# tum-vision/LDSO

Measured on AMD Instinct MI355X. Metric: GN iters/sec + Mresiduals/sec, 7-KF/2000-pt window, higher is better.
Workload: dtype f32; 1 GPU; C3: 7 KF x 2000 pt x 8 px, 640x480, R=12000, forced GN iterations, synthetic rank-6 marginalisation prior H_M/b_M; arithmetic=f32 residuals / Jacobians / accumulators as the reference, f64 stitch and solve, parallelism=1 GPU

## Files before the change

### ldso_amd/csrc/ba_api.hip

```cpp
#include "ba_host.h"
#include "lie_dev.h"

static thread_local std::string g_err;
void ldso_set_error(const std::string &s) { g_err = s; }

extern "C" {

int ldso_version(void) { return 100; }
const char *ldso_last_error(void) { return g_err.c_str(); }
int ldso_device_count(void) { int n = 0; if (hipGetDeviceCount(&n) != hipSuccess) return 0; return n; }

int ldso_settings_default(ldso_settings_t *s) {
    if (!s) return LDSO_E_INVALID;
    memset(s, 0, sizeof(*s));
    s->huberTH = 9; s->outlierTHSumComponent = 50 * 50; s->affineOptModeA = 1e12f; s->affineOptModeB = 1e8f;
    s->frameEnergyTHN = 0.7f; s->frameEnergyTHFacMedian = 1.5f; s->frameEnergyTHConstWeight = 0.5f; s->overallEnergyTHWeight = 1;
    s->initialCalibHessian = 5e9f; s->margWeightFac = 0.5f * 0.5f; s->idepthFixPriorMargFac = 600 * 600; s->thOptIterations = 1.2f;
    s->coarseCutoffTH = 20; s->minOptIterations = 1; s->solverMode = LDSO_SOLVER_FIX_LAMBDA | LDSO_SOLVER_ORTHOGONALIZE_X_LATER;
    s->forceAcceptStep = 1; s->solverModeDelta = 0.00001;
    return LDSO_OK;
}

int ldso_pyr_levels_used(int w, int h) {
    int wl = w, hl = h, lv = 1;
// ... 38 lines not shown
#define DA(ptr, n) do { int r_ = dalloc(H, &(ptr), (n)); if (r_ != LDSO_OK) return r_; } while (0)
static int down_reserve(ldso_ba *H, size_t bytes) {
    if (bytes <= H->downCap) return LDSO_OK;
    CHK(hipStreamSynchronize(H->stream));
    if (H->h_down) (void) hipHostFree(H->h_down);
    H->h_down = nullptr; H->downCap = 0;
    const size_t cap = bytes + bytes / 2 + 4096;
    CHK(hipHostMalloc((void **) &H->h_down, cap));
    H->downCap = cap;
    return LDSO_OK;
}
template <class T> static const T *down_put(ldso_ba *H, size_t &used, const T *src, size_t n, int &rc) {
    const size_t bytes = (n * sizeof(T) + 63) & ~(size_t) 63;
    const T *p = reinterpret_cast<const T *>(H->h_down + used);
    if (rc == LDSO_OK && n) { if (hipMemcpyAsync(H->h_down + used, src, n * sizeof(T), hipMemcpyDeviceToHost, H->stream) != hipSuccess) { ldso_set_error("hipMemcpyAsync (fetch) failed"); rc = LDSO_E_HIP; } }
    used += bytes;
    return p;
}

template <class T> static int d2h(ldso_ba *H, std::vector<T> &dst, const T *src, size_t n) {
    dst.resize(n);
    if (n == 0) return LDSO_OK;
    CHK(hipMemcpyAsync(dst.data(), src, n * sizeof(T), hipMemcpyDeviceToHost, H->stream));
    return LDSO_OK;
}
extern "C" {

static int alloc_set(ldso_ba *H, ResSet &S) {
    const size_t P = H->maxP, FS = H->FSmax, PS = P * FS, C = H->maxChunks;
    DA(S.slot, PS); DA(S.pt, P); DA(S.acc, P); DA(S.candE, P);
    DA(S.G, P * (8 * FS + LD_GEXTRA)); DA(S.topA, C * FS * LD_TOPN); DA(S.topL, C * FS * LD_TOPN);
    DA(S.chunkEnergy, C); DA(S.chunkCnt, C * 2); DA(S.chunkNID, C * 2);
    return LDSO_OK;
}

static int create_body(ldso_ba *H, int device, int w, int h, int max_frames, int max_points);

int ldso_ba_create(int device, int w, int h, int max_frames, int max_points, ldso_ba_t **out) {
    REQ(out && w > 8 && h > 8 && max_frames >= 2 && max_frames <= LD_MAXF && max_points > 0, "ldso_ba_create: bad arguments");
    *out = nullptr;
    int ndev = 0;
    if (hipGetDeviceCount(&ndev) != hipSuccess || ndev <= 0) { ldso_set_error("no HIP device visible"); return LDSO_E_NODEVICE; }
    REQ(device >= 0 && device < ndev, "ldso_ba_create: device index out of range");
    CHK(hipSetDevice(device));
    ldso_ba *H = new ldso_ba();
    { const char *e = getenv("LDSO_GN_GRAPHS"); if (e && e[0] == '0') H->gnUseGraphs = false; }
    const int r = create_body(H, device, w, h, max_frames, max_points);
    if (r != LDSO_OK) { const std::string keep = g_err; ldso_ba_destroy(H); g_err = keep; return r; }
    *out = H;
    return LDSO_OK;
}

static int create_body(ldso_ba *H, int device, int w, int h, int max_frames, int max_points) {
    H->device = device; H->w = w; H->h = h; H->maxF = max_frames; H->maxP = max_points;
    H->FSmax = (max_frames + 7) / 8 * 8;
    H->maxChunks = max_points / 4 + max_frames + 4;
    { hipDeviceProp_t pr; if (hipGetDeviceProperties(&pr, device) == hipSuccess && pr.multiProcessorCount > 0) H->numCU = pr.multiProcessorCount; }
    ldso_settings_default(&H->settings);
    CHK(hipStreamCreateWithFlags(&H->stream, hipStreamNonBlocking));
    H->ownStream = true;
    CHK(hipHostMalloc((void **) &H->h_item, sizeof(BatchItem)));
    { void *q_ = nullptr; CHK(hipMalloc(&q_, sizeof(BatchItem))); H->d_item = (BatchItem *) q_; }
    { void *q_ = nullptr; CHK(hipMalloc(&q_, (size_t) H->maxChunks * sizeof(BatchBlock))); H->d_blocks = (BatchBlock *) q_; }
    CHK(hipHostMalloc((void **) &H->h_stop, 4 * sizeof(int), hipHostMallocMapped));
    CHK(hipHostGetDevicePointer((void **) &H->d_stop, H->h_stop, 0));
    memset(&H->B, 0, sizeof(H->B));
    memset(&H->D, 0, sizeof(H->D));
    BaPtrs &B = H->B;
    const size_t F = max_frames, P = max_points, FS = H->FSmax, nmax = 8 * F + 4;
    DA(B.frames, F); DA(B.calib, 1); DA(B.pairs, F * F); DA(B.pairRt, F * F * 12);
    DA(B.adHost, F * F * 64); DA(B.adTarget, F * F * 64); DA(B.adHostF, F * F * 64); DA(B.adTargetF, F * F * 64);
    DA(B.nsProj, nmax * 7); DA(B.HM, nmax * nmax); DA(B.bM, nmax);
    DA(B.pgeo, P); DA(B.pcw, P * 8); DA(B.phost, P);
    DA(B.rtab, P * FS);
    DA(B.Jlin, P * FS); DA(B.rtz, P * FS * 8);
    DA(B.chunk_p0, H->maxChunks); DA(B.chunk_n, H->maxChunks); DA(B.chunk_host, H->maxChunks);
    DA(H->d_chunkStart, F + 2);
    DA(H->d_waitCtr, 4);
    DA(H->d_margFlags, P);
    DA(B.pairC, 2 * F * F * LD_PAIRC);
    const size_t GSPmax = (8 * FS + LD_GEXTRA + 15) / 16 * 16;
    DA(B.scPart, (size_t) LD_SC_SPLITS * GSPmax * GSPmax);
    DA(B.sys, 4 * (nmax * nmax + nmax));
    DA(B.acc, nmax * nmax + nmax); H->ownAcc = B.acc;
    DA(B.x, nmax); DA(B.xAd, F * F * 8); DA(B.xc, 4); DA(B.scalars, 16); DA(B.energyLog, 64);
    DA(H->d_dumpJ, P * FS);
    B.dumpJ = nullptr;
    int r;
    if ((r = alloc_set(H, H->sets[0])) != LDSO_OK) return r;
    if ((r = alloc_set(H, H->sets[1])) != LDSO_OK) return r;
    return LDSO_OK;
}

int ldso_ba_destroy(ldso_ba_t *H) {
    if (!H) return LDSO_OK;
    REQ(H->inBatch == nullptr, "ldso_ba_destroy: the handle is part of a live batch (ldso_ba_batch_destroy first: the batch dereferences its handles)");
    hipSetDevice(H->device);
    hipDeviceSynchronize();
    for (void *p : H->allocs) hipFree(p);
    for (int i = 0; i < LD_MAXF; i++) if (H->imgOwned[i] && H->imgSlots[i]) hipFree(H->imgSlots[i]);
    if (H->d_color) hipFree(H->d_color);
    if (H->h_item) hipHostFree(H->h_item);
    if (H->d_item) hipFree(H->d_item);
    if (H->d_blocks) hipFree(H->d_blocks);
    if (H->h_stop) hipHostFree(H->h_stop);
    if (H->h_down) hipHostFree(H->h_down);
    if (H->h_stage) hipHostFree(H->h_stage);
    if (H->d_stage) hipFree(H->d_stage);
    if (H->d_act) hipFree(H->d_act);
    if (H->d_sel) hipFree(H->d_sel);
    if (H->distBuf) hipFree(H->distBuf);
    if (H->d_p2pErr) hipFree(H->d_p2pErr);
    for (auto &t : H->timers) { hipEventDestroy(t.a); hipEventDestroy(t.b); }
    for (ldso_ba::GnGraph &g : H->gnGraphs) { hipGraphExecDestroy(g.exec); hipGraphDestroy(g.graph); }
    if (H->ownStream && H->stream) hipStreamDestroy(H->stream);
    delete H;
    return LDSO_OK;
}

int ldso_ba_set_stream(ldso_ba_t *H, void *s) {
    REQ(H, "null handle");
    CHK(hipSetDevice(H->device));
    if (H->stream && (H->ownStream || H->stageBusy)) { CHK(hipStreamSynchronize(H->stream)); H->stageBusy = false; }
    if (H->ownStream && H->stream && s) { hipStreamDestroy(H->stream); H->ownStream = false; }
    if (s) { H->stream = (hipStream_t) s; H->ownStream = false; }
    else if (!H->ownStream) { CHK(hipStreamCreateWithFlags(&H->stream, hipStreamNonBlocking)); H->ownStream = true; }
    return LDSO_OK;
}

int ldso_ba_set_settings(ldso_ba_t *H, const ldso_settings_t *s) {
    REQ(H && s, "null argument");
    if (s->solverMode & (LDSO_SOLVER_SVD | LDSO_SOLVER_ORTHOGONALIZE_SYSTEM | LDSO_SOLVER_ORTHOGONALIZE_POINTMARG | LDSO_SOLVER_ORTHOGONALIZE_FULL |
                         LDSO_SOLVER_MOMENTUM | LDSO_SOLVER_STEPMOMENTUM)) {
        ldso_set_error("solverMode bits SVD/ORTHOGONALIZE_SYSTEM/_POINTMARG/_FULL/MOMENTUM/STEPMOMENTUM are not provided by the device path");
        return LDSO_E_UNSUPPORTED;
    }
    H->settings = *s;
    return LDSO_OK;
}

static void rebind_slot(ldso_ba *H, int slot) {
    for (int f = 0; f < H->D.F && f < (int) H->imageSlot.size(); f++) if (H->imageSlot[f] == slot) H->B.img[f] = H->imgSlots[slot];
}

int ldso_ba_set_image(ldso_ba_t *H, int slot, const float *src) {
    REQ(H && src && slot >= 0 && slot < H->maxF, "ldso_ba_set_image: bad arguments");
    CHK(hipSetDevice(H->device));
    size_t bytes = (size_t) H->w * H->h * 3 * sizeof(float);
    if (!H->imgOwned[slot]) { void *p; CHK(hipMalloc(&p, bytes)); H->imgSlots[slot] = (float *) p; H->imgOwned[slot] = true; rebind_slot(H, slot); }
    CHK(hipMemcpyAsync(H->imgSlots[slot], src, bytes, hipMemcpyHostToDevice, H->stream));
    CHK(hipStreamSynchronize(H->stream));
    return LDSO_OK;
}

int ldso_ba_set_image_raw(ldso_ba_t *H, int slot, const float *irradiance) {
    REQ(H && irradiance && slot >= 0 && slot < H->maxF, "ldso_ba_set_image_raw: bad arguments");
    CHK(hipSetDevice(H->device));
    const size_t n = (size_t) H->w * H->h;
    if (!H->imgOwned[slot]) { void *q; CHK(hipMalloc(&q, n * 12)); H->imgSlots[slot] = (float *) q; H->imgOwned[slot] = true; rebind_slot(H, slot); }
    if (!H->d_color) CHK(hipMalloc(&H->d_color, n * sizeof(float)));
    CHK(hipMemcpyAsync(H->d_color, irradiance, n * sizeof(float), hipMemcpyHostToDevice, H->stream));
    float *lv[1] = {H->imgSlots[slot]};
    CHK(img_launch_make_images(H->d_color, H->w, H->h, 1, lv, H->stream));
    CHK(hipStreamSynchronize(H->stream));
    return LDSO_OK;
}

// ... 192 lines not shown
    if (rcD != LDSO_OK) return rcD;
    CHK(hipStreamSynchronize(H->stream));
    fetch_res_unpack(H, f, out, state_state, is_active, to_remove);
    return LDSO_OK;
}

int ldso_ba_get_points(ldso_ba_t *H, ldso_point_out_t *out) {
    REQ(H && out && H->D.P > 0, "bad arguments");
    CHK(hipSetDevice(H->device));
    RUN(down_reserve(H, fetch_pts_bytes(H)));
    size_t used = 0; int rcD = LDSO_OK;
    const FetchPts f = fetch_pts_put(H, used, rcD);
    if (rcD != LDSO_OK) return rcD;
    CHK(hipStreamSynchronize(H->stream));
    fetch_pts_unpack(H, f, out);
    return LDSO_OK;
}

int ldso_ba_get_frames(ldso_ba_t *H, ldso_frame_t *fr, double *step, double *cv, double *cs, double *pre) {
    REQ(H && H->D.F > 0, "no window");
    CHK(hipSetDevice(H->device));
    RUN(down_reserve(H, fetch_frm_bytes(H)));
    size_t used = 0; int rcD = LDSO_OK;
    const FetchFrm f = fetch_frm_put(H, used, rcD);
    if (rcD != LDSO_OK) return rcD;
    CHK(hipStreamSynchronize(H->stream));
    fetch_frm_unpack(H, f, fr, step, cv, cs, pre);
    return LDSO_OK;
}

int ldso_ba_get_results(ldso_ba_t *H, ldso_res_out_t *res, int32_t *state_state, int32_t *is_active, int32_t *to_remove, ldso_point_out_t *points,
                        ldso_frame_t *frames, double *step, double *calib_value, double *calib_step) {
    REQ(H && H->D.P > 0 && H->D.F > 0 && points, "ldso_ba_get_results: bad arguments");
    CHK(hipSetDevice(H->device));
    RUN(down_reserve(H, fetch_res_bytes(H) + fetch_pts_bytes(H) + fetch_frm_bytes(H)));
    size_t used = 0; int rcD = LDSO_OK;
    const FetchFrm ff = fetch_frm_put(H, used, rcD);
    const FetchPts fp = fetch_pts_put(H, used, rcD);
    const FetchRes fr_ = fetch_res_put(H, used, rcD);
    if (rcD != LDSO_OK) return rcD;
    CHK(hipStreamSynchronize(H->stream));
    fetch_frm_unpack(H, ff, frames, step, calib_value, calib_step, nullptr);
    fetch_pts_unpack(H, fp, points);
    fetch_res_unpack(H, fr_, res, state_state, is_active, to_remove);
    return LDSO_OK;
}

int ldso_ba_get_system(ldso_ba_t *H, double *HA, double *bA, double *HL, double *bL, double *Hsc, double *bsc, double *HF, double *bF, double *x) {
    REQ(H && H->D.n > 0, "no window");
    CHK(hipSetDevice(H->device));
    const size_t n = H->D.n, blk = n * n + n;
    std::vector<double> sys, xx;
    D2H(sys, H->B.sys, 4 * blk); D2H(xx, H->B.x, n);
    CHK(hipStreamSynchronize(H->stream));
    double *Hs[4] = {HA, HL, Hsc, HF}, *bs[4] = {bA, bL, bsc, bF};
    for (int m = 0; m < 4; m++) {
        if (Hs[m]) memcpy(Hs[m], sys.data() + m * blk, n * n * 8);
        if (bs[m]) memcpy(bs[m], sys.data() + m * blk + n * n, n * 8);
    }
    if (x) memcpy(x, xx.data(), n * 8);
    return LDSO_OK;
}

int ldso_ba_set_debug_split_launch(ldso_ba_t *H, int enable) {
    REQ(H, "null handle");
    H->noFusedLaunch = enable != 0;
    return LDSO_OK;
}

int ldso_ba_set_debug_dump(ldso_ba_t *H, int enable) {
    REQ(H, "null handle");
    H->B.dumpJ = enable ? H->d_dumpJ : nullptr;
    return LDSO_OK;
}

int ldso_ba_get_jacobians(ldso_ba_t *H, const int32_t *ids, int n, ldso_rawjac_t *out) {
    REQ(H && ids && out && n >= 0 && H->D.P > 0, "bad arguments");
    CHK(hipSetDevice(H->device));
    std::vector<ldso_rawjac_t> all;
    if (H->B.dumpJ == nullptr) {
        REQ(!H->pendingApply, "ldso_ba_get_jacobians: a linearisation is pending (call ldso_ba_apply_res first, or enable ldso_ba_set_debug_dump)");
        BaPtrs Bd = H->B;
        Bd.dumpJ = H->d_dumpJ;
        CHK(ba_launch_linearize(Bd, H->D, H->sets[H->cur], H->sets[H->cur ^ 1], H->settings, H->hasL, false, 0, GnInit{0, 0, 0.0f, -1}, H->stream));
    }
    D2H(all, H->d_dumpJ, (size_t) H->R);
    CHK(hipStreamSynchronize(H->stream));
    for (int i = 0; i < n; i++) { REQ(ids[i] >= 0 && ids[i] < H->R, "residual id out of range"); out[i] = all[ids[i]]; }
    return LDSO_OK;
}

int ldso_ba_get_precalc(ldso_ba_t *H, float *out) {
    REQ(H && out && H->D.F > 0, "bad arguments");
    CHK(hipSetDevice(H->device));
    const int F = H->D.F;
    std::vector<DevPair> dp;
    D2H(dp, H->B.pairs, (size_t) F * F);
    CHK(hipStreamSynchronize(H->stream));
    for (int i = 0; i < F * F; i++) {
        float *o = out + i * 27;
        memcpy(o, dp[i].KRKi, 36); memcpy(o + 9, dp[i].Kt, 12); memcpy(o + 12, dp[i].R0, 36); memcpy(o + 21, dp[i].t0, 12);
        o[24] = dp[i].aff[0]; o[25] = dp[i].aff[1]; o[26] = dp[i].b0;
    }
    return LDSO_OK;
}

int ldso_ba_get_pair_rt(ldso_ba_t *H, float *out) {
    REQ(H && out && H->D.F > 0, "bad arguments");
    CHK(hipSetDevice(H->device));
    const int F = H->D.F;
    std::vector<DevPair> dp;
    std::vector<float> rt;
    D2H(dp, H->B.pairs, (size_t) F * F);
    D2H(rt, H->B.pairRt, (size_t) F * F * 12);
    CHK(hipStreamSynchronize(H->stream));
    for (int i = 0; i < F * F; i++) { memcpy(out + i * 14, rt.data() + i * 12, 48); out[i * 14 + 12] = dp[i].aff[0]; out[i * 14 + 13] = dp[i].aff[1]; }
    return LDSO_OK;
}

int ldso_ba_get_counts(ldso_ba_t *H, int *a, int *l) {
    REQ(H, "null handle");
    double sc[16];
    RUN(read_scalars(H, sc));
    if (a) *a = (int) sc[9];
    if (l) *l = (int) sc[10];
    return LDSO_OK;
}

int ldso_ba_get_energy_log(ldso_ba_t *H, double *out, int cap) {
    REQ(H && out, "bad arguments");
    std::vector<double> e;
    D2H(e, H->B.energyLog, (size_t) 64);
    CHK(hipStreamSynchronize(H->stream));
    int n = H->lastIterations + 2;
    if (cap >= 64) { for (int i = 0; i < 64; i++) out[i] = e[i]; return n; }
    for (int i = 0; i < std::min(n, cap); i++) out[i] = e[i];
    return n;
}

}
```

### ldso_amd/csrc/ba_batch.hip

```cpp
#include "ba_host.h"

static int batch_refresh(ldso_ba_batch *Bt) {
    ldso_ba *H0 = Bt->h[0];
    const size_t n = Bt->h.size();
    for (int pass = 0; pass < 2; pass++) {
        int lin = 0, red = 0;
        for (size_t i = 0; i < n; i++) {
            ldso_ba *H = Bt->h[i];
            BatchItem &it = Bt->items[pass * n + i];
            if (pass == 1 && (int) i == Bt->n0) { Bt->halfChunks[0] = lin; Bt->halfReduce[0] = red; lin = 0; red = 0; }
            if (H->B.acc != H->ownAcc) H->B.acc = H->ownAcc;
            it.B = H->B; it.D = H->D; it.D.ks = Bt->ks; it.set[0] = H->sets[H->cur]; it.set[1] = H->sets[H->cur ^ 1]; it.cs = H->chunkStarts;
            it.hasPrior = H->hasPrior ? 1 : 0; it.GSP = H->GSP; it.linBlock0 = lin; it.redBlock0 = red; it.outSlot = (int32_t) i;
            lin += H->D.nChunks;
            red += reduce_grid(H->D.F, 0, Bt->ks, H->GSP).total;
        }
        if (pass == 0) { Bt->totalChunks = lin; Bt->totalReduce = red; }
        else if (Bt->n0 == (int) n) { Bt->halfChunks[0] = lin; Bt->halfReduce[0] = red; Bt->halfChunks[1] = 0; Bt->halfReduce[1] = 0; }
        else { Bt->halfChunks[1] = lin; Bt->halfReduce[1] = red; }
    }
    CHK(hipMemcpyAsync(Bt->d_items, Bt->items.data(), Bt->items.size() * sizeof(BatchItem), hipMemcpyHostToDevice, H0->stream));
    Bt->blocks.clear();
    for (size_t i = 0; i < n; i++) for (const BatchBlock &b : Bt->h[i]->h_blocks) Bt->blocks.push_back(BatchBlock{(int32_t) i, b.p0, b.np, b.host_chunk});
    for (size_t i = 0; i < n; i++) { const int32_t w = (int) i < Bt->n0 ? (int32_t) i : (int32_t) i - Bt->n0; for (const BatchBlock &b : Bt->h[i]->h_blocks) Bt->blocks.push_back(BatchBlock{w, b.p0, b.np, b.host_chunk}); }
    if (Bt->blocks.size() > Bt->blocksCap) {
        CHK(hipStreamSynchronize(H0->stream));
        if (Bt->aux) CHK(hipStreamSynchronize(Bt->aux));
        if (Bt->d_blocks) hipFree(Bt->d_blocks);
        Bt->d_blocks = nullptr; Bt->blocksCap = 0;
        void *q = nullptr;
        CHK(hipMalloc(&q, Bt->blocks.size() * sizeof(BatchBlock)));
        Bt->d_blocks = (BatchBlock *) q; Bt->blocksCap = Bt->blocks.size();
    }
    CHK(hipMemcpyAsync(Bt->d_blocks, Bt->blocks.data(), Bt->blocks.size() * sizeof(BatchBlock), hipMemcpyHostToDevice, H0->stream));
    if (Bt->balanced) {
        bool ok = (int) Bt->wg[0].size() >= 2 && Bt->wg[0].back() == Bt->totalChunks && Bt->wg[1].back() == Bt->halfChunks[0] && (Bt->halfChunks[1] == 0 || Bt->wg[2].back() == Bt->halfChunks[1]);
        REQ(ok, "ldso_ba_batch: the windows of the batch were re-chunked behind its back (ldso_ba_set_window / ldso_ba_set_chunk_points on a member): destroy and re-create the batch");
        std::vector<int32_t> all;
        for (int u = 0; u < 3; u++) { Bt->wgOff[u] = all.size(); Bt->nWG[u] = Bt->wg[u].empty() ? 0 : (int) Bt->wg[u].size() - 1; all.insert(all.end(), Bt->wg[u].begin(), Bt->wg[u].end()); }
        if (all.size() > Bt->wgCap) {
            CHK(hipStreamSynchronize(H0->stream));
            if (Bt->aux) CHK(hipStreamSynchronize(Bt->aux));
            if (Bt->d_wg) hipFree(Bt->d_wg);
            Bt->d_wg = nullptr; Bt->wgCap = 0;
            void *q = nullptr;
            CHK(hipMalloc(&q, all.size() * sizeof(int32_t)));
            Bt->d_wg = (int32_t *) q; Bt->wgCap = all.size();
        }
        Bt->wgHost.swap(all);
        CHK(hipMemcpyAsync(Bt->d_wg, Bt->wgHost.data(), Bt->wgHost.size() * sizeof(int32_t), hipMemcpyHostToDevice, H0->stream));
    }
    return LDSO_OK;
}

struct BalSeg { int owner, p0, n; };
static long balance_segments(const std::vector<BalSeg> &segs, int nWG, int c0, std::vector<std::vector<int32_t>> *cutsByOwner, std::vector<int32_t> *wg, std::vector<int32_t> *flatEnds) {
    long total = 0;
    for (const BalSeg &sg : segs) total += sg.n;
    auto run = [&](long budget, bool emit) -> bool {
        size_t si = 0; int used = 0;
        int blocks = 0;
        if (emit) { if (wg) wg->assign(1, 0); if (flatEnds) flatEnds->clear(); }
        for (int w = 0; w < nWG && si < segs.size(); w++) {
            long left = budget;
            while (si < segs.size()) {
                const int rem = segs[si].n - used;
                long can = left - c0;
                if (can < LD_WAVES && left != budget) break;
                if (can < 1) can = 1;
                int take = (int) std::min<long>(rem, can);
                if (take < rem) { take = std::max(take / LD_WAVES * LD_WAVES, 1); if (rem - take < LD_WAVES) take = rem; }
                if (emit) {
                    if (cutsByOwner) (*cutsByOwner)[(size_t) segs[si].owner].push_back(segs[si].p0 + used + take);
                    if (flatEnds) flatEnds->push_back(segs[si].p0 + used + take);
                }
                blocks++; left -= c0 + take; used += take;
                if (used == segs[si].n) { si++; used = 0; }
                if (left <= 0) break;
            }
            if (emit && wg) wg->push_back(blocks);
        }
        if (emit && wg) while ((int) wg->size() < nWG + 1) wg->push_back(blocks);
        return si == segs.size();
    };
    long lo = std::max<long>(1, total / std::max(nWG, 1)), hi = total + (long) c0 * (long) segs.size() + 1;
    while (lo < hi) { const long mid = (lo + hi) / 2; if (run(mid, false)) hi = mid; else lo = mid + 1; }
    run(lo, true);
    return lo;
}
static void balance_batch(ldso_ba *const *handles, int i0, int i1, int nWG, int c0, std::vector<std::vector<int32_t>> &cuts, std::vector<int32_t> &wg) {
    std::vector<BalSeg> segs;
    for (int i = i0; i < i1; i++) {
        const ldso_ba *H = handles[i];
        cuts[i].clear();
// ... 242 lines not shown
```

### ldso_amd/csrc/ba_dev.h

```cpp
#pragma once
#include <stdint.h>
#include "../../include/ldso_window.h"

#define LD_MAXF LDSO_MAX_FRAMES
#define LD_TOPN 91
#define LD_WAVES 8
#define LD_GEXTRA 8

struct DevPair {
    float KRKi[9];
    float Kt[3];
    float R0[9];
    float t0[3];
    float aff[2];
    float b0;
    float thMax;
    float dp[8];
};

struct DevFrame {
    double evalPT[12];
    double state[10], state_zero[10], state_backup[10], step[10];
    double prior[8], delta[8], delta_prior[8];
    double PRE_w2c[12], PRE_c2w[12];
// ... 43 lines not shown
static_assert(offsetof(PtRec, HdiF) == 0 && offsetof(PtRec, bdSumF) == 4 && offsetof(PtRec, idH) == 8 && offsetof(PtRec, nActive) == 12, "PtRec: lane 0's dwordx4");
static_assert(offsetof(PtRec, HcdA) == 16 && offsetof(PtRec, HcdL) == 32 && offsetof(PtRec, maxRelBS) == 48 && offsetof(PtRec, numGood) == 52, "PtRec: lanes 1..3");
static_assert(sizeof(PtAcc) == 16, "PtAcc: one dwordx4");
static_assert(offsetof(PtGeo, u) == 0 && offsetof(PtGeo, v) == 4 && offsetof(PtGeo, priorF) == 8 && offsetof(PtGeo, idepth) == 16 && offsetof(PtGeo, idepth_zero) == 20
              && offsetof(PtGeo, step) == 24 && offsetof(PtGeo, idepth_backup) == 28 && offsetof(PtGeo, lastHdiF) == 32 && offsetof(PtGeo, lastBdSumF) == 36 && offsetof(PtGeo, lastIdH) == 40,
              "PtGeo: dwords 0..7 are the scalar load, lane 1 stores dwords 4..7, lane 2 dwords 8..11");
static_assert(sizeof(PtCw) == 8, "PtCw: one dwordx2");

struct ResSet {
    SlotRec *slot;
    PtRec *pt;
    PtAcc *acc;
    float *candE;
    float *G;
    float *topA;
    float *topL;
    double *chunkEnergy;
    int32_t *chunkCnt;
    float *chunkNID;
};

struct BaDims {
    int32_t F, FS, P, R, n, GS, w, h, nChunks, nL, nsg;
    int32_t pBegin, pEnd;
    float wM3G, hM3G;
    int32_t ks;
};

struct BaPtrs {
    const float *img[LD_MAXF];
    DevFrame *frames;
    DevCalib *calib;
    DevPair *pairs;
    float *pairRt;
    double *adHost, *adTarget;
    float *adHostF, *adTargetF;
    double *nsProj;
    double *HM, *bM;
    PtGeo *pgeo;
    PtCw *pcw;
    SlotTab *rtab;
    int32_t *phost;
    ldso_rawjac_t *Jlin;
    float *rtz;
    int32_t *chunk_p0, *chunk_n;
    int32_t *chunk_host;
    double *pairC;
    float *scPart;
    double *sys;
    double *acc;
    double *x;
    float *xAd;
    float *xc;
    double *scalars;
    double *energyLog;
    ldso_rawjac_t *dumpJ;
};

struct ChunkStarts {
    int32_t v[LD_MAXF + 1];
};

struct LinHead {
    int32_t cs[LD_MAXF + 1];
    int32_t hostP0[LD_MAXF + 1];
    int32_t CH, F;
};

struct BatchBlock { int32_t win, p0, np, host_chunk; };

struct BatchItem {
    BaPtrs B;
    BaDims D;
    ResSet set[2];
    ChunkStarts cs;
    int32_t hasPrior, GSP, linBlock0, redBlock0;
    int32_t outSlot, pad_;
};

struct GnInit {
    int enable, hasPrior;
    float calibPrior;
    int itCheck;
};

#define LD_SC_STOP 11
#define LD_ITER_SKIPPED(B, itCheck) ((itCheck) >= 0 && (double) (itCheck) > (B).scalars[LD_SC_STOP])

#ifdef LDSO_STAMPS
#define LD_STAMP_ON 1
#else
#define LD_STAMP_ON 0
#endif

#define LD_PAIRC 296
#define LD_SC_SPLITS 16
#define LD_SCT_KS 8
#define LD_SYS_MATS 4

#ifdef __HIPCC__
struct ReduceGrid { int nPair, nTile, nExtra, total; };
__host__ __device__ inline int reduce_pairs(int F, int hasL) { return F * F * (hasL ? 2 : 1); }
__host__ __device__ inline int reduce_tiles(int ks, int GSP) { const int nT = GSP / 16; return ks * nT * (nT + 1) / 2; }
__host__ __device__ inline ReduceGrid reduce_grid(int F, int hasL, int ks, int GSP) {
    const int nTile = reduce_tiles(ks, GSP), nPair = reduce_pairs(F, hasL);
    return ReduceGrid{nPair, nTile, 1, nPair + nTile + 1};
}
#define LD_FUSED_CTL 2
__host__ __device__ inline int optimize_iteration_cap(int F, int mnumOptIts, int forceAll) {
    if (!forceAll) { if (F < 3) mnumOptIts = 20; if (F < 4) mnumOptIts = 15; }
    return mnumOptIts;
}
template <int LINES> __device__ __forceinline__ void ld_touch_kernarg();
template <> __device__ __forceinline__ void ld_touch_kernarg<8>() {
    const unsigned long long ka = (unsigned long long) __builtin_amdgcn_kernarg_segment_ptr();
    int t0, t1, t2, t3, t4, t5, t6, t7;
    asm volatile("s_load_dword %0, %8, 0x0\n\ts_load_dword %1, %8, 0x40\n\ts_load_dword %2, %8, 0x80\n\ts_load_dword %3, %8, 0xc0\n\ts_load_dword %4, %8, 0x100\n\ts_load_dword %5, %8, 0x140\n\ts_load_dword %6, %8, 0x180\n\ts_load_dword %7, %8, 0x1c0\n\ts_waitcnt lgkmcnt(0)"
                 : "=&s"(t0), "=&s"(t1), "=&s"(t2), "=&s"(t3), "=&s"(t4), "=&s"(t5), "=&s"(t6), "=&s"(t7) : "s"(ka) : "memory");
}
template <> __device__ __forceinline__ void ld_touch_kernarg<10>() {
    const unsigned long long ka = (unsigned long long) __builtin_amdgcn_kernarg_segment_ptr();
    int t0, t1, t2, t3, t4, t5, t6, t7, t8, t9;
    asm volatile("s_load_dword %0, %10, 0x0\n\ts_load_dword %1, %10, 0x40\n\ts_load_dword %2, %10, 0x80\n\ts_load_dword %3, %10, 0xc0\n\ts_load_dword %4, %10, 0x100\n\ts_load_dword %5, %10, 0x140\n\ts_load_dword %6, %10, 0x180\n\ts_load_dword %7, %10, 0x1c0\n\ts_load_dword %8, %10, 0x200\n\ts_load_dword %9, %10, 0x240\n\ts_waitcnt lgkmcnt(0)"
                 : "=&s"(t0), "=&s"(t1), "=&s"(t2), "=&s"(t3), "=&s"(t4), "=&s"(t5), "=&s"(t6), "=&s"(t7), "=&s"(t8), "=&s"(t9) : "s"(ka) : "memory");
}
template <> __device__ __forceinline__ void ld_touch_kernarg<12>() {
    const unsigned long long ka = (unsigned long long) __builtin_amdgcn_kernarg_segment_ptr();
    int t0, t1, t2, t3, t4, t5, t6, t7, t8, t9, t10, t11;
    asm volatile("s_load_dword %0, %12, 0x0\n\ts_load_dword %1, %12, 0x40\n\ts_load_dword %2, %12, 0x80\n\ts_load_dword %3, %12, 0xc0\n\ts_load_dword %4, %12, 0x100\n\ts_load_dword %5, %12, 0x140\n\ts_load_dword %6, %12, 0x180\n\ts_load_dword %7, %12, 0x1c0\n\ts_load_dword %8, %12, 0x200\n\ts_load_dword %9, %12, 0x240\n\ts_load_dword %10, %12, 0x280\n\ts_load_dword %11, %12, 0x2c0\n\ts_waitcnt lgkmcnt(0)"
                 : "=&s"(t0), "=&s"(t1), "=&s"(t2), "=&s"(t3), "=&s"(t4), "=&s"(t5), "=&s"(t6), "=&s"(t7), "=&s"(t8), "=&s"(t9), "=&s"(t10), "=&s"(t11) : "s"(ka) : "memory");
}
template <> __device__ __forceinline__ void ld_touch_kernarg<14>() {
    const unsigned long long ka = (unsigned long long) __builtin_amdgcn_kernarg_segment_ptr();
    int t0, t1, t2, t3, t4, t5, t6, t7, t8, t9, t10, t11, t12, t13;
    asm volatile("s_load_dword %0, %14, 0x0\n\ts_load_dword %1, %14, 0x40\n\ts_load_dword %2, %14, 0x80\n\ts_load_dword %3, %14, 0xc0\n\ts_load_dword %4, %14, 0x100\n\ts_load_dword %5, %14, 0x140\n\ts_load_dword %6, %14, 0x180\n\ts_load_dword %7, %14, 0x1c0\n\ts_load_dword %8, %14, 0x200\n\ts_load_dword %9, %14, 0x240\n\ts_load_dword %10, %14, 0x280\n\ts_load_dword %11, %14, 0x2c0\n\ts_load_dword %12, %14, 0x300\n\ts_load_dword %13, %14, 0x340\n\ts_waitcnt lgkmcnt(0)"
                 : "=&s"(t0), "=&s"(t1), "=&s"(t2), "=&s"(t3), "=&s"(t4), "=&s"(t5), "=&s"(t6), "=&s"(t7), "=&s"(t8), "=&s"(t9), "=&s"(t10), "=&s"(t11), "=&s"(t12), "=&s"(t13) : "s"(ka) : "memory");
}
template <> __device__ __forceinline__ void ld_touch_kernarg<16>() {
    const unsigned long long ka = (unsigned long long) __builtin_amdgcn_kernarg_segment_ptr();
    int t0, t1, t2, t3, t4, t5, t6, t7, t8, t9, t10, t11, t12, t13, t14, t15;
    asm volatile("s_load_dword %0, %16, 0x0\n\ts_load_dword %1, %16, 0x40\n\ts_load_dword %2, %16, 0x80\n\ts_load_dword %3, %16, 0xc0\n\ts_load_dword %4, %16, 0x100\n\ts_load_dword %5, %16, 0x140\n\ts_load_dword %6, %16, 0x180\n\ts_load_dword %7, %16, 0x1c0\n\ts_load_dword %8, %16, 0x200\n\ts_load_dword %9, %16, 0x240\n\ts_load_dword %10, %16, 0x280\n\ts_load_dword %11, %16, 0x2c0\n\ts_load_dword %12, %16, 0x300\n\ts_load_dword %13, %16, 0x340\n\ts_load_dword %14, %16, 0x380\n\ts_load_dword %15, %16, 0x3c0\n\ts_waitcnt lgkmcnt(0)"
                 : "=&s"(t0), "=&s"(t1), "=&s"(t2), "=&s"(t3), "=&s"(t4), "=&s"(t5), "=&s"(t6), "=&s"(t7), "=&s"(t8), "=&s"(t9), "=&s"(t10), "=&s"(t11), "=&s"(t12), "=&s"(t13), "=&s"(t14), "=&s"(t15) : "s"(ka) : "memory");
}
#endif
```

### ldso_amd/csrc/ba_host.h

```cpp
#pragma once
#include <hip/hip_runtime.h>
#include <vector>
#include <string>
#include <cstring>
#include <cstdio>
#include <cmath>
#include <algorithm>
#include "../../include/ldso_hip.h"
#include "ba_dev.h"
#include "pyramid.h"
#include "ba_solve.h"

void ldso_set_error(const std::string &s);
#define CHK(call) do { hipError_t e_ = (call); if (e_ != hipSuccess) { ldso_set_error(std::string(#call) + ": " + hipGetErrorString(e_)); return LDSO_E_HIP; } } while (0)
#define REQ(cond, msg) do { if (!(cond)) { ldso_set_error(msg); return LDSO_E_INVALID; } } while (0)
#define RUN(x) do { int r_ = (x); if (r_ != LDSO_OK) return r_; } while (0)

template <class Kernel, class... Args>
hipError_t launch_lds(Kernel kernel, dim3 grid, dim3 block, size_t ldsBytes, hipStream_t st, const Args &... args) {
    if (ldsBytes > 48 * 1024) (void) hipFuncSetAttribute((const void *) kernel, hipFuncAttributeMaxDynamicSharedMemorySize, (int) ldsBytes);
    hipLaunchKernelGGL(kernel, grid, block, ldsBytes, st, args...);
    return hipGetLastError();
}

hipError_t ba_launch_linearize(const BaPtrs &B, const BaDims &D, const ResSet &cur, const ResSet &nxt, const ldso_settings_t &S, bool hasL, bool fix, int stepMode, const GnInit &gi, hipStream_t st);
hipError_t ba_launch_reduce(const BaPtrs &B, const BaDims &D, const ResSet &S, const ChunkStarts &chunkStart, bool hasL, int GSP, int atomicMode, bool hasPrior, float calibPrior, double l1, double il, int itCheck, hipStream_t st);
hipError_t ba_launch_gather(const BaPtrs &B, const BaDims &D, const ResSet &S, bool hasL, bool hasPrior, int GSP, double lambda, const ldso_settings_t &St, int mode, double *rbuf, hipStream_t st);
hipError_t ba_launch_solve(const BaPtrs &B, const BaDims &D, const ResSet &S, const ldso_settings_t &St, const SolveArgs &A, hipStream_t st);
hipError_t ba_launch_point_step(const BaPtrs &B, const BaDims &D, const ResSet &S, int mode, hipStream_t st);
hipError_t ba_launch_linearize_one(const BaPtrs &B, const BaDims &D, const ResSet &cur, const ResSet &nxt, const ldso_settings_t &S, int stepMode, const GnInit &gi, const LinHead &hd, hipStream_t st);
hipError_t ba_launch_linearize_marg(const BaPtrs &B, const BaDims &D, const ResSet &cur, const ResSet &nxt, const ldso_settings_t &S, const int32_t *margFlags, hipStream_t st);
hipError_t ba_launch_marg_frame(const BaPtrs &B, const BaDims &D, int idx, double *work, double *outH, double *outb, hipStream_t st);
hipError_t ba_launch_acc_init(const BaPtrs &B, const BaDims &D, const GnInit &gi, hipStream_t st);
hipError_t ba_launch_gn_export(const BaPtrs &B, const BaDims &D, const ResSet &S, double *tail, hipStream_t st);
hipError_t ba_launch_activate(const BaPtrs &B, const BaDims &D, const ldso_settings_t &S, const ldso_immature_t *d_pts, ldso_activation_t *d_out, int n, int minObs, float minIdepthH_act, int GNIts, hipStream_t st);
hipError_t ba_launch_activate_selected(const BaPtrs &B, const BaDims &D, const ldso_settings_t &S, const ldso_immature_t *d_pts, const int32_t *d_sel, const int32_t *d_nSel, ldso_activation_t *d_out, int nMax, int minObs, float minIdepthH_act, int GNIts, hipStream_t st);
hipError_t ba_launch_linearize_batch(const BatchItem *d_items, const BatchBlock *d_blocks, int totalChunks, const int32_t *d_wgStart, int nWG, int FS, int cur, const ldso_settings_t &S, int stepMode, float calibPrior, hipStream_t st, int itCheck = -1);
hipError_t ba_launch_reduce_batch(const BatchItem *d_items, int nWin, int totalBlocks, int cur, float calibPrior, double l1, double il, hipStream_t st, int itCheck = -1);
hipError_t ba_launch_gn_solve_batch(const BatchItem *d_items, int nWin, const BaDims &Dmax, int cur, const ldso_settings_t &St, int iteration, double lambda, hipStream_t st, int logIdx = -1, int itCheck = -1);
hipError_t ba_launch_batch_begin(const BatchItem *d_items, int nWin, int mnumOptIts, int forceAll, hipStream_t st);
hipError_t ba_launch_solve_batch(const BatchItem *d_items, int nWin, const BaDims &Dmax, const ldso_settings_t &St, unsigned flags, int phase, double *d_scalarsOut, hipStream_t st);
hipError_t ba_launch_linearize_batch_fix(const BatchItem *d_items, const BatchBlock *d_blocks, int totalChunks, const int32_t *d_wgStart, int nWG, const ldso_settings_t &S, float calibPrior, hipStream_t st);
hipError_t ba_launch_lm_energies(const BaPtrs &B, const BaDims &D, const ResSet &S, float calibPrior, bool hasPrior, hipStream_t st);
hipError_t ba_launch_marg_update(const BaPtrs &B, const BaDims &D, double w, hipStream_t st);
hipError_t ba_launch_gn_solve(const BaPtrs &B, const BaDims &D, const ResSet &S, const ldso_settings_t &St, const SolveArgs &A, hipStream_t st);
hipError_t ba_launch_reduce_solve(const BaPtrs &B, const BaDims &D, const ResSet &S, const ldso_settings_t &St, const SolveArgs &A, const ChunkStarts &chunkStart, int atomicMode, float calibPrior, double l1, double il, hipStream_t st);

struct Timer { hipEvent_t a, b; int which; };
struct ldso_ba {
    int device = 0, w = 0, h = 0, maxF = 0, maxP = 0, FSmax = 0, maxChunks = 0, numCU = 256;
    hipStream_t stream = nullptr;
    bool ownStream = false;
    ldso_settings_t settings;
    BaDims D;
    BaPtrs B;
    ResSet sets[2];
    int cur = 0;
    bool pendingApply = false;
    bool hasL = false;
    bool hasPrior = false;
    int GSP = 0;
    int R = 0;
    float *imgSlots[LD_MAXF] = {nullptr};
    bool imgOwned[LD_MAXF] = {false};
    int32_t *d_chunkStart = nullptr;
    int *d_waitCtr = nullptr;
    int32_t *d_margFlags = nullptr;
    float *d_color = nullptr;
    void *d_act = nullptr;
    int actCap = 0;
    void *d_sel = nullptr;
    size_t selCap = 0, selMapOffset = 0;
    int selW1 = 0, selH1 = 0;
    int selLdsLimit = -1, selLdsSet = 0;
    std::vector<char> selHost;
    double *ownAcc = nullptr;
    ChunkStarts chunkStarts;
    ldso_rawjac_t *d_dumpJ = nullptr;
    std::vector<int32_t> flat2slot;
    std::vector<int32_t> imageSlot;
    std::vector<void *> allocs;
    std::vector<int32_t> h_phost;
    BatchItem *d_item = nullptr, *h_item = nullptr;
    BatchBlock *d_blocks = nullptr;
    std::vector<BatchBlock> h_blocks;
    bool appliedValid = false;
    LinHead linHead;
    int reduceSplits = LD_SCT_KS;
    bool linHeadOk = false;
    const void *inBatch = nullptr;
    int chunkPoints = 0;
    std::vector<int32_t> chunkCuts;
    BatchItem itemShadow;
    bool itemValid = false;
    int *h_stop = nullptr, *d_stop = nullptr;
    char *h_down = nullptr;
    size_t downCap = 0;
    bool stageBusy = false;
    struct NewPoint { ldso_point_t p; int before; std::vector<ldso_residual_t> res; float mrb; int32_t ngr; };
    struct WindowEdit {
        bool active = false;
        int oF = 0, oP = 0;
        std::vector<char> frameGone, rowGone;
        std::vector<int32_t> insertedSlots;
        std::vector<uint32_t> mask;
        std::vector<NewPoint> fresh;
    } edit;
    char *h_stage = nullptr, *d_stage = nullptr;
    size_t stageCap = 0;
    bool profile = false;
    std::vector<Timer> timers;
    double tsum[5] = {0, 0, 0, 0, 0};
    int tcnt[5] = {0, 0, 0, 0, 0};
    int lastIterations = 0;
    bool noFusedLaunch = false;
    struct GnGraph { unsigned long long sig; std::vector<unsigned char> key; hipGraphExec_t exec; hipGraph_t graph; };
    std::vector<GnGraph> gnGraphs;
    std::vector<unsigned char> gnKeyScratch;
    bool gnUseGraphs = true;
    double *distBuf = nullptr;
    unsigned p2pSeq = 0;
    int *d_p2pErr = nullptr;
    double neverStop = 1e300;
};

#define REQ_UNSHARDED(name) REQ(H->D.pBegin == 0 && H->D.pEnd == H->D.P, name ": not available on a sharded handle (ldso_ba_set_shard): " \
                                    "use ldso_ba_gn_reduce_local / ldso_ba_gn_solve_reduced or ldso_ba_reduce_local / ldso_ba_solve_reduced around the all-reduce")

struct ldso_ba_batch {
    std::vector<ldso_ba *> h;
    BatchItem *d_items = nullptr;
    std::vector<BatchItem> items;
    BatchBlock *d_blocks = nullptr;
    std::vector<BatchBlock> blocks;
    size_t blocksCap = 0;
    int chunkPoints = 0;
    int totalChunks = 0, totalReduce = 0, FS = 0, cur = 0;
    int n0 = 0;
    int ks = LD_SCT_KS;
    int halfChunks[2] = {0, 0}, halfReduce[2] = {0, 0};
    std::vector<int32_t> wg[3];
    int32_t *d_wg = nullptr; size_t wgCap = 0;
    std::vector<int32_t> wgHost;
    int nWG[3] = {0, 0, 0}; size_t wgOff[3] = {0, 0, 0};
    bool balanced = false;
    hipStream_t aux = nullptr;
    hipEvent_t ev0 = nullptr, ev1 = nullptr, evEnd = nullptr;
    BaDims Dmax;
    double *d_scalars = nullptr, *h_scalars = nullptr;
};

struct ldso_tracer {
    int device = 0, w = 0, h = 0, maxPoints = 0, n = 0;
    hipStream_t stream = nullptr;
    ldso_trace_settings_t settings;
    ldso_immature_t *d_pts = nullptr, *d_alt = nullptr;
    float *d_type = nullptr, *d_typeAlt = nullptr;
    unsigned char *d_keep = nullptr, *d_flag = nullptr;
    int32_t *d_cmp = nullptr;
    int nAfterCompact = 0;
    float *d_img = nullptr, *d_color = nullptr, *d_pose = nullptr;
    const float *img = nullptr;
    int *d_counts = nullptr;
    bool haveFrame = false;
};

#pragma GCC visibility push(hidden)
int trace_compact_enqueue(ldso_tracer *T, const unsigned char *d_keep8, const int32_t *d_keep32, int keepValue, int n_hosts, bool haveMap, hipStream_t st);
void trace_compact_finish(ldso_tracer *T);
int build_chunks(ldso_ba *H);
int rechunk(ldso_ba *H);
void t_begin(ldso_ba *H, int which);
void t_end(ldso_ba *H);
int launch_linearize(ldso_ba *H, bool fix, int stepMode = 0, int itCheck = -1);
int launch_reduce(ldso_ba *H, const ResSet &S, bool atomicMode = false, double lambda = 0.0, int itCheck = -1);
int launch_gather(ldso_ba *H, const ResSet &S, double lambda, int mode, double *rbuf);
int launch_solve(ldso_ba *H, const ResSet &S, unsigned flags, int iteration = 0, double lambda = 0, int logIdx = -1, double *rout = nullptr, const double *rin = nullptr);
int launch_pstep(ldso_ba *H, const ResSet &S, int mode);
int refresh_item(ldso_ba *H);
int read_scalars(ldso_ba *H, double *sc);
SolveArgs solve_args(const ldso_ba *H, unsigned flags);
struct Damping { double lam, l1, il; };
Damping damping(const ldso_settings_t &St, double lambda);
GnInit gn_init(const ldso_ba *H, int itCheck);
int lend_acc(ldso_ba *H, double *buf);
template <class Launch> int time_launches(hipStream_t st, int reps, double *avg_us, Launch launch) {
    hipEvent_t a, b;
    CHK(hipEventCreate(&a)); CHK(hipEventCreate(&b));
    RUN(launch());
    CHK(hipEventRecord(a, st));
    for (int i = 0; i < reps; i++) RUN(launch());
    CHK(hipEventRecord(b, st));
    CHK(hipEventSynchronize(b));
    float ms = 0;
    CHK(hipEventElapsedTime(&ms, a, b));
    (void) hipEventDestroy(a); (void) hipEventDestroy(b);
    *avg_us = (double) ms * 1e3 / reps;
    return LDSO_OK;
}
#pragma GCC visibility pop
```

### ldso_amd/csrc/ba_linearize.hip

```cpp
#include <hip/hip_runtime.h>
#include <type_traits>
#include "ba_host.h"

#define RES_IN 0
#define RES_OOB 1
#define RES_OUTLIER 2

__device__ __forceinline__ float dpp_row_shr1(float x) {
    return __builtin_bit_cast(float, __builtin_amdgcn_update_dpp(0, __builtin_bit_cast(int, x), 0x111, 0xF, 0xF, true));
}
__device__ __forceinline__ float dpp_quad_xor1(float x) {
    return __builtin_bit_cast(float, __builtin_amdgcn_update_dpp(0, __builtin_bit_cast(int, x), 0xB1, 0xF, 0xF, true));
}
__device__ __forceinline__ float dpp_quad_xor2(float x) {
    return __builtin_bit_cast(float, __builtin_amdgcn_update_dpp(0, __builtin_bit_cast(int, x), 0x4E, 0xF, 0xF, true));
}
__device__ __forceinline__ float dpp_quad_xor3(float x) {
    return __builtin_bit_cast(float, __builtin_amdgcn_update_dpp(0, __builtin_bit_cast(int, x), 0x1B, 0xF, 0xF, true));
}
__device__ __forceinline__ float dpp_half_mirror(float x) {
    return __builtin_bit_cast(float, __builtin_amdgcn_update_dpp(0, __builtin_bit_cast(int, x), 0x141, 0xF, 0xF, true));
}
__device__ __forceinline__ float sum8(float x) {
    x += dpp_quad_xor1(x);
// ... 135 lines not shown
#pragma unroll
        for (int g = 0; g < NSG; g++) {
            if constexpr (FIX || HAS_L) {
                const v4i32_t t4 = AT(rtab + (size_t) pU * FS, g * 8 + s);
                q.rflat[g] = t4.x; q.rlin[g] = t4.y; q.rnew[g] = FIX ? t4.z : 0; q.rlidx[g] = HAS_L ? t4.w : 0;
            } else {
                const v2i32_t t2 = AT((const v2i32_t *) (rtab + (size_t) pU * FS), (g * 8 + s) * 2);
                q.rflat[g] = t2.x; q.rlin[g] = t2.y; q.rnew[g] = 0; q.rlidx[g] = 0;
            }
        }
    }
    {
        const v16i_t s0 = ldg16<DESC, OFF_S0>(&cur);
        const v2f_t *slots = GP(const v2f_t, s0, RS_SLOT);
        const float *pts = GP(const float, s0, RS_PT);
        q.rrec = AT(pts + (size_t) pU * (sizeof(PtRec) / 4), lane & 15u);
#pragma unroll
        for (int g = 0; g < NSG; g++) {
            const v2f_t e = AT(slots + (size_t) pU * FS * 8, (g * 8 + s) * 8 + k);
            q.jp[g] = e.x; q.m[g] = e.y;
        }
    }
}

struct PairIn {
    float rgeo, rrec, colA, wgtA, colB, wgtB;
    int rfA0, rfB0, rf1;
    float jpA0, mA0, jpB0, mB0, jp1, m1;
};
template <bool DESC>
static __device__ __forceinline__ void load_pair(PairIn &q, const BaPtrs &B, const ResSet &cur, unsigned FS, unsigned pA, unsigned dAB, unsigned s, unsigned k, unsigned lane) {
    const unsigned pU = (unsigned) __builtin_amdgcn_readfirstlane((int) pA), dU = (unsigned) __builtin_amdgcn_readfirstlane((int) dAB);
    const unsigned hoff = (lane & 32u) ? dU : 0u;
    const unsigned s1 = 8u + (s & 3u);
    {
        const v16i_t b0 = ldg16<DESC, OFF_B0>(&B);
        const float *geo = GP(const float, b0, BP_GEO);
        const v2f_t *pcw = GP(const v2f_t, b0, BP_CW);
        const v2i32_t *rtab = (const v2i32_t *) GP(const v4i32_t, b0, BP_RTAB);
        q.rgeo = AT(geo + (size_t) pU * (sizeof(PtGeo) / 4), hoff * (unsigned) (sizeof(PtGeo) / 4) + (lane & 15u));
        const v2f_t ca = AT(pcw + (size_t) pU * 8, k), cb = AT(pcw + (size_t) pU * 8, dU * 8u + k);
        q.colA = ca.x; q.wgtA = ca.y; q.colB = cb.x; q.wgtB = cb.y;
        q.rfA0 = AT(rtab + (size_t) pU * FS * 2, s * 2u).x;
        q.rfB0 = AT(rtab + (size_t) pU * FS * 2, (dU * FS + s) * 2u).x;
        q.rf1 = AT(rtab + (size_t) pU * FS * 2, (hoff * FS + s1) * 2u).x;
    }
    {
        const v16i_t s0 = ldg16<DESC, OFF_S0>(&cur);
        const v2f_t *slots = GP(const v2f_t, s0, RS_SLOT);
        const float *pts = GP(const float, s0, RS_PT);
        q.rrec = AT(pts + (size_t) pU * (sizeof(PtRec) / 4), hoff * (unsigned) (sizeof(PtRec) / 4) + (lane & 15u));
        const v2f_t a0 = AT(slots + (size_t) pU * FS * 8, s * 8u + k), b0_ = AT(slots + (size_t) pU * FS * 8, (dU * FS + s) * 8u + k);
        const v2f_t p1 = AT(slots + (size_t) pU * FS * 8, (hoff * FS + s1) * 8u + k);
        q.jpA0 = a0.x; q.mA0 = a0.y; q.jpB0 = b0_.x; q.mB0 = b0_.y; q.jp1 = p1.x; q.m1 = p1.y;
    }
}

struct TapsG { float t[12]; float Ku, Kv; };
struct Hit { float h0, h1, h2, Ku, Kv; };
struct PtStep { float idp, idz; };

template <int NSG, bool HAS_L, bool FIX, bool MARG, bool DESC, bool ONE = false, bool PAIR = false>
static __device__ __forceinline__ void linearize_body(const BaPtrs &B, const BaDims &D, const ResSet &cur, const ResSet &nxt, const ldso_settings_t &S, const int stepMode,
                                                      const GnInit &gi, const int32_t *__restrict__ margFlags, const int chunk, const int gridBlocks,
                                                      const int p0, const int np, const int h) {
    if (LD_ITER_SKIPPED(B, gi.itCheck)) return;
    extern __shared__ __attribute__((aligned(16))) float smem[];
    const int FS = D.FS, F = D.F;
    int tid_ = (int) threadIdx.x;
    asm volatile("" : "+v"(tid_));
    const int tid = tid_, wave = tid >> 6, lane = tid & 63, s = lane >> 3, k = lane & 7;
    const long long t0_ = wall_clock64();
#define LSTAMP(i) do { if (LD_STAMP_ON && chunk == 0 && tid == 0) B.energyLog[8 + (i)] = (double) (wall_clock64() - t0_); } while (0)

    DevPair *sPair = (DevPair *) smem;
    float *sAd = smem + FS * (sizeof(DevPair) / 4);
    float *sRed = sAd + 2 * FS * 64;
    float *sTopL = sRed + LD_WAVES * FS * LD_TOPN;
    float *sXa = sTopL + (HAS_L ? LD_WAVES * FS * LD_TOPN : 0);
    const float **sImg = (const float **) (sXa + FS * 8 + LD_TAIL_FLOATS);
    float *sRec = (float *) (sImg + FS);

    if (gi.enable) {
        const int n = D.n, N1 = n * n + n, per = (N1 + gridBlocks - 1) / gridBlocks;
        const int z0 = chunk * per, z1 = min(N1, z0 + per);
        for (int e = z0 + tid; e < z1; e += blockDim.x) {
            double v = 0.0;
            if (e < n * n) {
                const int i = e / n, j = e % n;
                if (j <= i && gi.enable == 1) {
                    if (gi.hasPrior) v = B.HM[e];
                    if (i == j) { v += (i < 4) ? (double) gi.calibPrior : B.frames[(i - 4) >> 3].prior[(i - 4) & 7]; }
                }
            }
            B.acc[e] = v;
        }
    }
    const float fx = B.calib->sf[0], fy = B.calib->sf[1], cx = B.calib->sf[2], cy = B.calib->sf[3];
    const float fxi = B.calib->si[0], fyi = B.calib->si[1];
    const float cD0 = B.calib->cDeltaF[0], cD1 = B.calib->cDeltaF[1], cD2 = B.calib->cDeltaF[2], cD3 = B.calib->cDeltaF[3];
    float xc0 = 0, xc1 = 0, xc2 = 0, xc3 = 0;
    if (stepMode & 1) { xc0 = B.xc[0]; xc1 = B.xc[1]; xc2 = B.xc[2]; xc3 = B.xc[3]; }

    const int waveU = __builtin_amdgcn_readfirstlane(wave);
    PtIn<NSG> qa = {}, qb = {}, qc = {};
    int pi = waveU;
    if (!PAIR && pi < np) load_point<NSG, HAS_L, FIX, DESC>(qa, B, cur, FS, p0 + pi, s, k, lane);

    {
        constexpr int PW = (int) (sizeof(DevPair) / 4), TH_OFF = (int) (offsetof(DevPair, thMax) / 4);
        constexpr int NPB = (LD_MAXF * PW + 64 * LD_WAVES - 1) / (64 * LD_WAVES), NAB = (LD_MAXF * 64) / (64 * LD_WAVES);
        const float thHost = B.frames[h].frameEnergyTH;
        float pv[NPB], ahv[NAB], atv[NAB], xav = 0.0f;
#pragma unroll
        for (int u = 0; u < NPB; u++) {
            const int i = tid + u * 64 * LD_WAVES, t = i / PW, o = i % PW;
            float v = 0.0f;
            if (i < FS * PW && t < F) {
                v = (o == TH_OFF) ? fmaxf(thHost, B.frames[t].frameEnergyTH) : ((const float *) &B.pairs[h * F + t])[o];
            }
            pv[u] = v;
        }
#pragma unroll
        for (int u = 0; u < NAB; u++) {
            const int i = tid + u * 64 * LD_WAVES, t = i >> 6, o = i & 63;
            const bool in = (i < FS * 64) && (t < F);
            ahv[u] = in ? B.adHostF[(h + t * F) * 64 + o] : 0.0f;
            atv[u] = in ? B.adTargetF[(h + t * F) * 64 + o] : 0.0f;
        }
        if ((stepMode & 1) && tid < FS * 8) xav = ((tid >> 3) < F) ? B.xAd[(size_t) (h * F + (tid >> 3)) * 8 + (tid & 7)] : 0.0f;
#pragma unroll
        for (int u = 0; u < NPB; u++) { const int i = tid + u * 64 * LD_WAVES; if (i < FS * PW) ((float *) sPair)[i] = pv[u]; }
#pragma unroll
        for (int u = 0; u < NAB; u++) {
            const int i = tid + u * 64 * LD_WAVES;
            if (i < FS * 64) { const int kk = (i >> 3) & 7, e = (i & ~7) | ((i ^ kk) & 7); sAd[2 * e] = atv[u]; sAd[2 * e + 1] = ahv[u]; }
        }
        if ((stepMode & 1) && tid < FS * 8) sXa[tid] = xav;
        if (tid < FS) sImg[tid] = B.img[(tid < F) ? tid : 0];
    }
    if (HAS_L) for (int i = tid; i < LD_WAVES * FS * LD_TOPN; i += blockDim.x) sTopL[i] = 0.0f;
    __syncthreads();
    LSTAMP(1);

    const int ox = (k == 1 || k == 6) ? -1 : (k == 2) ? 1 : (k == 3) ? -2 : (k == 5) ? 2 : 0;
    const int oy = (k == 0) ? -2 : (k == 1 || k == 2) ? -1 : (k == 6) ? 1 : (k == 7) ? 2 : 0;
    const int W = D.w;
    const float wM3G = D.wM3G, hM3G = D.hM3G;
    const unsigned GSu = (unsigned) D.GS;
    ldso_rawjac_t *const dumpJ = B.dumpJ;
    const int a16 = (lane ^ 16) << 2, a32 = (lane ^ 32) << 2;

    float accR[NSG][18];
#pragma unroll
    for (int g = 0; g < NSG; g++)
#pragma unroll
        for (int i = 0; i < 18; i++) accR[g][i] = 0.0f;
    double energySum = 0.0;
    int nresA = 0, nresL = 0;
    float nidSum = 0.0f;
    int nidCnt = 0;

    using LM0 = std::false_type;
    auto qgeo = [&](auto lc, const PtIn<NSG> &q, const int i) -> float { if constexpr (decltype(lc)::value) return q.ls[i * 4]; else return RLF(q.rgeo, i); };
    auto qrec = [&](auto lc, const PtIn<NSG> &q, const int i) -> float { if constexpr (decltype(lc)::value) return q.ls[i * 4 + 1]; else return RLF(q.rrec, i); };
    auto qreci = [&](auto lc, const PtIn<NSG> &q, const int i) -> int { const float f_ = qrec(lc, q, i); return __builtin_bit_cast(int, f_); };
    auto qmlane = [&](auto lc, auto jc, const PtIn<NSG> &q, const int g) -> float {
// ... 678 lines not shown
                do one_point(); while (pi < np);
            }
            }
        }
#if LD_STAMP_ON
        if (chunk == 0 && tid == 0) for (int u = 0; u < 6; u++) B.energyLog[24 + u] = (double) cy_[u];
#endif
    }

    LSTAMP(6);
#pragma unroll
    for (int g = 0; g < NSG; g++) {
        float *cell = sRed + (size_t) (wave * FS + g * 8 + s) * LD_TOPN;
        const int b1 = k * 13 - (k * (k - 1)) / 2 - k;
        const int r2 = k + 8, b2 = r2 * 13 - (r2 * (r2 - 1)) / 2 - r2;
#pragma unroll
        for (int c = 0; c < 13; c++) if (c >= k) cell[b1 + c] = accR[g][c];
#pragma unroll
        for (int c = 8; c < 13; c++) if (k < 5 && c >= r2) cell[b2 + c] = accR[g][13 + c - 8];
    }
    double *sE = (double *) (sXa + FS * 8);
    int *sC = (int *) (sE + LD_WAVES);
    float *sN = (float *) (sC + 4 * LD_WAVES);
    {
        double e = energySum;
        int na = nresA, nl = nresL;
        for (int o = 32; o > 0; o >>= 1) { double e2 = __shfl_xor(e, o, 64); int a2 = __shfl_xor(na, o, 64), l2 = __shfl_xor(nl, o, 64); e += e2; na += a2; nl += l2; }
        if (lane == 0) { sE[wave] = e; sC[wave * 4 + 0] = na; sC[wave * 4 + 1] = nl; sC[wave * 4 + 2] = nidCnt; sN[wave] = nidSum; }
    }
    __syncthreads();
    LSTAMP(7);
    const v16i_t e2 = ldg16<DESC, OFF_S0>(&nxt);
    float *o_topA = GP(float, e2, RS_TOPA), *o_topL = GP(float, e2, RS_TOPL);
    double *o_chunkE = GP(double, e2, RS_CHUNKE);
    for (int i = tid; i < FS * LD_TOPN; i += blockDim.x) {
        float a = 0;
#pragma unroll
        for (int wv = 0; wv < LD_WAVES; wv++) a += sRed[wv * FS * LD_TOPN + i];
        if constexpr (PAIR) {
            const int t_ = i / LD_TOPN;
            if (t_ >= 12) a = 0.0f;
            else if (t_ >= 8) {
#pragma unroll
                for (int wv = 0; wv < LD_WAVES; wv++) a += sRed[wv * FS * LD_TOPN + i + 4 * LD_TOPN];
            }
        }
        o_topA[(size_t) chunk * FS * LD_TOPN + i] = a;
        if (HAS_L) {
            float l = 0;
#pragma unroll
            for (int wv = 0; wv < LD_WAVES; wv++) l += sTopL[wv * FS * LD_TOPN + i];
            o_topL[(size_t) chunk * FS * LD_TOPN + i] = l;
        }
    }
    if (tid == 0) {
        double e = 0; int na = 0, nl = 0, nc = 0; float ns = 0;
        for (int wv = 0; wv < LD_WAVES; wv++) { e += sE[wv]; na += sC[wv * 4 + 0]; nl += sC[wv * 4 + 1]; nc += sC[wv * 4 + 2]; ns += sN[wv]; }
        o_chunkE[chunk] = e;
        const v4i_t e3 = ldg4<DESC, (int) offsetof(ResSet, chunkCnt)>(&nxt);
        int32_t *o_cnt = GP(int32_t, e3, 0); float *o_nid = GP(float, e3, 1);
        o_cnt[chunk * 2 + 0] = na; o_cnt[chunk * 2 + 1] = nl;
        o_nid[chunk * 2 + 0] = ns; o_nid[chunk * 2 + 1] = (float) nc;
    }
}

template <int NSG, bool HAS_L, bool FIX, bool MARG>
__global__ __launch_bounds__(64 * LD_WAVES) void k_linearize(BaPtrs B, BaDims D, ResSet cur, ResSet nxt, ldso_settings_t S, int stepMode, GnInit gi,
                                                             const int32_t *__restrict__ margFlags) {
    static_assert(sizeof(BaPtrs) + sizeof(BaDims) + 2 * sizeof(ResSet) + sizeof(ldso_settings_t) + sizeof(GnInit) + 256 >= 14 * 64 - 60, "k_linearize: ld_touch_kernarg<14> must stay inside the explicit arguments + the 256 bytes of hidden arguments behind them (the kernel uses dynamic LDS: the whole hidden block is part of its kernarg segment)");
    ld_touch_kernarg<14>();
    const int chunk = (int) blockIdx.x;
    linearize_body<NSG, HAS_L, FIX, MARG, false>(B, D, cur, nxt, S, stepMode, gi, margFlags, chunk, (int) gridDim.x, B.chunk_p0[chunk], B.chunk_n[chunk], B.chunk_host[chunk]);
}

template <int NSG>
__global__ __launch_bounds__(64 * LD_WAVES) void k_linearize_batch(const BatchItem *__restrict__ items, const BatchBlock *__restrict__ blocks, const int32_t *__restrict__ wgStart, int cur,
                                                                   ldso_settings_t S, int stepMode, float calibPrior, int itCheck) {
    int b0 = (int) blockIdx.x, b1 = b0 + 1;
    if (wgStart != nullptr) { b0 = wgStart[blockIdx.x]; b1 = wgStart[blockIdx.x + 1]; }
#pragma clang loop unroll(disable)
    for (int b = b0; b < b1; b++) {
        const BatchBlock bb = blocks[b];
        const BatchItem &it = items[bb.win];
        GnInit gi; gi.enable = 1; gi.hasPrior = it.hasPrior; gi.calibPrior = calibPrior; gi.itCheck = itCheck;
        linearize_body<NSG, false, false, false, true>(it.B, it.D, it.set[cur], it.set[cur ^ 1], S, stepMode, gi, nullptr, bb.host_chunk >> 8, it.D.nChunks, bb.p0, bb.np, bb.host_chunk & 0xFF);
        __syncthreads();
    }
}

__global__ __launch_bounds__(64 * LD_WAVES) void k_linearize_batch_fix(const BatchItem *__restrict__ items, const BatchBlock *__restrict__ blocks, const int32_t *__restrict__ wgStart,
                                                                       ldso_settings_t S, float calibPrior) {
    int b0 = (int) blockIdx.x, b1 = b0 + 1;
    if (wgStart != nullptr) { b0 = wgStart[blockIdx.x]; b1 = wgStart[blockIdx.x + 1]; }
#pragma clang loop unroll(disable)
    for (int b = b0; b < b1; b++) {
        const BatchBlock bb = blocks[b];
        const BatchItem &it = items[bb.win];
        const int applied = __builtin_amdgcn_readfirstlane((int) it.B.scalars[LD_SC_STOP]) & 1;
        GnInit gi; gi.enable = 1; gi.hasPrior = it.hasPrior; gi.calibPrior = calibPrior; gi.itCheck = -1;
        linearize_body<1, false, true, false, true>(it.B, it.D, it.set[applied], it.set[applied ^ 1], S, 0, gi, nullptr, bb.host_chunk >> 8, it.D.nChunks, bb.p0, bb.np, bb.host_chunk & 0xFF);
        __syncthreads();
    }
}

struct OneArgs { BaPtrs B; BaDims D; ResSet cur, nxt; ldso_settings_t S; int stepMode; GnInit gi; LinHead hd; };
template <int NSG, bool PAIR = false>
__global__ __launch_bounds__(64 * LD_WAVES) void k_linearize_one(OneArgs a) {
    const OneArgs &A = *(const OneArgs *) __builtin_amdgcn_kernarg_segment_ptr();
    static_assert(sizeof(OneArgs) >= 12 * 64 && sizeof(OneArgs) <= 16 * 64, "k_linearize_one: 16 lines = the explicit arguments (>= 768 bytes) + the 256 bytes of hidden arguments behind them");
    ld_touch_kernarg<16>();
    const LinHead &hd = a.hd;
    const int chunk = (int) blockIdx.x;
    int h = 0;
#pragma unroll
    for (int i = 1; i < LD_MAXF; i++) h += (i < hd.F && chunk >= hd.cs[i]) ? 1 : 0;
    int c0 = 0, q0 = 0, q1 = 0;
#pragma unroll
    for (int i = 0; i < LD_MAXF; i++) { const bool m = (i == h); c0 = m ? hd.cs[i] : c0; q0 = m ? hd.hostP0[i] : q0; q1 = m ? hd.hostP0[i + 1] : q1; }
    const int p0 = q0 + (chunk - c0) * hd.CH, np = min(hd.CH, q1 - p0);
    linearize_body<NSG, false, false, false, true, true, PAIR>(A.B, A.D, A.cur, A.nxt, a.S, a.stepMode, a.gi, nullptr, chunk, (int) gridDim.x, p0, np, h);
}

size_t ba_linearize_lds_bytes(int FS, bool hasL, bool stash = false) {
    size_t fl = (size_t) FS * (sizeof(DevPair) / 4) + 2 * (size_t) FS * 64 + (size_t) LD_WAVES * FS * LD_TOPN + (hasL ? (size_t) LD_WAVES * FS * LD_TOPN : 0) + (size_t) FS * 8 + LD_TAIL_FLOATS + 2 * (size_t) FS;
    return fl * sizeof(float) + 256 + ((stash && FS == 8) ? (size_t) LD_WAVES * 4096 : 0);
}

template <int NSG, bool HAS_L, bool FIX, bool MARG = false>
static hipError_t launch_one(const BaPtrs &B, const BaDims &D, const ResSet &cur, const ResSet &nxt, const ldso_settings_t &S, int stepMode, const GnInit &gi, hipStream_t st,
                            const int32_t *margFlags = nullptr) {
    return launch_lds(k_linearize<NSG, HAS_L, FIX, MARG>, dim3(D.nChunks), dim3(64 * LD_WAVES), ba_linearize_lds_bytes(D.FS, HAS_L), st, B, D, cur, nxt, S, stepMode, gi, margFlags);
}

hipError_t ba_launch_linearize(const BaPtrs &B, const BaDims &D, const ResSet &cur, const ResSet &nxt, const ldso_settings_t &S,
                               bool hasL, bool fix, int stepMode, const GnInit &gi, hipStream_t st) {
    if (D.nChunks == 0) return hipSuccess;
    if (D.nsg == 1) {
        if (hasL) return fix ? launch_one<1, true, true>(B, D, cur, nxt, S, stepMode, gi, st) : launch_one<1, true, false>(B, D, cur, nxt, S, stepMode, gi, st);
        return fix ? launch_one<1, false, true>(B, D, cur, nxt, S, stepMode, gi, st) : launch_one<1, false, false>(B, D, cur, nxt, S, stepMode, gi, st);
    } else {
        if (hasL) return fix ? launch_one<2, true, true>(B, D, cur, nxt, S, stepMode, gi, st) : launch_one<2, true, false>(B, D, cur, nxt, S, stepMode, gi, st);
        return fix ? launch_one<2, false, true>(B, D, cur, nxt, S, stepMode, gi, st) : launch_one<2, false, false>(B, D, cur, nxt, S, stepMode, gi, st);
    }
}

hipError_t ba_launch_linearize_one(const BaPtrs &B, const BaDims &D, const ResSet &cur, const ResSet &nxt, const ldso_settings_t &S, int stepMode, const GnInit &gi, const LinHead &hd,
                                   hipStream_t st) {
    if (D.nChunks == 0) return hipSuccess;
    const size_t lds = ba_linearize_lds_bytes(D.FS, false);
    OneArgs a;
    a.B = B; a.D = D; a.cur = cur; a.nxt = nxt; a.S = S; a.stepMode = stepMode; a.gi = gi; a.hd = hd;
    const dim3 grid(D.nChunks), block(64 * LD_WAVES);
    if (D.nsg == 1) return launch_lds(k_linearize_one<1>, grid, block, lds, st, a);
    if (D.F <= 12) return launch_lds(k_linearize_one<2, true>, grid, block, lds, st, a);
    return launch_lds(k_linearize_one<2>, grid, block, lds, st, a);
}

hipError_t ba_launch_linearize_marg(const BaPtrs &B, const BaDims &D, const ResSet &cur, const ResSet &nxt, const ldso_settings_t &S, const int32_t *margFlags,
                                    hipStream_t st) {
    if (D.nChunks == 0) return hipSuccess;
    const GnInit gi{0, 0, 0.0f};
    if (D.nsg == 1) return launch_one<1, false, false, true>(B, D, cur, nxt, S, 0, gi, st, margFlags);
    return launch_one<2, false, false, true>(B, D, cur, nxt, S, 0, gi, st, margFlags);
}

hipError_t ba_launch_linearize_batch(const BatchItem *d_items, const BatchBlock *d_blocks, int totalChunks, const int32_t *d_wgStart, int nWG, int FS, int cur, const ldso_settings_t &S, int stepMode,
                                     float calibPrior, hipStream_t st, int itCheck) {
    if (totalChunks == 0) return hipSuccess;
    const size_t lds = ba_linearize_lds_bytes(FS, false, true);
    const int grid = d_wgStart != nullptr ? nWG : totalChunks;
    if (grid <= 0) return hipSuccess;
    if (FS == 8) return launch_lds(k_linearize_batch<1>, dim3(grid), dim3(64 * LD_WAVES), lds, st, d_items, d_blocks, d_wgStart, cur, S, stepMode, calibPrior, itCheck);
    return launch_lds(k_linearize_batch<2>, dim3(grid), dim3(64 * LD_WAVES), lds, st, d_items, d_blocks, d_wgStart, cur, S, stepMode, calibPrior, itCheck);
}

hipError_t ba_launch_linearize_batch_fix(const BatchItem *d_items, const BatchBlock *d_blocks, int totalChunks, const int32_t *d_wgStart, int nWG, const ldso_settings_t &S, float calibPrior, hipStream_t st) {
    if (totalChunks == 0) return hipSuccess;
    const size_t lds = ba_linearize_lds_bytes(8, false, true);
    const int grid = d_wgStart != nullptr ? nWG : totalChunks;
    if (grid <= 0) return hipSuccess;
    return launch_lds(k_linearize_batch_fix, dim3(grid), dim3(64 * LD_WAVES), lds, st, d_items, d_blocks, d_wgStart, S, calibPrior);
}
```

### ldso_amd/csrc/ba_optimize.hip

```cpp
#include "ba_host.h"

void t_begin(ldso_ba *H, int which) {
    if (!H->profile) return;
    Timer t; t.which = which;
    hipEventCreate(&t.a); hipEventCreate(&t.b);
    hipEventRecord(t.a, H->stream);
    H->timers.push_back(t);
}
void t_end(ldso_ba *H) { if (H->profile) hipEventRecord(H->timers.back().b, H->stream); }

int launch_solve(ldso_ba *H, const ResSet &S, unsigned flags, int iteration, double lambda, int logIdx, double *rout, const double *rin) {
    SolveArgs A = solve_args(H, flags);
    A.iteration = iteration; A.lambda = lambda; A.logIdx = logIdx; A.reduceOut = rout; A.reduceIn = rin;
    t_begin(H, 2);
    CHK(ba_launch_solve(H->B, H->D, S, H->settings, A, H->stream));
    t_end(H);
    return LDSO_OK;
}
int refresh_item(ldso_ba *H) {
    BatchItem it;
    memset(&it, 0, sizeof(it));
    it.B = H->B; it.D = H->D; it.set[0] = H->sets[0]; it.set[1] = H->sets[1]; it.cs = H->chunkStarts;
    it.hasPrior = H->hasPrior ? 1 : 0; it.GSP = H->GSP; it.linBlock0 = 0; it.redBlock0 = 0;
    if (H->itemValid && memcmp(&it, &H->itemShadow, sizeof(it)) == 0) return LDSO_OK;
    CHK(hipStreamSynchronize(H->stream));
    memcpy(H->h_item, &it, sizeof(it));
    CHK(hipMemcpyAsync(H->d_item, H->h_item, sizeof(it), hipMemcpyHostToDevice, H->stream));
    H->itemShadow = it; H->itemValid = true;
    return LDSO_OK;
}

int launch_linearize(ldso_ba *H, bool fix, int stepMode, int itCheck) {
    t_begin(H, 0);
    const GnInit gi = gn_init(H, itCheck);
    if (!fix && !H->hasL && gi.enable == 1 && H->linHeadOk && H->B.dumpJ == nullptr) {
        CHK(ba_launch_linearize_one(H->B, H->D, H->sets[H->cur], H->sets[H->cur ^ 1], H->settings, stepMode, gi, H->linHead, H->stream));
    } else
    CHK(ba_launch_linearize(H->B, H->D, H->sets[H->cur], H->sets[H->cur ^ 1], H->settings, H->hasL, fix, stepMode, gi, H->stream));
    t_end(H);
    if (H->profile) { t_begin(H, 4); t_end(H); }
    return LDSO_OK;
}
int launch_reduce(ldso_ba *H, const ResSet &S, bool atomicMode, double lambda, int itCheck) {
    t_begin(H, 1);
    const Damping d = damping(H->settings, lambda);
    CHK(ba_launch_reduce(H->B, H->D, S, H->chunkStarts, H->hasL, H->GSP, atomicMode ? ((H->D.pBegin > 0) ? 2 : 1) : 0, H->hasPrior, H->settings.initialCalibHessian, d.l1, d.il, itCheck, H->stream));
    t_end(H);
    return LDSO_OK;
}
int launch_gather(ldso_ba *H, const ResSet &S, double lambda, int mode, double *rbuf) {
    t_begin(H, 1);
    CHK(ba_launch_gather(H->B, H->D, S, H->hasL, H->hasPrior, H->GSP, lambda, H->settings, mode, rbuf, H->stream));
    t_end(H);
    return LDSO_OK;
}
int launch_pstep(ldso_ba *H, const ResSet &S, int mode) {
    t_begin(H, 3);
    CHK(ba_launch_point_step(H->B, H->D, S, mode, H->stream));
    t_end(H);
    return LDSO_OK;
}

int read_scalars(ldso_ba *H, double *sc) {
    CHK(hipMemcpyAsync(sc, H->B.scalars, 16 * sizeof(double), hipMemcpyDeviceToHost, H->stream));
    CHK(hipStreamSynchronize(H->stream));
    return LDSO_OK;
}
SolveArgs solve_args(const ldso_ba *H, unsigned flags) {
    SolveArgs A;
    A.flags = flags; A.hasL = H->hasL ? 1 : 0; A.hasPrior = H->hasPrior ? 1 : 0; A.GSP = H->GSP;
    return A;
}
Damping damping(const ldso_settings_t &St, double lam) {
    if (St.solverMode & LDSO_SOLVER_USE_GN) lam = 0;
    if (St.solverMode & LDSO_SOLVER_FIX_LAMBDA) lam = 1e-5;
    return Damping{lam, 1 + lam, (double) (1.0f / (1 + lam))};
}
GnInit gn_init(const ldso_ba *H, int itCheck) {
    GnInit gi; gi.enable = (H->D.pBegin > 0) ? 2 : 1; gi.hasPrior = H->hasPrior ? 1 : 0; gi.calibPrior = H->settings.initialCalibHessian; gi.itCheck = itCheck;
    return gi;
}
int lend_acc(ldso_ba *H, double *buf) {
    if (H->B.acc == buf) return LDSO_OK;
    H->B.acc = buf;
    CHK(ba_launch_acc_init(H->B, H->D, gn_init(H, -1), H->stream));
    return LDSO_OK;
}

extern "C" {

int ldso_ba_time_linearize(ldso_ba_t *H, int reps, double *avg_us) {
    REQ(H && H->D.P > 0 && reps > 0 && avg_us, "bad arguments");
    CHK(hipSetDevice(H->device));
    REQ(!H->pendingApply, "ldso_ba_time_linearize: a linearizeAll result is pending");
    const bool prof = H->profile;
    H->profile = false;
    const int rc = time_launches(H->stream, reps, avg_us, [H] { return launch_linearize(H, false, 0); });
    H->profile = prof;
    return rc;
}

int ldso_ba_collect_active(ldso_ba_t *H) {
    REQ(H && H->D.P > 0, "no window");
    CHK(hipSetDevice(H->device));
    H->pendingApply = false;
    return launch_solve(H, H->sets[H->cur], SK_COLLECT);
}

int ldso_ba_linearize_all(ldso_ba_t *H, int fix, double *energy_out) {
    REQ(H && H->D.P > 0, "no window");
    CHK(hipSetDevice(H->device));
    RUN(launch_linearize(H, fix != 0));
    RUN(launch_solve(H, H->sets[H->cur ^ 1], SK_POST | SK_THRESH));
    H->pendingApply = true;
    if (fix) { H->cur ^= 1; H->pendingApply = false; H->appliedValid = true; }
    double sc[16];
    RUN(read_scalars(H, sc));
    if (energy_out) *energy_out = sc[0];
    if (!std::isfinite(sc[0])) return LDSO_E_NONFINITE;
    return LDSO_OK;
}

int ldso_ba_apply_res(ldso_ba_t *H) {
    REQ(H, "null handle");
    if (H->pendingApply) { H->cur ^= 1; H->pendingApply = false; H->appliedValid = true; }
    return LDSO_OK;
}

int ldso_ba_backup_state(ldso_ba_t *H) {
    REQ(H && H->D.P > 0, "no window");
    CHK(hipSetDevice(H->device));
    RUN(launch_solve(H, H->sets[H->cur], SK_BACKUP));
    RUN(launch_pstep(H, H->sets[H->cur], PS_BACKUP));
    return LDSO_OK;
}

int ldso_ba_solve_system(ldso_ba_t *H, int iteration, double lambda) {
    REQ(H && H->D.P > 0, "no window");
    REQ_UNSHARDED("ldso_ba_solve_system");
    CHK(hipSetDevice(H->device));
    const ResSet &S = H->sets[H->cur];
    RUN(launch_reduce(H, S));
    RUN(launch_gather(H, S, lambda, 0, nullptr));
    RUN(launch_solve(H, S, SK_SOLVE, iteration, lambda));
    RUN(launch_pstep(H, S, PS_RESUB));
    double sc[16];
    RUN(read_scalars(H, sc));
    if (sc[4] != 0.0) return LDSO_E_NONFINITE;
    return LDSO_OK;
}

int ldso_ba_do_step(ldso_ba_t *H, int *canbreak) {
    REQ(H && H->D.P > 0, "no window");
    CHK(hipSetDevice(H->device));
    RUN(launch_solve(H, H->sets[H->cur], SK_STEP | SK_PRECALC));
    RUN(launch_pstep(H, H->sets[H->cur], PS_STEP));
    double sc[16];
    RUN(read_scalars(H, sc));
    if (canbreak) *canbreak = sc[3] != 0.0;
    return LDSO_OK;
}

int ldso_ba_load_state_backup(ldso_ba_t *H) {
    REQ(H && H->D.P > 0, "no window");
    CHK(hipSetDevice(H->device));
    RUN(launch_solve(H, H->sets[H->cur], SK_LOADBK | SK_PRECALC));
    RUN(launch_pstep(H, H->sets[H->cur], PS_LOAD));
    H->pendingApply = false;
    return LDSO_OK;
}

static int enqueue_iteration(ldso_ba *H, int iteration, double lambda, int logIdx, int itCheck = -1, int lastIt = -1) {
    const ResSet &S = H->sets[H->cur];
    RUN(lend_acc(H, H->ownAcc));
    SolveArgs A = solve_args(H, 0);
    A.iteration = iteration; A.lambda = lambda; A.logIdx = logIdx; A.itCheck = itCheck; A.hostStop = (itCheck >= 0) ? H->d_stop : nullptr; A.lastIt = lastIt;
    if (reduce_grid(H->D.F, H->hasL, H->D.ks, H->GSP).total + LD_FUSED_CTL <= H->numCU && !H->noFusedLaunch) {
        A.waitCtr = H->d_waitCtr;
        const Damping d = damping(H->settings, lambda);
        t_begin(H, 2);
        CHK(ba_launch_reduce_solve(H->B, H->D, S, H->settings, A, H->chunkStarts, (H->D.pBegin > 0) ? 2 : 1, H->settings.initialCalibHessian, d.l1, d.il, H->stream));
        t_end(H);
    } else {
        RUN(launch_reduce(H, S, true, lambda, itCheck));
        t_begin(H, 2);
        CHK(ba_launch_gn_solve(H->B, H->D, S, H->settings, A, H->stream));
        t_end(H);
    }
    RUN(launch_linearize(H, false, 1, itCheck));
    H->cur ^= 1; H->appliedValid = true;
    return LDSO_OK;
}

static unsigned long long fnv1a(unsigned long long h, const void *p, size_t n) {
    const unsigned char *b = (const unsigned char *) p;
    for (size_t i = 0; i < n; i++) { h ^= b[i]; h *= 1099511628211ull; }
    return h;
}
static void gn_key(const ldso_ba *H, int first_iteration, int iters, std::vector<unsigned char> &key) {
    key.clear();
    auto put = [&key](const void *p, size_t n) { const unsigned char *b = (const unsigned char *) p; key.insert(key.end(), b, b + n); };
    put(&H->B, sizeof(H->B)); put(&H->D, sizeof(H->D)); put(H->sets, sizeof(H->sets)); put(&H->settings, sizeof(H->settings));
    put(&H->chunkStarts, sizeof(H->chunkStarts)); put(&H->linHead, sizeof(H->linHead));
    const long long misc[12] = {first_iteration, iters, H->cur, H->hasL, H->hasPrior, H->GSP, H->linHeadOk, H->noFusedLaunch, H->numCU, (long long) (size_t) H->stream, (long long) (size_t) H->ownAcc,
                                (long long) (size_t) H->d_waitCtr};
    put(misc, sizeof(misc));
}
static unsigned long long gn_signature(const std::vector<unsigned char> &key) { return fnv1a(1469598103934665603ull, key.data(), key.size()); }
static int enqueue_gn_plain(ldso_ba *H, int first_iteration, int iters) {
    CHK(hipMemsetAsync(H->d_waitCtr, 0, 4 * sizeof(int), H->stream));
    for (int i = 0; i < iters; i++) RUN(enqueue_iteration(H, first_iteration + i, 1e-1, -1));
    return LDSO_OK;
}
int ldso_ba_enqueue_gn(ldso_ba_t *H, int first_iteration, int iters) {
    REQ(H && H->D.P > 0 && iters >= 0, "bad arguments");
    REQ_UNSHARDED("ldso_ba_enqueue_gn");
    CHK(hipSetDevice(H->device));
    hipStreamCaptureStatus cs = hipStreamCaptureStatusNone;
    if (!H->gnUseGraphs || H->profile || iters < 2 || H->B.acc != H->ownAcc || hipStreamIsCapturing(H->stream, &cs) != hipSuccess || cs != hipStreamCaptureStatusNone)
        return enqueue_gn_plain(H, first_iteration, iters);
    std::vector<unsigned char> &key = H->gnKeyScratch;
    gn_key(H, first_iteration, iters, key);
    const unsigned long long sig = gn_signature(key);
    for (ldso_ba::GnGraph &g : H->gnGraphs)
        if (g.sig == sig && g.key == key) {
            CHK(hipGraphLaunch(g.exec, H->stream));
            if (iters & 1) H->cur ^= 1;
            H->appliedValid = true;
            return LDSO_OK;
        }
    const int cur0 = H->cur;
    hipGraph_t graph = nullptr;
    if (hipStreamBeginCapture(H->stream, hipStreamCaptureModeThreadLocal) != hipSuccess) { (void) hipGetLastError(); return enqueue_gn_plain(H, first_iteration, iters); }
    const int rc = enqueue_gn_plain(H, first_iteration, iters);
    const hipError_t ec = hipStreamEndCapture(H->stream, &graph);
    hipGraphExec_t exec = nullptr;
    if (rc != LDSO_OK || ec != hipSuccess || graph == nullptr || hipGraphInstantiate(&exec, graph, nullptr, nullptr, 0) != hipSuccess) {
        (void) hipGetLastError();
        if (graph) hipGraphDestroy(graph);
        H->cur = cur0;
        H->gnUseGraphs = false;
        return enqueue_gn_plain(H, first_iteration, iters);
    }
    if (H->gnGraphs.size() >= 4) { hipGraphExecDestroy(H->gnGraphs.front().exec); hipGraphDestroy(H->gnGraphs.front().graph); H->gnGraphs.erase(H->gnGraphs.begin()); }
    H->gnGraphs.push_back(ldso_ba::GnGraph{sig, key, exec, graph});
    CHK(hipGraphLaunch(exec, H->stream));
    return LDSO_OK;
}

int ldso_ba_calc_lm_energies(ldso_ba_t *H, double *energy_M, double *energy_L) {
    REQ(H && H->D.P > 0, "no window");
    CHK(hipSetDevice(H->device));
    CHK(ba_launch_lm_energies(H->B, H->D, H->sets[H->cur], H->settings.initialCalibHessian, H->hasPrior, H->stream));
    double sc[16];
    RUN(read_scalars(H, sc));
    if (energy_M) *energy_M = sc[12];
    if (energy_L) *energy_L = sc[13];
    return LDSO_OK;
}

static int optimize_lm(ldso_ba *H, int mnumOptIts, int force_all, float *rmse_out, int *iters_out) {
    mnumOptIts = optimize_iteration_cap(H->D.F, mnumOptIts, force_all);
    REQ(mnumOptIts + 2 < 64, "too many iterations");
    std::vector<double> elog;
    RUN(ldso_ba_collect_active(H));
    double lastE = 0, lastL = 0, lastM = 0;
    RUN(ldso_ba_linearize_all(H, 0, &lastE));
    RUN(ldso_ba_calc_lm_energies(H, &lastM, &lastL));
    elog.push_back(lastE);
    RUN(ldso_ba_apply_res(H));
    double lambda = 1e-1;
    int done = 0;
    for (int it = 0; it < mnumOptIts; it++) {
        RUN(ldso_ba_backup_state(H));
        RUN(ldso_ba_solve_system(H, it, lambda));
        int canbreak = 0;
        RUN(ldso_ba_do_step(H, &canbreak));
        double newE = 0, newL = 0, newM = 0;
        RUN(ldso_ba_linearize_all(H, 0, &newE));
        RUN(ldso_ba_calc_lm_energies(H, &newM, &newL));
        elog.push_back(newE);
        done = it + 1;
        if (newE + newL + newM < lastE + lastL + lastM) {
            RUN(ldso_ba_apply_res(H));
            lastE = newE; lastL = newL; lastM = newM;
            lambda *= 0.25;
        } else {
            RUN(ldso_ba_load_state_backup(H));
            RUN(ldso_ba_linearize_all(H, 0, &lastE));
            H->pendingApply = false;
            RUN(ldso_ba_calc_lm_energies(H, &lastM, &lastL));
            lambda *= 1e2;
        }
        if (canbreak && it >= H->settings.minOptIterations && !force_all) break;
    }
    RUN(launch_solve(H, H->sets[H->cur], SK_REANCHOR | SK_ADJ | SK_NONULLSPACE | SK_PRECALC));
    double Efix = 0;
    RUN(ldso_ba_linearize_all(H, 1, &Efix));
    elog.push_back(Efix);
    CHK(hipMemsetAsync(H->B.energyLog, 0, 64 * 8, H->stream));
    CHK(hipMemcpyAsync(H->B.energyLog, elog.data(), elog.size() * sizeof(double), hipMemcpyHostToDevice, H->stream));
    double sc[16];
    RUN(read_scalars(H, sc));
    H->lastIterations = (int) elog.size() - 2;
    if (iters_out) *iters_out = done;
    if (rmse_out) *rmse_out = sqrtf((float) (sc[0] / (8 * sc[9])));
    if (!std::isfinite(sc[0]) || sc[4] != 0.0) return LDSO_E_NONFINITE;
    return LDSO_OK;
}

int ldso_ba_optimize(ldso_ba_t *H, int mnumOptIts, int force_all, float *rmse_out, int *iters_out) {
// ... 111 lines not shown
```

### ldso_amd/csrc/ba_reduce.hip

```cpp
#include <hip/hip_runtime.h>
#include "ba_host.h"

#include "ba_reduce_body.h"

__global__ __launch_bounds__(256) void k_reduce(BaPtrs B, BaDims D, ResSet S, ChunkStarts chunkStart, int hasL, int GSP, int atomicMode,
                                                int hasPrior, float calibPrior, double l1, double il, int itCheck) {
    static_assert(sizeof(BaPtrs) + sizeof(BaDims) + sizeof(ResSet) + sizeof(ChunkStarts) >= 8 * 64 - 60, "k_reduce: ld_touch_kernarg<8> must stay inside the arguments");
    ld_touch_kernarg<8>();
    reduce_body(B, D, S, chunkStart, hasL, GSP, atomicMode, hasPrior, calibPrior, l1, il, itCheck, (int) blockIdx.x);
}

static __device__ __forceinline__ int g_col(int i, int FS) { return (i < 4) ? (8 * FS + i) : (i - 4); }

static __device__ __forceinline__ double sum_f(const double *PC, int F, int base, int stride, int off, double init = 0.0) {
    double q[LD_MAXF];
#pragma unroll
    for (int x = 0; x < LD_MAXF; x++) q[x] = (x < F) ? PC[(size_t) (base + x * stride) * LD_PAIRC + off] : 0.0;
    double v = init;
#pragma unroll
    for (int x = 0; x < LD_MAXF; x++) if (x < F) v += q[x];
    return v;
}
static __device__ __forceinline__ double sum_pairs(const double *PC, int F, int off) {
    double v = 0;
// ... 111 lines not shown
    else if (e < n * n + n) B.bM[e - n * n] += (bA[e - n * n] - bsc[e - n * n]) * w;
}

hipError_t ba_launch_marg_update(const BaPtrs &B, const BaDims &D, double w, hipStream_t st) {
    const int N = D.n * D.n + D.n;
    hipLaunchKernelGGL(k_marg_update, dim3((N + 255) / 256), dim3(256), 0, st, B, D, w);
    return hipGetLastError();
}

__global__ __launch_bounds__(256) void k_marg_frame(BaPtrs B, BaDims D, int idx, double *W, double *outH, double *outb) {
    const int tid = threadIdx.x, n = D.n, nd = n - 8;
    double *Hs = W, *bs = W + (size_t) n * n;
    __shared__ double sSV[8 * LD_MAXF + 4], sHpi[64], sLU[64], sBLI[(8 * LD_MAXF + 4) * 8];
    __shared__ int sPiv[8];
    auto perm = [&](int i) { const int io = 4 + 8 * idx; return (i < io) ? i : (i < nd) ? i + 8 : io + (i - nd); };
    const DevFrame &fh = B.frames[idx];
    for (int e = tid; e < n * n; e += 256) {
        const int i = e / n, j = e % n;
        double v = B.HM[(size_t) perm(i) * n + perm(j)];
        if (i == j && i >= nd) v += fh.prior[i - nd];
        Hs[e] = v;
    }
    for (int i = tid; i < n; i += 256) bs[i] = B.bM[perm(i)] + ((i >= nd) ? fh.prior[i - nd] * fh.delta_prior[i - nd] : 0.0);
    __syncthreads();
    for (int i = tid; i < n; i += 256) sSV[i] = sqrt(fabs(Hs[(size_t) i * n + i]) + 10.0);
    __syncthreads();
    for (int e = tid; e < n * n; e += 256) { const int i = e / n, j = e % n; Hs[e] = (1.0 / sSV[i]) * Hs[e] * (1.0 / sSV[j]); }
    for (int i = tid; i < n; i += 256) bs[i] = (1.0 / sSV[i]) * bs[i];
    __syncthreads();
    if (tid < 64) { const int r = tid >> 3, c = tid & 7; const double v = Hs[(size_t) (nd + r) * n + nd + c]; sLU[tid] = 0.5 * (v + v); }
    __syncthreads();
    if (tid == 0) {
        for (int k = 0; k < 8; k++) {
            int p = k; double best = fabs(sLU[k * 8 + k]);
            for (int i = k + 1; i < 8; i++) if (fabs(sLU[i * 8 + k]) > best) { best = fabs(sLU[i * 8 + k]); p = i; }
            sPiv[k] = p;
            if (p != k) for (int j = 0; j < 8; j++) { double t = sLU[k * 8 + j]; sLU[k * 8 + j] = sLU[p * 8 + j]; sLU[p * 8 + j] = t; }
            for (int i = k + 1; i < 8; i++) {
                sLU[i * 8 + k] /= sLU[k * 8 + k];
                for (int j = k + 1; j < 8; j++) sLU[i * 8 + j] -= sLU[i * 8 + k] * sLU[k * 8 + j];
            }
        }
    }
    __syncthreads();
    if (tid < 8) {
        double x[8];
        for (int i = 0; i < 8; i++) x[i] = (i == tid) ? 1.0 : 0.0;
        for (int k = 0; k < 8; k++) { const int p = sPiv[k]; if (p != k) { double t = x[k]; x[k] = x[p]; x[p] = t; } }
        for (int i = 0; i < 8; i++) for (int j = 0; j < i; j++) x[i] -= sLU[i * 8 + j] * x[j];
        for (int i = 7; i >= 0; i--) { for (int j = i + 1; j < 8; j++) x[i] -= sLU[i * 8 + j] * x[j]; x[i] /= sLU[i * 8 + i]; }
        for (int i = 0; i < 8; i++) sHpi[i * 8 + tid] = x[i];
    }
    __syncthreads();
    if (tid < 64) sHpi[tid] = 0.5 * (sHpi[tid] + sHpi[tid]);
    __syncthreads();
    for (int e = tid; e < nd * 8; e += 256) {
        const int i = e >> 3, c = e & 7;
        double s_ = 0;
        for (int k = 0; k < 8; k++) s_ += Hs[(size_t) (nd + k) * n + i] * sHpi[k * 8 + c];
        sBLI[e] = s_;
    }
    __syncthreads();
    for (int e = tid; e < nd * (nd + 1); e += 256) {
        const int i = e / (nd + 1), j = e % (nd + 1);
        const double *bl = sBLI + i * 8;
        double s_ = 0;
        if (j < nd) { for (int k = 0; k < 8; k++) s_ += bl[k] * Hs[(size_t) (nd + k) * n + j]; Hs[(size_t) i * n + j] -= s_; }
        else { for (int k = 0; k < 8; k++) s_ += bl[k] * bs[nd + k]; bs[i] -= s_; }
    }
    __syncthreads();
    for (int e = tid; e < nd * nd; e += 256) {
        const int i = e / nd, j = e % nd;
        outH[e] = 0.5 * (sSV[i] * Hs[(size_t) i * n + j] * sSV[j] + sSV[j] * Hs[(size_t) j * n + i] * sSV[i]);
    }
    for (int i = tid; i < nd; i += 256) outb[i] = sSV[i] * bs[i];
}

hipError_t ba_launch_marg_frame(const BaPtrs &B, const BaDims &D, int idx, double *work, double *outH, double *outb, hipStream_t st) {
    hipLaunchKernelGGL(k_marg_frame, dim3(1), dim3(256), 0, st, B, D, idx, work, outH, outb);
    return hipGetLastError();
}

__global__ __launch_bounds__(256) void k_acc_init(BaPtrs B, BaDims D, GnInit gi) {
    const int n = D.n, e = blockIdx.x * blockDim.x + threadIdx.x;
    if (e >= n * n + n) return;
    double v = 0.0;
    if (e < n * n && gi.enable == 1) {
        const int i = e / n, j = e % n;
        if (j <= i) {
            if (gi.hasPrior) v = B.HM[e];
            if (i == j) v += (i < 4) ? (double) gi.calibPrior : B.frames[(i - 4) >> 3].prior[(i - 4) & 7];
        }
    }
    B.acc[e] = v;
}

hipError_t ba_launch_acc_init(const BaPtrs &B, const BaDims &D, const GnInit &gi, hipStream_t st) {
    const int N = D.n * D.n + D.n;
    hipLaunchKernelGGL(k_acc_init, dim3((N + 255) / 256), dim3(256), 0, st, B, D, gi);
    return hipGetLastError();
}
```

### ldso_amd/csrc/ba_reduce_body.h

```cpp
#pragma once
#include <hip/hip_runtime.h>
#include "ba_dev.h"

typedef float f32x4 __attribute__((ext_vector_type(4)));
#define SC_SLAB 128
#define PA_SLICES 2
#define PA_UNROLL 24
#define SCT_KS LD_SCT_KS
#define SCT_SLAB 512
#define SC_MAXT 12

__host__ __device__ constexpr int tri13r(int r, int c) { return r * 13 - (r * (r - 1)) / 2 + (c - r); }
__host__ __device__ constexpr size_t reduce_atomic_lds_bytes() { return (size_t) (2 * SCT_SLAB * 16 + SCT_SLAB) * sizeof(float); }

static __device__ __forceinline__ void acc_add(double *p, double v) { __hip_atomic_fetch_add(p, v, __ATOMIC_RELAXED, __HIP_MEMORY_SCOPE_AGENT); }

template <int NT, int W> static __device__ __forceinline__ void schur_wave(const float *sG, int GSP, int cnt, int wcol, int li, int lk, f32x4 *acc);

static __device__ __forceinline__ void reduce_body(const BaPtrs &B, const BaDims &D, const ResSet &S, const ChunkStarts &chunkStart, int hasL, int GSP, int atomicMode,
                                   int hasPrior, float calibPrior, double l1, double il, int itCheck, const int bid) {
    if (LD_ITER_SKIPPED(B, itCheck)) return;
    const int F = D.F, FS = D.FS;
    const int nPairBlocks = reduce_pairs(F, hasL);
    const int tid = threadIdx.x;
    __shared__ double sA[13 * 13];
    __shared__ double sT[2][64];
    const long long t0_ = wall_clock64();
#define RSTAMP(i) do { if (LD_STAMP_ON && tid == 0) B.energyLog[(i)] = (double) (wall_clock64() - t0_); } while (0)

    if (bid < nPairBlocks) {
        const int which = bid / (F * F);
        const int pair = bid % (F * F);
        const int h = pair / F, t = pair % F;
        const float *part = which ? S.topL : S.topA;
        const int c0 = chunkStart.v[h], c1 = chunkStart.v[h + 1];
        if (bid == 0 && c1 > c0) RSTAMP(22);
        __shared__ double sAH[64], sAT[64];
        __shared__ double sPart[PA_SLICES][LD_TOPN];
        if (tid >= 128 && tid < 192) { sAH[tid - 128] = B.adHost[(size_t) (h + t * F) * 64 + (tid - 128)]; }
        if (tid >= 192) { sAT[tid - 192] = B.adTarget[(size_t) (h + t * F) * 64 + (tid - 192)]; }
        const int slice = tid / LD_TOPN, ent = tid % LD_TOPN;
        if (slice < PA_SLICES) {
            double a = 0;
            for (int cb = c0 + slice; cb < c1; cb += PA_SLICES * PA_UNROLL) {
                float q[PA_UNROLL];
#pragma unroll
                for (int u = 0; u < PA_UNROLL; u++) {
                    const int c = cb + u * PA_SLICES, cc = max(min(c, c1 - 1), 0);
                    const float v = part[((unsigned) cc * (unsigned) FS + (unsigned) t) * LD_TOPN + (unsigned) ent];
                    q[u] = (c < c1) ? v : 0.0f;
                }
#pragma unroll
                for (int u = 0; u < PA_UNROLL; u++) a += (double) q[u];
            }
            sPart[slice][ent] = a;
            if (bid == 0 && a != 12345.678) RSTAMP(23);
        }
        __syncthreads();
        if (bid == 0) RSTAMP(20);
        if (tid < LD_TOPN) {
            double a = sPart[0][tid];
#pragma unroll
            for (int sl = 1; sl < PA_SLICES; sl++) a += sPart[sl][tid];
            int r = 0, rem = tid;
            while (rem >= 13 - r) { rem -= 13 - r; r++; }
            int cidx = r + rem;
            sA[r * 13 + cidx] = a;
            sA[cidx * 13 + r] = a;
        }
        __syncthreads();
        double *out = B.pairC + ((size_t) which * F * F + pair) * LD_PAIRC;
        const double *AH = sAH, *AT = sAT;
        if (tid < 64) {
            int i = tid >> 3, j = tid & 7;
            double th = 0, tt = 0;
            for (int m = 0; m < 8; m++) { th += AH[i * 8 + m] * sA[(4 + m) * 13 + 4 + j]; tt += AT[i * 8 + m] * sA[(4 + m) * 13 + 4 + j]; }
            sT[0][tid] = th; sT[1][tid] = tt;
        }
        __syncthreads();
        const int n = D.n;
        double *accT = B.acc, *accb = B.acc + (size_t) n * n;
        const int rh = 4 + 8 * h, rt = 4 + 8 * t;
        if (tid < 64) {
            int i = tid >> 3, j = tid & 7;
            double hh = 0, tt = 0, ht = 0;
            for (int m = 0; m < 8; m++) { hh += sT[0][i * 8 + m] * AH[j * 8 + m]; tt += sT[1][i * 8 + m] * AT[j * 8 + m]; ht += sT[0][i * 8 + m] * AT[j * 8 + m]; }
            if (!atomicMode) { out[tid] = hh; out[64 + tid] = tt; out[128 + tid] = ht; }
            else {
                if (i >= j) { const double dsc = (i == j) ? l1 : 1.0; acc_add(&accT[(size_t) (rh + i) * n + rh + j], hh * dsc); acc_add(&accT[(size_t) (rt + i) * n + rt + j], tt * dsc); }
                if (h > t) acc_add(&accT[(size_t) (rh + i) * n + rt + j], ht);
                else if (h < t) acc_add(&accT[(size_t) (rt + j) * n + rh + i], ht);
            }
        } else if (tid < 64 + 32) {
            int e = tid - 64, i = e >> 2, c = e & 3;
            double hc = 0, tc = 0;
            for (int m = 0; m < 8; m++) { hc += AH[i * 8 + m] * sA[(4 + m) * 13 + c]; tc += AT[i * 8 + m] * sA[(4 + m) * 13 + c]; }
            if (!atomicMode) { out[192 + e] = hc; out[224 + e] = tc; }
            else { acc_add(&accT[(size_t) (rh + i) * n + c], hc); acc_add(&accT[(size_t) (rt + i) * n + c], tc); }
        } else if (tid < 96 + 16) {
            int e = tid - 96;
            if (!atomicMode) out[256 + e] = sA[(e >> 2) * 13 + (e & 3)];
            else if ((e >> 2) >= (e & 3)) acc_add(&accT[(size_t) (e >> 2) * n + (e & 3)], sA[(e >> 2) * 13 + (e & 3)] * (((e >> 2) == (e & 3)) ? l1 : 1.0));
        } else if (tid < 112 + 8) {
            int i = tid - 112;
            double bh = 0, bt = 0;
            for (int m = 0; m < 8; m++) { bh += AH[i * 8 + m] * sA[(4 + m) * 13 + 12]; bt += AT[i * 8 + m] * sA[(4 + m) * 13 + 12]; }
            if (!atomicMode) { out[272 + i] = bh; out[280 + i] = bt; }
            else { acc_add(&accb[rh + i], bh); acc_add(&accb[rt + i], bt); }
        } else if (tid < 120 + 4) {
            int i = tid - 120;
            if (!atomicMode) out[288 + i] = sA[i * 13 + 12];
            else acc_add(&accb[i], sA[i * 13 + 12]);
        }
        if (bid == 0) RSTAMP(21);
        return;
    }

    const int nSplitBase = nPairBlocks;
    const int KS = D.ks;
    if (atomicMode && bid < nSplitBase + reduce_tiles(KS, GSP)) {
        extern __shared__ __attribute__((aligned(16))) float sT_[];
        float *sAc = sT_, *sBc = sAc + SCT_SLAB * 16, *sWc = sBc + SCT_SLAB * 16;
        const int bb = bid - nSplitBase, tile = bb / KS, ks = bb % KS;
        const int nT = GSP / 16, GS = D.GS, n = D.n;
        int ti = 0, rem = tile;
        while (rem >= nT - ti) { rem -= nT - ti; ti++; }
        const int tj = ti + rem;
        const int P0 = D.pBegin, Pn = D.pEnd - D.pBegin, per = ((Pn + KS - 1) / KS + 3) & ~3;
        const int pa = P0 + ks * per, pb = min(P0 + Pn, pa + per);
        const int wave = tid >> 6, lane = tid & 63, li = lane & 15, lk = lane >> 4;
        const int wcol = 8 * FS + 5;
        f32x4 acc = (f32x4){0.f, 0.f, 0.f, 0.f}, acc2 = acc;
        for (int base = pa; base < pb; base += SCT_SLAB) {
            const int cnt = min(SCT_SLAB, pb - base), rows = (cnt + 3) & ~3;
            __syncthreads();
            {
                float4 q[16];
                float wq[2];
#pragma unroll
                for (int u = 0; u < 16; u++) {
                    const int e = tid + u * 256, r = e >> 3, half = (e >> 2) & 1, c4 = e & 3;
                    const int col = (half ? tj : ti) * 16 + c4 * 4;
                    const float4 v = *(const float4 *) (S.G + (unsigned) ((base + min(r, cnt - 1)) * GS + min(col, GS - 4)));
                    const bool in = r < cnt && col < GS;
                    q[u] = make_float4(in ? v.x : 0.f, in ? v.y : 0.f, in ? v.z : 0.f, in ? v.w : 0.f);
                }
#pragma unroll
                for (int u = 0; u < 2; u++) { const int r = tid + u * 256; const float v = S.G[(unsigned) ((base + min(r, cnt - 1)) * GS + wcol)]; wq[u] = (r < cnt) ? v : 0.f; }
#pragma unroll
                for (int u = 0; u < 16; u++) {
                    const int e = tid + u * 256, r = e >> 3, half = (e >> 2) & 1, c4 = e & 3;
                    if (r < rows) *(float4 *) ((half ? sBc : sAc) + r * 16 + c4 * 4) = q[u];
                }
#pragma unroll
                for (int u = 0; u < 2; u++) { const int r = tid + u * 256; if (r < rows) sWc[r] = wq[u]; }
            }
            __syncthreads();
            if (bb == 0) RSTAMP(25);
#pragma unroll 4
            for (int k0 = wave * 4; k0 < rows; k0 += 32) {
                const int k1 = k0 + 16;
                const float a0 = sAc[(k0 + lk) * 16 + li] * sWc[k0 + lk], b0 = sBc[(k0 + lk) * 16 + li];
                const bool in1 = k1 < rows;
                const int k1c = in1 ? k1 : k0;
                const float a1 = in1 ? sAc[(k1c + lk) * 16 + li] * sWc[k1c + lk] : 0.f, b1 = sBc[(k1c + lk) * 16 + li];
                acc = __builtin_amdgcn_mfma_f32_16x16x4f32(a0, b0, acc, 0, 0, 0);
                acc2 = __builtin_amdgcn_mfma_f32_16x16x4f32(a1, b1, acc2, 0, 0, 0);
            }
        }
        __syncthreads();
        if (bb == 0) RSTAMP(26);
        float *sR = sT_;
#pragma unroll
        for (int r = 0; r < 4; r++) sR[wave * 256 + (lk * 4 + r) * 16 + li] = acc[r] + acc2[r];
        __syncthreads();
        {
            const float v = ((sR[tid] + sR[256 + tid]) + sR[512 + tid]) + sR[768 + tid];
            const int rr = ti * 16 + (tid >> 4), cc = tj * 16 + (tid & 15);
            const int F8 = 8 * D.F, FS8 = 8 * FS;
            const int I = (rr < F8) ? 4 + rr : (rr >= FS8 && rr < FS8 + 4) ? rr - FS8 : (rr == FS8 + 4) ? n : -1;
            const int J = (cc < F8) ? 4 + cc : (cc >= FS8 && cc < FS8 + 4) ? cc - FS8 : (cc == FS8 + 4) ? n : -1;
            const bool use = !(ti == tj && rr > cc) && I >= 0 && J >= 0 && I != n;
            if (use) {
                if (J == n) acc_add(&B.acc[(size_t) n * n + I], -(double) v);
                else acc_add(&B.acc[(size_t) max(I, J) * n + min(I, J)], -(double) v * il);
            }
        }
        if (bb == 0) RSTAMP(27);
        return;
    }
    if (atomicMode == 2) return;
    if (atomicMode) {
        const int n = D.n;
        __shared__ double sDelta[8 * LD_MAXF + 4];
        if (tid < n) sDelta[tid] = (tid < 4) ? (double) B.calib->cDeltaF[tid] : B.frames[(tid - 4) >> 3].delta[(tid - 4) & 7];
        double prb = 0, prH = 0, bm = 0;
        if (tid < n) {
            if (tid < 4) { prH = (double) calibPrior; prb = (double) calibPrior * (double) B.calib->cDeltaF[tid]; }
            else { const DevFrame &f = B.frames[(tid - 4) >> 3]; prH = f.prior[(tid - 4) & 7]; prb = prH * f.delta_prior[(tid - 4) & 7]; }
            if (hasPrior) bm = B.bM[tid];
        }
        const int rowT = tid >> 2, quarter = tid & 3;
        constexpr int QW = 16;
        double hq[QW];
        const int per = (n + 3) >> 2, j0 = quarter * per;
        const bool rowOn = hasPrior && rowT < n && 4 * n <= 256;
#pragma unroll
        for (int u = 0; u < QW; u++) hq[u] = (rowOn && u < per && j0 + u < n) ? B.HM[(size_t) rowT * n + j0 + u] : 0.0;
        __syncthreads();
        double part = 0;
#pragma unroll
        for (int u = 0; u < QW; u++) if (u < per && j0 + u < n) part += hq[u] * sDelta[j0 + u];
        part += __shfl_xor(part, 1, 64); part += __shfl_xor(part, 2, 64);
        __shared__ double sHd[8 * LD_MAXF + 4];
        if (quarter == 0 && rowT < n) sHd[rowT] = part;
        __syncthreads();
        if (tid < n) {
            double s_ = 0;
            if (hasPrior) {
                s_ = bm;
                if (4 * n <= 256) s_ += sHd[tid];
                else for (int j0_ = 0; j0_ < n; j0_ += 16) {
                    double q[16];
#pragma unroll
                    for (int u = 0; u < 16; u++) q[u] = (j0_ + u < n) ? B.HM[(size_t) tid * n + j0_ + u] : 0.0;
#pragma unroll
                    for (int u = 0; u < 16; u++) if (j0_ + u < n) s_ += q[u] * sDelta[j0_ + u];
                }
            }
            acc_add(&B.acc[(size_t) n * n + tid], prb + s_);
            const double dterm = prH + (hasPrior ? B.HM[(size_t) tid * n + tid] : 0.0);
            acc_add(&B.acc[(size_t) tid * n + tid], dterm * (l1 - 1.0));
        }
        RSTAMP(28);
        return;
    }

    extern __shared__ __attribute__((aligned(16))) float sG[];
    const int sp = bid - nSplitBase;
    const int wave = tid >> 6, lane = tid & 63;
    const int nT = GSP / 16;
    const int P0 = D.pBegin, Pn = D.pEnd - D.pBegin;
    const int per = (Pn + LD_SC_SPLITS - 1) / LD_SC_SPLITS;
    const int pa = P0 + sp * per, pb = min(P0 + Pn, pa + per);
    const int GS = D.GS;
    const int li = lane & 15, lk = lane >> 4;
    float *Mout = B.scPart + (size_t) sp * GSP * GSP;
    f32x4 acc[SC_MAXT];
#pragma unroll
    for (int q = 0; q < SC_MAXT; q++) acc[q] = (f32x4){0.f, 0.f, 0.f, 0.f};
    for (int base = pa; base < pb; base += SC_SLAB) {
        const int cnt = min(SC_SLAB, pb - base);
        __syncthreads();
        {
            const int g4 = GS >> 2, p4 = GSP >> 2;
            const int rows = (cnt + 3) & ~3;
            for (int e0 = tid; e0 < rows * p4; e0 += 256 * 8) {
                float4 q[8];
#pragma unroll
                for (int u = 0; u < 8; u++) {
                    const int e = e0 + u * 256, r = e / p4, c = e % p4;
                    q[u] = make_float4(0.f, 0.f, 0.f, 0.f);
                    if (e < rows * p4 && r < cnt && c < g4) q[u] = ((const float4 *) (S.G + (size_t) (base + r) * GS))[c];
                }
#pragma unroll
                for (int u = 0; u < 8; u++) { const int e = e0 + u * 256; if (e < rows * p4) ((float4 *) sG)[e] = q[u]; }
            }
        }
// ... 61 lines not shown
```

### ldso_amd/csrc/ba_solve.hip

```cpp
#include <hip/hip_runtime.h>
#include "ba_host.h"
#include "lie_dev.h"

#include "ba_reduce_body.h"
#define NT 256
#define TH_CAP 8192
#define LD_THRESH_DOUBLES ((256 + 8 + TH_CAP) / 2)

static __device__ __forceinline__ double wave_sum(double v) {
    for (int o = 32; o > 0; o >>= 1) v += __shfl_xor(v, o, 64);
    return v;
}
template <int CTRL> static __device__ __forceinline__ double dpp_f64(double v) {
    const unsigned long long u = __builtin_bit_cast(unsigned long long, v);
    const unsigned lo = (unsigned) __builtin_amdgcn_update_dpp(0, (int) (u & 0xFFFFFFFFu), CTRL, 0xF, 0xF, true);
    const unsigned hi = (unsigned) __builtin_amdgcn_update_dpp(0, (int) (u >> 32), CTRL, 0xF, 0xF, true);
    return __builtin_bit_cast(double, ((unsigned long long) hi << 32) | lo);
}
static __device__ __forceinline__ double readlane_d(double v, int lane) {
    const unsigned long long u = __builtin_bit_cast(unsigned long long, v);
    const unsigned lo = (unsigned) __builtin_amdgcn_readlane((int) (u & 0xFFFFFFFFu), lane), hi = (unsigned) __builtin_amdgcn_readlane((int) (u >> 32), lane);
    return __builtin_bit_cast(double, ((unsigned long long) hi << 32) | lo);
}
static __device__ __forceinline__ double wave_sum_dpp(double v) {
// ... 428 lines not shown

struct SolveLds { size_t sW, sEv, end; };
static __host__ __device__ constexpr SolveLds solve_lds(int n) {
    SolveLds o{};
    o.sW = 0;
    o.sEv = o.sW + 96;
    o.end = o.sW + 7 * (size_t) n + 64;
    return o;
}
static __host__ __device__ constexpr size_t solve_lds_bytes(int n) { return (core_lds_end(LD_SOLVE_NB(n), n) + solve_lds(n).end) * sizeof(double) + LD_LDS_SLACK; }

#define LD_SW_DOUBLES 64
#define LD_SW_RED 8
#define LD_TAIL_KI 8
#define LD_TAIL_FLAG 20
static __host__ __device__ constexpr bool gn_mirrors_adjoints(int F) { return F <= 8; }
static __host__ __device__ constexpr int gn_ad_floats(int F) { return F * F * LD_AD_LDS_PITCH; }
struct GnLds { size_t sW, sFr, sCal, ldsAd; };
static __host__ __device__ constexpr GnLds gn_lds(int F) {
    GnLds o{};
    o.sW = 0;
    o.sFr = o.sW + LD_SW_DOUBLES * sizeof(double);
    o.sCal = o.sFr + F * sizeof(DevFrame);
    o.ldsAd = o.sCal + sizeof(DevCalib);
    return o;
}
static __host__ __device__ constexpr size_t gn_lds_end(int F) { return gn_lds(F).ldsAd + (gn_mirrors_adjoints(F) ? 2 * gn_ad_floats(F) * sizeof(float) : 0); }
struct GnStatsLds { size_t sW, sTh, end; };
static __host__ __device__ constexpr GnStatsLds gn_stats_lds() {
    GnStatsLds o{};
    o.sW = 0;
    o.sTh = o.sW + LD_SW_DOUBLES * sizeof(double);
    o.end = o.sTh + LD_THRESH_DOUBLES * sizeof(double);
    return o;
}
static __host__ __device__ constexpr size_t gn_lds_bytes(int F, int n) {
    const size_t role0 = core_lds_end(LD_SOLVE_NB(n), n) * sizeof(double) + gn_lds_end(F), role1 = gn_stats_lds().end;
    return (role0 > role1 ? role0 : role1) + LD_LDS_SLACK;
}

static constexpr bool lds_layouts_ok() {
    size_t solvePrev = 0, gnPrev = 0;
    for (int F = 1; F <= LD_MAXF; F++) {
        const int n = 8 * F + 4;
        const CoreLds c = core_lds(LD_SOLVE_NB(n), n);
        const SolveLds s = solve_lds(n);
        const GnLds g = gn_lds(F);
        if ((c.sD | c.sY | c.sFp | c.sGp | c.sPn | c.sSc | c.sx | c.sNs | c.end | s.sW | s.sEv) % 2 != 0 || (g.sW | g.sFr | g.sCal | g.ldsAd | gn_stats_lds().sTh) % 16 != 0 || LD_XFP % 4 != 0 || g.ldsAd != g.sCal + sizeof(DevCalib)) return false;
        if (c.sTail * sizeof(double) + 3 * 2 * LD_XFP * sizeof(float) > c.sSc * sizeof(double)) return false;
        if (LD_THRESH_DOUBLES > c.end || 37 * (size_t) F * F > c.end || s.sEv + 12 > s.end || s.sW + 14 * 6 > s.sEv) return false;
        if (solve_lds_bytes(n) < solvePrev || (F != 9 && gn_lds_bytes(F, n) < gnPrev)) return false;
        solvePrev = solve_lds_bytes(n); gnPrev = gn_lds_bytes(F, n);
    }
    return true;
}
static_assert(lds_layouts_ok(), "solve kernels: an offset lost its alignment, an alias outgrew what it lies over, or a smaller window needs more LDS than a larger one");
typedef double __attribute__((ext_vector_type(4))) ld_d4;

template <int NB, int C, bool GN, bool WAIT = false, bool MF = false>
static __device__ __forceinline__ void solve_core(const BaPtrs &B, const BaDims &D, const ResSet &S, const ldso_settings_t &St, int iteration, double *sm, SolveIO &io) {
    constexpr int M = 16 * NB;
    constexpr int CP = C + 2;
    constexpr int NTILE = NB * (NB + 1) / 2;
    static_assert(MF == (NB == 4) && C == solve_cols(NB), "core_lds lays the panel buffers out for this variant");
    constexpr CoreLds lds = core_lds(NB, 0);
    constexpr int LSZ = (int) (lds.sD - lds.sL);
    const double TINY = 2.2250738585072014e-308;
    const int tid = threadIdx.x, ty = tid >> 4, tx = tid & 15, F = D.F, n = D.n;
    double *sL = sm + lds.sL, *sD = sm + lds.sD, *sY = sm + lds.sY, *sFp = sm + lds.sFp, *sGp = sm + lds.sGp, *sPn = sm + lds.sPn, *sSc = sm + lds.sSc, *sx = sm + lds.sx, *sNs = sm + lds.sNs;
    const double *HF = B.sys + 3 * (n * n + n), *bF = HF + n * n;
    const bool ortho = (St.solverMode & LDSO_SOLVER_ORTHOGONALIZE_X) || (iteration >= 2 && (St.solverMode & LDSO_SOLVER_ORTHOGONALIZE_X_LATER));

    double v[NTILE], dI[NB], dJ[NB], dS = 0.0;
    static_assert(!MF || (NB == 4 && C == 4), "the MFMA variant is written for the 64x64 system, 4 columns per round");
    const int lane = tid & 63, wv = __builtin_amdgcn_readfirstlane(tid >> 6);
    constexpr int NS = MF ? 3 : 1;
    int mta[NS], mtb[NS];
    if constexpr (MF) {
        mta[0] = (0x3210 >> (4 * wv)) & 15; mta[1] = (0xF321 >> (4 * wv)) & 15; mta[2] = (0xF332 >> (4 * wv)) & 15;
        mtb[0] = 0; mtb[1] = (0xF111 >> (4 * wv)) & 15; mtb[2] = (0xF322 >> (4 * wv)) & 15;
    } else { mta[0] = 15; mtb[0] = 0; }
    ld_d4 Dv[NS];
    if (GN) { HF = B.acc; bF = HF + (size_t) n * n; }
#define LD_LOAD_H() do { \
        const int nn_ = n * n + n - 1; \
_Pragma("unroll") \
        for (int a = 0; a < NB; a++) { \
            const int i = ty + 16 * a, j = tx + 16 * a; \
            const double vi = HF[min(i * n + i, nn_)], vj = HF[min(j * n + j, nn_)]; \
            dI[a] = (i < n) ? vi : 0.0; \
            dJ[a] = (j < n) ? vj : 0.0; \
        } \
_Pragma("unroll") \
        for (int a = 0; a < NB; a++) \
_Pragma("unroll") \
            for (int b = 0; b <= a; b++) { \
                const int i = ty + 16 * a, j = tx + 16 * b; \
                const double q = HF[min(i * n + j, nn_)]; \
                v[a * (a + 1) / 2 + b] = (j < n && (!GN || j <= i) && i <= n) ? q : 0.0; \
            } \
        { const double q = HF[min(tid * n + tid, nn_)]; dS = (tid < n) ? q : 0.0; } \
    } while (0)
#define LD_LOAD_H_MF() do { \
        const int nn_ = n * n + n - 1; \
_Pragma("unroll") \
        for (int s_ = 0; s_ < NS; s_++) \
_Pragma("unroll") \
            for (int r = 0; r < 4; r++) { \
                const int i = 16 * mta[s_] + (lane >> 4) + 4 * r, j = 16 * mtb[s_] + (lane & 15); \
                const double q = HF[min(i * n + j, nn_)]; \
                Dv[s_][r] = (mta[s_] < NB && j < n && (!GN || j <= i) && i <= n) ? q : 0.0; \
            } \
        { const double q = HF[min(tid * n + tid, nn_)]; dS = (tid < n) ? q : 0.0; } \
    } while (0)
    constexpr bool waitH = GN && WAIT;
    if constexpr (!waitH) { if constexpr (MF) { LD_LOAD_H_MF(); } else { LD_LOAD_H(); } }
    double nsv[4];
    if (ortho) {
#pragma unroll
        for (int u = 0; u < 4; u++) { const int i = tid + u * NT; nsv[u] = (i < 7 * n) ? B.nsProj[i] : 0.0; }
    }
    if (GN) {
        constexpr int FW = (int) (sizeof(DevFrame) / 4), CW = (int) (sizeof(DevCalib) / 4), MW = (LD_MAXF * FW + NT - 1) / NT;
        unsigned mw[MW];
        const unsigned *gF = (const unsigned *) B.frames;
#pragma unroll
        for (int u = 0; u < MW; u++) { const int i = tid + u * NT; mw[u] = (i < F * FW) ? gF[i] : 0u; }
        const unsigned cw = (tid < CW) ? ((const unsigned *) B.calib)[tid] : 0u;
        float4 ah[4], at[4];
        if (io.ldsAd != nullptr) {
#pragma unroll
            for (int u = 0; u < 4; u++) {
                const int i = tid + u * NT;
                ah[u] = (i < F * F * 16) ? ((const float4 *) B.adHostF)[i] : make_float4(0, 0, 0, 0);
                at[u] = (i < F * F * 16) ? ((const float4 *) B.adTargetF)[i] : make_float4(0, 0, 0, 0);
            }
        }
        double ns = 0, nc = 0;
        for (int c = tid; c < D.nChunks; c += NT) { ns += (double) S.chunkNID[c * 2]; nc += (double) S.chunkNID[c * 2 + 1]; }
        unsigned *lF = (unsigned *) io.fr;
#pragma unroll
        for (int u = 0; u < MW; u++) { const int i = tid + u * NT; if (i < F * FW) lF[i] = mw[u]; }
        if (tid < CW) ((unsigned *) io.cal)[tid] = cw;
        if (io.ldsAd != nullptr) {
            float4 *lh = (float4 *) io.ldsAd, *lt = (float4 *) (io.ldsAd + gn_ad_floats(F));
#pragma unroll
            for (int u = 0; u < 4; u++) { const int i = tid + u * NT, sl = i >> 4, j = ((sl % F) * F + sl / F) * (LD_AD_LDS_PITCH / 4) + (i & 15); if (i < F * F * 16) { lh[j] = ah[u]; lt[j] = at[u]; } }
            io.adH = io.ldsAd; io.adT = io.ldsAd + gn_ad_floats(F); io.adPitch = LD_AD_LDS_PITCH;
        }
        for (int o = 32; o > 0; o >>= 1) { double a_ = __shfl_xor(ns, o, 64), b_ = __shfl_xor(nc, o, 64); ns += a_; nc += b_; }
        if ((tid & 63) == 0) { io.sRed[tid >> 6] = ns; io.sRed[4 + (tid >> 6)] = nc; }
    }
    if (ortho) {
#pragma unroll
        for (int u = 0; u < 4; u++) { const int i = tid + u * NT; if (i < 7 * n) sNs[i] = nsv[u]; }
    }
    if (NB == 4) {
        for (int i = tid; i < LSZ / 2; i += NT) st2(&sL[2 * i], 0.0, 0.0);
    }
    if constexpr (waitH) {
        if (LD_STAMP_ON && tid == 0) B.energyLog[47] = (double) wall_clock64();
        if (tid == 0) {
            while (__hip_atomic_load(io.waitCtr, __ATOMIC_RELAXED, __HIP_MEMORY_SCOPE_AGENT) < io.waitTarget) __builtin_amdgcn_s_sleep(1);
            __hip_atomic_store(io.waitCtr, 0, __ATOMIC_RELAXED, __HIP_MEMORY_SCOPE_AGENT);
        }
        __syncthreads();
        __builtin_amdgcn_fence(__ATOMIC_ACQUIRE, "agent");
        if (LD_STAMP_ON && tid == 0) B.energyLog[48] = (double) wall_clock64();
        if constexpr (MF) { LD_LOAD_H_MF(); } else { LD_LOAD_H(); }
    }
    if (tid < M) sSc[tid] = fast_rsqrt(dS + 10.0);
    if constexpr (MF) {
        __syncthreads();
#pragma unroll
        for (int s_ = 0; s_ < NS; s_++) {
            const double sj = sSc[min(16 * mtb[s_] + (lane & 15), M - 1)];
#pragma unroll
            for (int r = 0; r < 4; r++) {
                const int i = 16 * mta[s_] + (lane >> 4) + 4 * r;
                const double si = (i == n) ? 1.0 : sSc[min(i, M - 1)];
                Dv[s_][r] = si * Dv[s_][r] * sj;
            }
        }
#pragma unroll
        for (int s_ = 0; s_ < NS; s_++) {
            if (mta[s_] >= NB || mtb[s_] != 0) continue;
            if ((lane & 15) < C) {
#pragma unroll
                for (int r = 0; r < 4; r++) sFp[(16 * mta[s_] + (lane >> 4) + 4 * r) * CP + (lane & 15)] = Dv[s_][r];
            }
        }
    } else {
        double sI[NB], sJ[NB];
#pragma unroll
        for (int a = 0; a < NB; a++) { sI[a] = (ty + 16 * a == n) ? 1.0 : fast_rsqrt(dI[a] + 10.0); sJ[a] = fast_rsqrt(dJ[a] + 10.0); }
#pragma unroll
        for (int a = 0; a < NB; a++)
#pragma unroll
// ... 450 lines not shown
            }
            if (LD_STAMP_ON && lane == 0) B.energyLog[63] = (double) wall_clock64();
        }
        if (LD_STAMP_ON && tid == 64) B.energyLog[58] = (double) wall_clock64();
    }
    if (!split) {
        __syncthreads();
        for (int i = tid; i < F * F; i += NT) pair_record<false>(B, fr, C, F, i, sKi);
    }
    __syncthreads();
}

template <bool WAIT>
static __device__ __forceinline__ void gn_solve_body(const BaPtrs &B, const BaDims &D, const ResSet &S, const ldso_settings_t &St, const SolveArgs &A, const int role) {
    extern __shared__ __attribute__((aligned(16))) double sm[];
    const int tid = threadIdx.x, F = D.F, n = D.n;
    char *const top = (char *) (sm + core_lds_end(LD_SOLVE_NB(n), n));
    if (LD_ITER_SKIPPED(B, A.itCheck)) return;
    const long long t0_ = wall_clock64();
#define GSTAMP(i) do { if (LD_STAMP_ON && tid == 0) B.energyLog[40 + (i)] = (double) (wall_clock64() - t0_); } while (0)
    if (role == 1) {
        constexpr GnStatsLds lds = gn_stats_lds();
        double *sW1 = (double *) ((char *) sm + lds.sW);
        int *sTh = (int *) ((char *) sm + lds.sTh);
        if (A.reduceIn != nullptr) {
            const double *sc = A.reduceIn;
            if (tid == 0) { B.scalars[0] = sc[0]; B.scalars[1] = sc[1]; B.scalars[2] = sc[2]; B.scalars[6] = sc[3]; B.scalars[7] = sc[4]; B.scalars[9] = sc[5]; B.scalars[10] = sc[6]; }
            __syncthreads();
            post_thresh(B, D, S, St, A.reduceIn + 8, sTh);
        } else {
            post_sums(B, D, S, sW1);
            GSTAMP(10);
            res_counts(B, D, S, sW1);
            GSTAMP(11);
            post_thresh(B, D, S, St, nullptr, sTh);
            GSTAMP(12);
        }
        if (tid == 0 && A.logIdx >= 0 && A.logIdx < 64) B.energyLog[A.logIdx] = B.scalars[0];
        return;
    }
    const GnLds lds = gn_lds(F);
    double *sW = (double *) (top + lds.sW);
    DevFrame *sFr = (DevFrame *) (top + lds.sFr);
    DevCalib *sCal = (DevCalib *) (top + lds.sCal);
    if (LD_STAMP_ON && tid == 0) B.energyLog[39] = (double) t0_;
    SolveIO io;
    io.fr = sFr; io.cal = sCal; io.adH = B.adHostF; io.adT = B.adTargetF; io.adPitch = 64; io.sRed = sW; io.sumNID = 0; io.lambda = A.lambda; io.hasPrior = A.hasPrior; io.redScalars = A.reduceIn; io.waitCtr = A.waitCtr; io.waitTarget = A.waitTarget;
    io.ldsAd = gn_mirrors_adjoints(F) ? (float *) (sCal + 1) : nullptr;
    if (tid == 0) *(int *) ((float *) (sW + LD_SW_RED) + LD_TAIL_FLAG) = 0;
    solve_core_dispatch<true, WAIT>(B, D, S, St, A.iteration, sm, io);
    GSTAMP(4);
    GSTAMP(5);
    gn_tail(B, D, sFr, sCal, io, St, (float *) (sW + LD_SW_RED), A.itCheck, A.hostStop, A.lastIt);
    GSTAMP(6);
    {
        unsigned *gF = (unsigned *) B.frames; const unsigned *lF = (const unsigned *) sFr;
        const int W = (int) (sizeof(DevFrame) / 4), skip = (int) (offsetof(DevFrame, frameEnergyTH) / 4);
        const int s0 = (int) (offsetof(DevFrame, state) / 4), dp0 = (int) (offsetof(DevFrame, delta_prior) / 4);
        for (int i = tid; i < F * W; i += NT) {
            const int w = i % W;
            if (w != skip) gF[i] = lF[(w >= s0 && w < s0 + 16) ? i - s0 + dp0 : i];
        }
        unsigned *gC = (unsigned *) B.calib; const unsigned *lC = (const unsigned *) sCal;
        for (int i = tid; i < (int) (sizeof(DevCalib) / 4); i += NT) gC[i] = lC[i];
    }
}

__global__ __launch_bounds__(NT) void k_gn_solve(BaPtrs B, BaDims D, ResSet S, ldso_settings_t St, SolveArgs A) {
    static_assert(sizeof(BaPtrs) + sizeof(BaDims) + sizeof(ResSet) + sizeof(ldso_settings_t) + sizeof(SolveArgs) >= 10 * 64 - 60, "k_gn_solve: ld_touch_kernarg<10> must stay inside the arguments");
    if (LD_SOLVE_NB(D.n) == 4) ld_touch_kernarg<10>();
    gn_solve_body<false>(B, D, S, St, A, (int) blockIdx.x);
}

__global__ __launch_bounds__(NT) void k_reduce_solve(BaPtrs B, BaDims D, ResSet S, ldso_settings_t St, SolveArgs A, ChunkStarts chunkStart, int atomicMode,
                                                     float calibPrior, double l1, double il) {
    static_assert(sizeof(BaPtrs) + sizeof(BaDims) + sizeof(ResSet) + sizeof(ldso_settings_t) + sizeof(SolveArgs) + sizeof(ChunkStarts) + 24 >= 12 * 64 - 60, "k_reduce_solve: ld_touch_kernarg<12> must stay inside the arguments");
    ld_touch_kernarg<12>();
    if (blockIdx.x >= LD_FUSED_CTL) {
        const long long tStart_ = LD_STAMP_ON ? wall_clock64() : 0;
        if (LD_ITER_SKIPPED(B, A.itCheck)) return;
        const ReduceGrid rg = reduce_grid(D.F, A.hasL, D.ks, A.GSP);
        const int q = (int) blockIdx.x - LD_FUSED_CTL;
        const int bid = (q < rg.nTile) ? rg.nPair + q : (q < rg.nTile + rg.nPair) ? q - rg.nTile : q;
        reduce_body(B, D, S, chunkStart, A.hasL, A.GSP, atomicMode, A.hasPrior, calibPrior, l1, il, -1, bid);
        __builtin_amdgcn_s_waitcnt(0);
        __syncthreads();
        if (threadIdx.x == 0) {
            const int prev = __hip_atomic_fetch_add(A.waitCtr, 1, __ATOMIC_RELAXED, __HIP_MEMORY_SCOPE_AGENT);
            if (LD_STAMP_ON && prev == A.waitTarget - 1) { B.energyLog[29] = (double) wall_clock64(); B.energyLog[30] = (double) bid; B.energyLog[31] = (double) tStart_; }
        }
        return;
    }
    gn_solve_body<true>(B, D, S, St, A, (int) blockIdx.x);
}

#define LD_REDB_BLOCKS 4
#define LD_REDB_DENSE_PER_CU 6
static __device__ __forceinline__ void reduce_batch_body(const BatchItem *__restrict__ items, int nWin, int cur, float calibPrior, double l1, double il, int itCheck) {
    int w = 0;
    for (int i = 1; i < nWin; i++) if ((int) blockIdx.x >= items[i].redBlock0) w = i;
    const BatchItem &it = items[w];
    reduce_body(it.B, it.D, it.set[cur], it.cs, 0, it.GSP, 1, it.hasPrior, calibPrior, l1, il, itCheck, (int) blockIdx.x - it.redBlock0);
}
__global__ __launch_bounds__(NT) void k_reduce_batch(const BatchItem *__restrict__ items, int nWin, int cur, float calibPrior, double l1, double il, int itCheck) {
    reduce_batch_body(items, nWin, cur, calibPrior, l1, il, itCheck);
}
__global__ __launch_bounds__(NT, LD_REDB_BLOCKS) void k_reduce_batch_dense(const BatchItem *__restrict__ items, int nWin, int cur, float calibPrior, double l1, double il, int itCheck) {
    reduce_batch_body(items, nWin, cur, calibPrior, l1, il, itCheck);
}

__global__ __launch_bounds__(NT) void k_gn_solve_batch(const BatchItem *__restrict__ items, int cur, ldso_settings_t St, int iteration, double lambda, int logIdx, int itCheck) {
    const BatchItem &it = items[blockIdx.x >> 1];
    SolveArgs A;
    A.iteration = iteration; A.lambda = lambda; A.hasPrior = it.hasPrior; A.GSP = it.GSP; A.logIdx = logIdx; A.itCheck = itCheck;
    gn_solve_body<false>(it.B, it.D, it.set[cur], St, A, (int) (blockIdx.x & 1));
}

__global__ __launch_bounds__(64) void k_batch_begin(const BatchItem *__restrict__ items, int mnumOptIts, int forceAll) {
    const BatchItem &it = items[blockIdx.x];
    it.B.energyLog[threadIdx.x] = 0.0;
    if (threadIdx.x == 0) it.B.scalars[LD_SC_STOP] = (double) (optimize_iteration_cap(it.D.F, mnumOptIts, forceAll) - 1);
}
__global__ __launch_bounds__(NT) void k_solve_batch(const BatchItem *__restrict__ items, ldso_settings_t St, unsigned flags, int phase, int nRoles, double *__restrict__ scalarsOut) {
    const int w = (int) blockIdx.x / nRoles, role = (int) blockIdx.x % nRoles;
    const BatchItem &it = items[w];
    const int stop = (int) it.B.scalars[LD_SC_STOP], applied = stop & 1;
    SolveArgs A;
    A.flags = flags; A.hasPrior = it.hasPrior; A.GSP = it.GSP; A.logIdx = stop + 1 + phase;
    solve_body(it.B, it.D, it.set[applied ^ phase], St, A, nRoles, role);
    if (scalarsOut != nullptr) {
        __syncthreads();
        if (threadIdx.x < 16) scalarsOut[(size_t) it.outSlot * 16 + threadIdx.x] = it.B.scalars[threadIdx.x];
    }
}

hipError_t ba_launch_reduce_batch(const BatchItem *d_items, int nWin, int totalBlocks, int cur, float calibPrior, double l1, double il, hipStream_t st, int itCheck) {
    static int numCU[64] = {0};
    int dev = 0;
    if (hipGetDevice(&dev) != hipSuccess || dev < 0 || dev >= 64) dev = 0;
    if (numCU[dev] == 0) { int cu = 0; if (hipDeviceGetAttribute(&cu, hipDeviceAttributeMultiprocessorCount, dev) != hipSuccess || cu <= 0) cu = 256; numCU[dev] = cu; }
    return launch_lds(totalBlocks >= LD_REDB_DENSE_PER_CU * numCU[dev] ? k_reduce_batch_dense : k_reduce_batch, dim3(totalBlocks), dim3(NT), reduce_atomic_lds_bytes(), st,
                      d_items, nWin, cur, calibPrior, l1, il, itCheck);
}

hipError_t ba_launch_gn_solve_batch(const BatchItem *d_items, int nWin, const BaDims &Dmax, int cur, const ldso_settings_t &St, int iteration, double lambda, hipStream_t st, int logIdx, int itCheck) {
    return launch_lds(k_gn_solve_batch, dim3(2 * nWin), dim3(NT), gn_lds_bytes(Dmax.F, Dmax.n), st, d_items, cur, St, iteration, lambda, logIdx, itCheck);
}

hipError_t ba_launch_batch_begin(const BatchItem *d_items, int nWin, int mnumOptIts, int forceAll, hipStream_t st) {
    hipLaunchKernelGGL(k_batch_begin, dim3(nWin), dim3(64), 0, st, d_items, mnumOptIts, forceAll);
    return hipGetLastError();
}

hipError_t ba_launch_solve_batch(const BatchItem *d_items, int nWin, const BaDims &Dmax, const ldso_settings_t &St, unsigned flags, int phase, double *d_scalarsOut, hipStream_t st) {
    const int nRoles = solve_roles(flags);
    return launch_lds(k_solve_batch, dim3(nRoles * nWin), dim3(NT), solve_lds_bytes(Dmax.n), st, d_items, St, flags, phase, nRoles, d_scalarsOut);
}

__global__ __launch_bounds__(NT) void k_gn_export(BaPtrs B, BaDims D, ResSet S, double *tail) {
    __shared__ double sW[16];
    const int tid = threadIdx.x;
    if (blockIdx.x == 0) {
        post_sums(B, D, S, sW);
        res_counts(B, D, S, sW);
        if (tid == 0) { tail[0] = B.scalars[0]; tail[1] = B.scalars[1]; tail[2] = B.scalars[2]; tail[3] = B.scalars[6]; tail[4] = B.scalars[7];
                        tail[5] = B.scalars[9]; tail[6] = B.scalars[10]; tail[7] = 0; }
        return;
    }
    const int i = (blockIdx.x - 1) * NT + tid;
// ... 123 lines not shown
```

### ldso_amd/csrc/ba_window.hip

```cpp
#include "ba_host.h"

struct WinXfer { void *dst; unsigned long long src; unsigned long long words; };
#define LD_XFER_ZERO 0xFFFFFFFFFFFFFFFFull
#define LD_XFER_MAX 96
__global__ __launch_bounds__(256) void k_win_scatter(const char *__restrict__ arena, int nEntries) {
    const WinXfer *tab = reinterpret_cast<const WinXfer *>(arena);
    for (int e = 0; e < nEntries; e++) {
        const WinXfer x = tab[e];
        unsigned *dst = static_cast<unsigned *>(x.dst);
        const size_t n = (size_t) x.words, stride = (size_t) gridDim.x * blockDim.x;
        if (x.src == LD_XFER_ZERO) { for (size_t i = (size_t) blockIdx.x * blockDim.x + threadIdx.x; i < n; i += stride) dst[i] = 0u; }
        else {
            const unsigned *src = reinterpret_cast<const unsigned *>(arena + x.src);
            for (size_t i = (size_t) blockIdx.x * blockDim.x + threadIdx.x; i < n; i += stride) dst[i] = src[i];
        }
    }
}
__global__ __launch_bounds__(256) void k_point_stats(PtRec *__restrict__ a, PtRec *__restrict__ b, const float *__restrict__ mrb, const int32_t *__restrict__ ngr, int P) {
    const int i = blockIdx.x * blockDim.x + threadIdx.x;
    if (i >= P) return;
    const float m = mrb[i]; const int32_t g = ngr[i];
    a[i].maxRelBS = m; a[i].numGood = g; b[i].maxRelBS = m; b[i].numGood = g;
}
struct WinDelta {
// ... 95 lines not shown
    if (src.empty()) return LDSO_OK;
    CHK(hipMemcpyAsync(dst, src.data(), src.size() * sizeof(T), hipMemcpyHostToDevice, H->stream));
    return LDSO_OK;
}
#define H2D(dst, vec) do { int r_ = h2d(H, (dst), (vec)); if (r_ != LDSO_OK) return r_; } while (0)

int build_chunks(ldso_ba *H) {
    BaDims &D = H->D;
    int CH = 4;
    if (!H->chunkCuts.empty() && H->chunkCuts.back() != D.pEnd) H->chunkCuts.clear();
    const std::vector<int32_t> &cuts = H->chunkCuts;
    if (!cuts.empty()) CH = 1 << 30;
    else if (H->chunkPoints > 0) CH = H->chunkPoints;
    else for (;; CH += 4) {
        int cnt = 0, run = 0, prev = -1;
        for (int q = D.pBegin; q < D.pEnd; q++) { int hq = H->h_phost[q]; if (hq != prev) { cnt += (run + CH - 1) / CH; run = 0; prev = hq; } run++; }
        cnt += (run + CH - 1) / CH;
        if (cnt <= H->numCU || CH >= 1024) break;
    }
    std::vector<int32_t> p0, cn, ch, cs(D.F + 1, 0);
    int p = D.pBegin;
    size_t ci = 0;
    for (int hst = 0; hst < D.F; hst++) {
        cs[hst] = (int) p0.size();
        while (p < D.pEnd && H->h_phost[p] == hst) {
            int e = p;
            while (ci < cuts.size() && cuts[ci] <= p) ci++;
            const int stop = ci < cuts.size() ? cuts[ci] : D.pEnd;
            while (e < D.pEnd && H->h_phost[e] == hst && e - p < CH && e < stop) e++;
            p0.push_back(p); cn.push_back(e - p); ch.push_back(hst);
            p = e;
        }
    }
    cs[D.F] = (int) p0.size();
    REQ(p == D.pEnd, "ldso_ba_set_window: points must be ordered by host frame (EnergyFunctional::allPoints order)");
    REQ((int) p0.size() <= H->maxChunks, "too many chunks");
    D.nChunks = (int) p0.size();
    H2D(H->B.chunk_p0, p0); H2D(H->B.chunk_n, cn); H2D(H->B.chunk_host, ch); H2D(H->d_chunkStart, cs);
    H->h_blocks.resize(p0.size());
    for (size_t i = 0; i < p0.size(); i++) H->h_blocks[i] = BatchBlock{0, p0[i], cn[i], ch[i] | ((int32_t) i << 8)};
    CHK(hipMemcpyAsync(H->d_blocks, H->h_blocks.data(), p0.size() * sizeof(BatchBlock), hipMemcpyHostToDevice, H->stream));
    for (int i = 0; i <= LD_MAXF; i++) H->chunkStarts.v[i] = (i <= D.F) ? cs[i] : cs[D.F];
    {
        LinHead &L = H->linHead;
        memset(&L, 0, sizeof(L));
        L.CH = CH; L.F = D.F;
        int q = D.pBegin;
        for (int hst = 0; hst <= LD_MAXF; hst++) {
            L.cs[hst] = (hst <= D.F) ? cs[hst] : cs[D.F];
            L.hostP0[hst] = q;
            while (hst < D.F && q < D.pEnd && H->h_phost[q] == hst) q++;
        }
        bool ok = true;
        for (size_t i = 0; i < p0.size() && ok; i++) {
            const int hst = ch[i];
            ok = p0[i] == L.hostP0[hst] + ((int) i - L.cs[hst]) * CH && cn[i] == std::min(CH, L.hostP0[hst + 1] - p0[i]);
        }
        H->linHeadOk = ok;
    }
    CHK(hipStreamSynchronize(H->stream));
    return LDSO_OK;
}

int rechunk(ldso_ba *H) {
    H->itemValid = false;
    RUN(build_chunks(H));
    if (H->appliedValid && !H->pendingApply) { RUN(launch_linearize(H, false, 4, -1)); H->cur ^= 1; }
    return LDSO_OK;
}

extern "C" {

int ldso_ba_set_window(ldso_ba_t *H, int F, const int32_t *image_slot, int P, const ldso_point_t *pts, int R, const ldso_residual_t *res,
                       const ldso_rawjac_t *linJ, const float *lin_rtz) {
    REQ(H && image_slot && pts && res, "ldso_ba_set_window: null argument");
    REQ(F >= 2 && F <= H->maxF && P >= 1 && P <= H->maxP && R >= 0, "ldso_ba_set_window: window exceeds the handle's capacity");
    CHK(hipSetDevice(H->device));
    BaDims &D = H->D;
    BaPtrs &B = H->B;
    struct WinGuard { ldso_ba *H; bool ok; ~WinGuard() { if (!ok) { H->D.P = 0; H->D.R = 0; H->R = 0; H->appliedValid = false; H->itemValid = false; } } } guard{H, false};
    D.F = F; D.FS = (F + 7) / 8 * 8; D.P = P; D.R = R; D.n = 8 * F + 4; D.GS = 8 * D.FS + LD_GEXTRA; D.w = H->w; D.h = H->h; D.nsg = D.FS / 8; D.ks = H->reduceSplits;
    D.pBegin = 0; D.pEnd = P; D.wM3G = (float) (H->w - 3); D.hM3G = (float) (H->h - 3);
    H->GSP = (D.GS + 15) / 16 * 16;
    H->R = R;
    H->imageSlot.assign(image_slot, image_slot + F);
    for (int f = 0; f < F; f++) {
        REQ(image_slot[f] >= 0 && image_slot[f] < H->maxF && H->imgSlots[image_slot[f]] != nullptr, "ldso_ba_set_window: image slot not set");
        B.img[f] = H->imgSlots[image_slot[f]];
    }
    const int FS = D.FS;
    const size_t PS = (size_t) P * FS;
    size_t nLin = 0;
    for (int i = 0; i < R; i++) nLin += res[i].is_linearized ? 1 : 0;
    REQ(nLin == 0 || (linJ && lin_rtz), "ldso_ba_set_window: linearised residual without linJ / lin_res_toZeroF");
    auto A16 = [](size_t b) { return (b + 15) & ~(size_t) 15; };
    const size_t tabBytes = A16(LD_XFER_MAX * sizeof(WinXfer));
    const size_t need = tabBytes + A16((size_t) P * sizeof(PtGeo)) + A16((size_t) P * 8 * sizeof(PtCw)) + A16((size_t) P * 4) + A16(PS * sizeof(SlotTab)) + A16(nLin * sizeof(ldso_rawjac_t)) + A16(nLin * 32)
                      + A16(PS * sizeof(SlotRec)) + 64;
    if (need > H->stageCap) {
        CHK(hipStreamSynchronize(H->stream));
        if (H->h_stage) hipHostFree(H->h_stage);
        if (H->d_stage) hipFree(H->d_stage);
        H->h_stage = nullptr; H->d_stage = nullptr; H->stageCap = 0;
        const size_t cap = need + need / 4;
        CHK(hipHostMalloc((void **) &H->h_stage, cap));
        CHK(hipMalloc((void **) &H->d_stage, cap));
        H->stageCap = cap;
    }
    if (H->stageBusy) { CHK(hipStreamSynchronize(H->stream)); H->stageBusy = false; }
    WinStage W{H->h_stage, H->stageCap, tabBytes, reinterpret_cast<WinXfer *>(H->h_stage), 0};
    PtGeo *geo = W.put(B.pgeo, P);
    PtCw *pcw = W.put(B.pcw, (size_t) P * 8);
    int32_t *phost = W.put(B.phost, P);
    SlotTab *tab = W.put(B.rtab, PS);
    ldso_rawjac_t *Jl = W.put(B.Jlin, nLin);
    float *rtz = W.put(B.rtz, nLin * 8);
    SlotRec *sr = W.put(H->sets[0].slot, PS);
    REQ(geo && pcw && phost && tab && Jl && rtz && sr, "ldso_ba_set_window: staging arena too small (internal)");
    H->h_phost.resize(P);
    for (int i = 0; i < P; i++) {
        PtGeo g_;
        memset(&g_, 0, sizeof(g_));
        g_.u = pts[i].u; g_.v = pts[i].v; g_.priorF = pts[i].priorF; g_.idepth = pts[i].idepth; g_.idepth_zero = pts[i].idepth_zero; g_.idepth_backup = pts[i].idepth;
        geo[i] = g_;
        REQ(pts[i].host >= 0 && pts[i].host < F, "ldso_ba_set_window: point host out of range");
        H->h_phost[i] = pts[i].host; phost[i] = pts[i].host;
        for (int k = 0; k < 8; k++) pcw[(size_t) i * 8 + k] = PtCw{pts[i].color[k], pts[i].weights[k]};
    }
    memset(sr, 0, PS * sizeof(SlotRec));
    for (size_t q = 0; q < PS; q++) { tab[q] = SlotTab{-1, 0, 0, -1}; sr[q].e[LD_SM_STATE].m.i = LDSO_RES_OOB; }
    H->flat2slot.assign(R, -1);
    size_t nl = 0;
    for (int i = 0; i < R; i++) {
        const ldso_residual_t &r = res[i];
        REQ(r.point >= 0 && r.point < P && r.target >= 0 && r.target < F && r.host == pts[r.point].host && r.target != r.host, "ldso_ba_set_window: bad residual indices");
        size_t slot = (size_t) r.point * FS + r.target;
        REQ(tab[slot].rflat < 0, "ldso_ba_set_window: two residuals of one point target the same frame");
        tab[slot].rflat = i; tab[slot].rlin = r.is_linearized ? 1 : 0; tab[slot].rnew = r.is_new ? 1 : 0;
        sr[slot].e[LD_SM_STATE].m.i = r.state_state; sr[slot].e[LD_SM_ACTIVE].m.i = r.is_active ? 1 : 0; sr[slot].e[LD_SM_ENERGY].m.f = r.state_energy;
        H->flat2slot[i] = (int32_t) slot;
        if (r.is_linearized) {
            tab[slot].rlidx = (int32_t) nl;
            Jl[nl] = linJ[i];
            for (int k = 0; k < 8; k++) rtz[nl * 8 + k] = lin_rtz[(size_t) i * 8 + k];
            nl++;
            const ldso_rawjac_t &J = linJ[i];
            float v0 = J.JIdx2[0] * J.Jpdd[0] + J.JIdx2[1] * J.Jpdd[1], v1 = J.JIdx2[2] * J.Jpdd[0] + J.JIdx2[3] * J.Jpdd[1];
            for (int k = 0; k < 6; k++) sr[slot].e[k].jp = J.Jpdxi[0][k] * v0 + J.Jpdxi[1][k] * v1;
            sr[slot].e[6].jp = J.JabJIdx[0] * J.Jpdd[0] + J.JabJIdx[1] * J.Jpdd[1];
            sr[slot].e[7].jp = J.JabJIdx[2] * J.Jpdd[0] + J.JabJIdx[3] * J.Jpdd[1];
        }
    }
    D.nL = (int) nLin;
    H->hasL = D.nL > 0;
    H->cur = 0; H->pendingApply = false; H->appliedValid = false;
    bool okT = W.again(H->sets[1].slot, sr, PS);
    for (int s_ = 0; s_ < 2; s_++) {
        ResSet &S = H->sets[s_];
        okT = okT && W.zero(S.pt, (size_t) P) && W.zero(S.acc, (size_t) P) && W.zero(S.G, (size_t) P * D.GS);
    }
    okT = okT && W.zero(B.HM, (size_t) D.n * D.n) && W.zero(B.bM, (size_t) D.n) && W.zero(B.scalars, (size_t) 16)
              && W.zero(B.scPart, (size_t) LD_SC_SPLITS * H->GSP * H->GSP);
    REQ(okT, "ldso_ba_set_window: upload table overflow (internal)");
    H->hasPrior = false;
    CHK(hipMemcpyAsync(H->d_stage, H->h_stage, W.used, hipMemcpyHostToDevice, H->stream));
    hipLaunchKernelGGL(k_win_scatter, dim3(256), dim3(256), 0, H->stream, (const char *) H->d_stage, W.n);
// ... 55 lines not shown
                REQ(from < oD.P && from > lastOld, "ldso_ba_update_window: surviving points must keep their order");
                lastOld = from;
                host = oldToNew[H->h_phost[from]];
                REQ(host >= 0, "ldso_ba_update_window: a surviving point is hosted by a frame that left the window");
            } else {
                REQ(-1 - from == nextFresh && nextFresh < n_fresh, "ldso_ba_update_window: fresh points must be numbered in window order");
                host = fresh[nextFresh].host;
                REQ(host >= 0 && host < F, "ldso_ba_update_window: fresh point host out of range");
                const int cnt = __builtin_popcount(res_mask[i]);
                freshResBegin[nextFresh] = fr;
                for (int c = 0; c < cnt; c++) {
                    REQ(fr < n_fresh_res && fresh_res[fr].target >= 0 && fresh_res[fr].target < F && fresh_res[fr].host == host,
                        "ldso_ba_update_window: fresh residual names a target outside the window or another host than its point's");
                    REQ(fresh_res[fr].point == nextFresh && !fresh_res[fr].is_linearized && ((res_mask[i] >> fresh_res[fr].target) & 1u)
                        && (c == 0 || fresh_res[fr - 1].target < fresh_res[fr].target), "ldso_ba_update_window: fresh residuals must be point-major, target-ascending and match res_mask");
                    fr++;
                }
                nextFresh++;
            }
            REQ((res_mask[i] & ~fmask) == 0 && !((res_mask[i] >> host) & 1u), "ldso_ba_update_window: res_mask names a frame outside the window or the host itself");
            REQ(i == 0 || newHost[i - 1] <= host, "ldso_ba_update_window: points must be ordered by host frame (EnergyFunctional::allPoints order)");
            newHost[i] = host;
            resBegin[i] = acc; acc += __builtin_popcount(res_mask[i]);
        }
        resBegin[P] = acc;
        freshResBegin[n_fresh] = fr;
        REQ(nextFresh == n_fresh && fr == n_fresh_res, "ldso_ba_update_window: unused fresh points / residuals");
    }
    const int R = resBegin[P];
    auto A16 = [](size_t b) { return (b + 15) & ~(size_t) 15; };
    const size_t tabBytes = A16(LD_XFER_MAX * sizeof(WinXfer));
    const size_t deltaBytes = A16((size_t) F * 4) + 2 * A16((size_t) P * 4) + A16(((size_t) P + 1) * 4) + A16((size_t) n_fresh * sizeof(ldso_point_t)) + A16((size_t) n_fresh_res * sizeof(ldso_residual_t))
                              + A16(((size_t) n_fresh + 1) * 4) + 2 * A16((size_t) n_fresh * 4);
    const size_t need = tabBytes + deltaBytes + A16((size_t) P * sizeof(PtGeo)) + A16((size_t) P * 8 * sizeof(PtCw)) + A16((size_t) P * 4) + A16(PS * sizeof(SlotTab)) + A16(PS * sizeof(SlotRec))
                        + 2 * A16((size_t) P * 4) + 64;
    if (need > H->stageCap) {
        CHK(hipStreamSynchronize(H->stream));
        if (H->h_stage) hipHostFree(H->h_stage);
        if (H->d_stage) hipFree(H->d_stage);
        H->h_stage = nullptr; H->d_stage = nullptr; H->stageCap = 0; H->stageBusy = false;
        const size_t cap = need + need / 4;
        CHK(hipHostMalloc((void **) &H->h_stage, cap));
        CHK(hipMalloc((void **) &H->d_stage, cap));
        H->stageCap = cap;
    }
    if (H->stageBusy) { CHK(hipStreamSynchronize(H->stream)); H->stageBusy = false; }
    WinStage W{H->h_stage, H->stageCap, tabBytes, reinterpret_cast<WinXfer *>(H->h_stage), 0};
    int32_t *hFrameFrom = W.raw<int32_t>(F), *hPointFrom = W.raw<int32_t>(P);
    uint32_t *hMask = W.raw<uint32_t>(P);
    int32_t *hResBegin = W.raw<int32_t>((size_t) P + 1);
    ldso_point_t *hFresh = W.raw<ldso_point_t>(n_fresh);
    ldso_residual_t *hFreshRes = W.raw<ldso_residual_t>(n_fresh_res);
    int32_t *hFreshResBegin = W.raw<int32_t>((size_t) n_fresh + 1);
    float *hMrb = W.raw<float>(n_fresh); int32_t *hNgr = W.raw<int32_t>(n_fresh);
    REQ(hFrameFrom && hPointFrom && hMask && hResBegin && hFresh && hFreshRes && hFreshResBegin && hMrb && hNgr, "ldso_ba_update_window: staging arena too small (internal)");
    const size_t upBytes = W.used;
    memcpy(hFrameFrom, frame_from, (size_t) F * 4); memcpy(hPointFrom, point_from, (size_t) P * 4); memcpy(hMask, res_mask, (size_t) P * 4);
    memcpy(hResBegin, resBegin.data(), ((size_t) P + 1) * 4); memcpy(hFreshResBegin, freshResBegin.data(), ((size_t) n_fresh + 1) * 4);
    if (n_fresh) { memcpy(hFresh, fresh, (size_t) n_fresh * sizeof(ldso_point_t)); memcpy(hMrb, fresh_mrb, (size_t) n_fresh * 4); memcpy(hNgr, fresh_ngr, (size_t) n_fresh * 4); }
    if (n_fresh_res) memcpy(hFreshRes, fresh_res, (size_t) n_fresh_res * sizeof(ldso_residual_t));
    BaPtrs &B = H->B;
    PtGeo *geo = W.put(B.pgeo, P);
    PtCw *pcw = W.put(B.pcw, (size_t) P * 8);
    int32_t *phost = W.put(B.phost, P);
    SlotTab *tab = W.put(B.rtab, PS);
    SlotRec *sr = W.put(H->sets[0].slot, PS);
    REQ(geo && pcw && phost && tab && sr, "ldso_ba_update_window: staging arena too small (internal)");
    float *mrb = W.raw<float>(P); int32_t *ngr = W.raw<int32_t>(P);
    REQ(mrb && ngr, "ldso_ba_update_window: staging arena too small (internal)");
    auto dev = [&](const void *hp) { return H->d_stage + (reinterpret_cast<const char *>(hp) - H->h_stage); };
    WinDelta Wd;
    const ResSet &So = H->sets[H->cur];
    Wd.oGeo = B.pgeo; Wd.oPcw = B.pcw; Wd.oHost = B.phost; Wd.oTab = B.rtab; Wd.oSlot = So.slot; Wd.oPt = So.pt; Wd.oF = oD.F; Wd.oFS = oD.FS; Wd.oP = oD.P;
    Wd.frameFrom = (const int32_t *) dev(hFrameFrom); Wd.pointFrom = (const int32_t *) dev(hPointFrom); Wd.resMask = (const uint32_t *) dev(hMask); Wd.resBegin = (const int32_t *) dev(hResBegin);
    Wd.fresh = (const ldso_point_t *) dev(hFresh); Wd.freshRes = (const ldso_residual_t *) dev(hFreshRes); Wd.freshResBegin = (const int32_t *) dev(hFreshResBegin);
    Wd.freshMrb = (const float *) dev(hMrb); Wd.freshNgr = (const int32_t *) dev(hNgr);
    Wd.F = F; Wd.FS = FS; Wd.P = P;
    Wd.geo = (PtGeo *) dev(geo); Wd.pcw = (PtCw *) dev(pcw); Wd.phost = (int32_t *) dev(phost); Wd.tab = (SlotTab *) dev(tab); Wd.sr = (SlotRec *) dev(sr); Wd.mrb = (float *) dev(mrb); Wd.ngr = (int32_t *) dev(ngr);
    struct WinGuard { ldso_ba *H; bool ok; ~WinGuard() { if (!ok) { H->D.P = 0; H->D.R = 0; H->R = 0; H->appliedValid = false; H->itemValid = false; } } } guard{H, false};
    BaDims &D = H->D;
    D.F = F; D.FS = FS; D.P = P; D.R = R; D.n = 8 * F + 4; D.GS = 8 * D.FS + LD_GEXTRA; D.w = H->w; D.h = H->h; D.nsg = D.FS / 8; D.ks = H->reduceSplits;
    D.pBegin = 0; D.pEnd = P; D.wM3G = (float) (H->w - 3); D.hM3G = (float) (H->h - 3); D.nL = 0;
    H->GSP = (D.GS + 15) / 16 * 16;
    H->R = R;
    H->imageSlot.assign(image_slot, image_slot + F);
    for (int f = 0; f < F; f++) B.img[f] = H->imgSlots[image_slot[f]];
    H->h_phost.assign(newHost.begin(), newHost.end());
    H->flat2slot.assign(R, -1);
    for (int i = 0; i < P; i++) { int k = resBegin[i]; for (int t = 0; t < F; t++) if ((res_mask[i] >> t) & 1u) H->flat2slot[k++] = (int32_t) ((size_t) i * FS + t); }
    H->hasL = false; H->cur = 0; H->pendingApply = false; H->appliedValid = false; H->itemValid = false;
    bool okT = W.again(H->sets[1].slot, sr, PS);
    for (int s_ = 0; s_ < 2; s_++) {
        ResSet &S = H->sets[s_];
        okT = okT && W.zero(S.pt, (size_t) P) && W.zero(S.acc, (size_t) P) && W.zero(S.G, (size_t) P * D.GS);
    }
    okT = okT && W.zero(B.HM, (size_t) D.n * D.n) && W.zero(B.bM, (size_t) D.n) && W.zero(B.scalars, (size_t) 16) && W.zero(B.scPart, (size_t) LD_SC_SPLITS * H->GSP * H->GSP);
    REQ(okT, "ldso_ba_update_window: upload table overflow (internal)");
    H->hasPrior = false;
    CHK(hipMemcpyAsync(H->d_stage, H->h_stage, upBytes, hipMemcpyHostToDevice, H->stream));
    hipLaunchKernelGGL(k_win_rebuild, dim3((unsigned) ((PS + 255) / 256)), dim3(256), 0, H->stream, Wd);
    CHK(hipGetLastError());
    hipLaunchKernelGGL(k_win_scatter, dim3(256), dim3(256), 0, H->stream, (const char *) H->d_stage, W.n);
    CHK(hipGetLastError());
    hipLaunchKernelGGL(k_point_stats, dim3((unsigned) ((P + 255) / 256)), dim3(256), 0, H->stream, H->sets[0].pt, H->sets[1].pt, (const float *) Wd.mrb, (const int32_t *) Wd.ngr, P);
    CHK(hipGetLastError());
    CHK(hipStreamSynchronize(H->stream));
    const int rc_ = build_chunks(H);
    guard.ok = (rc_ == LDSO_OK);
    return rc_;
}

int ldso_ba_window_begin(ldso_ba_t *H) {
    REQ(H && H->D.P > 0 && !H->hasL && !H->pendingApply, "ldso_ba_window_begin: no resident window to edit (or linearised residuals / a pending linearisation)");
    ldso_ba::WindowEdit &E = H->edit;
    E = ldso_ba::WindowEdit();
    E.active = true; E.oF = H->D.F; E.oP = H->D.P;
    E.frameGone.assign(E.oF, 0); E.rowGone.assign(E.oP, 0); E.mask.assign(E.oP, 0u);
    for (int i = 0; i < H->R; i++) { const int sl = H->flat2slot[i]; E.mask[sl / H->D.FS] |= 1u << (sl % H->D.FS); }
    return LDSO_OK;
}
#define REQ_EDIT(name) REQ(H && H->edit.active, name ": no edit in progress (ldso_ba_window_begin first)")
int ldso_ba_remove_frame(ldso_ba_t *H, int frame_idx) {
    REQ_EDIT("ldso_ba_remove_frame");
    REQ(frame_idx >= 0 && frame_idx < H->edit.oF && !H->edit.frameGone[frame_idx], "ldso_ba_remove_frame: not a frame of the resident window");
    H->edit.frameGone[frame_idx] = 1;
    for (int r = 0; r < H->edit.oP; r++) { if (H->h_phost[r] == frame_idx) H->edit.rowGone[r] = 1; H->edit.mask[r] &= ~(1u << frame_idx); }
    return LDSO_OK;
}
int ldso_ba_insert_frame(ldso_ba_t *H, int image_slot, int *frame_id_out) {
    REQ_EDIT("ldso_ba_insert_frame");
    REQ(image_slot >= 0 && image_slot < H->maxF && H->imgSlots[image_slot] != nullptr, "ldso_ba_insert_frame: image slot not set");
    REQ(H->edit.oF + (int) H->edit.insertedSlots.size() < 32, "ldso_ba_insert_frame: too many frames in one edit");
    if (frame_id_out) *frame_id_out = H->edit.oF + (int) H->edit.insertedSlots.size();
    H->edit.insertedSlots.push_back(image_slot);
    return LDSO_OK;
}
int ldso_ba_remove_points(ldso_ba_t *H, int n, const int32_t *rows) {
    REQ_EDIT("ldso_ba_remove_points");
    REQ(n >= 0 && (n == 0 || rows), "ldso_ba_remove_points: bad arguments");
    for (int i = 0; i < n; i++) REQ(rows[i] >= 0 && rows[i] < H->edit.oP, "ldso_ba_remove_points: row out of range");
    for (int i = 0; i < n; i++) H->edit.rowGone[rows[i]] = 1;
    return LDSO_OK;
}
static int edit_residuals(ldso_ba *H, int n, const int32_t *rows, const int32_t *targets, bool add, const char *) {
    const int nF = H->edit.oF + (int) H->edit.insertedSlots.size();
    for (int i = 0; i < n; i++) {
        REQ(rows[i] >= 0 && rows[i] < H->edit.oP && targets[i] >= 0 && targets[i] < nF, "residual edit: row / target out of range");
        const bool has = (H->edit.mask[rows[i]] >> targets[i]) & 1u;
        REQ(add ? (!has && targets[i] != H->h_phost[rows[i]] && (targets[i] >= H->edit.oF || !H->edit.frameGone[targets[i]])) : has,
            add ? "ldso_ba_add_residuals: the point already has that residual, or the target is its host / a removed frame" : "ldso_ba_drop_residuals: the point has no such residual");
    }
    for (int i = 0; i < n; i++) { if (add) H->edit.mask[rows[i]] |= 1u << targets[i]; else H->edit.mask[rows[i]] &= ~(1u << targets[i]); }
    return LDSO_OK;
}
int ldso_ba_drop_residuals(ldso_ba_t *H, int n, const int32_t *rows, const int32_t *targets) {
    REQ_EDIT("ldso_ba_drop_residuals");
    REQ(n >= 0 && (n == 0 || (rows && targets)), "ldso_ba_drop_residuals: bad arguments");
    return edit_residuals(H, n, rows, targets, false, "");
}
int ldso_ba_add_residuals(ldso_ba_t *H, int n, const int32_t *rows, const int32_t *targets) {
    REQ_EDIT("ldso_ba_add_residuals");
    REQ(n >= 0 && (n == 0 || (rows && targets)), "ldso_ba_add_residuals: bad arguments");
    return edit_residuals(H, n, rows, targets, true, "");
}
int ldso_ba_add_points(ldso_ba_t *H, int n, const ldso_point_t *pts, const int32_t *before_row, int n_res, const ldso_residual_t *res, const float *mrb, const int32_t *ngr) {
    REQ_EDIT("ldso_ba_add_points");
    REQ(n >= 0 && n_res >= 0 && (n == 0 || (pts && before_row)) && (n_res == 0 || res), "ldso_ba_add_points: bad arguments");
    const int nF = H->edit.oF + (int) H->edit.insertedSlots.size();
    const size_t first = H->edit.fresh.size();
    for (int i = 0; i < n; i++) {
        REQ(before_row[i] >= 0 && before_row[i] <= H->edit.oP && pts[i].host >= 0 && pts[i].host < nF, "ldso_ba_add_points: before_row / host out of range");
        ldso_ba::NewPoint q; q.p = pts[i]; q.before = before_row[i]; q.mrb = mrb ? mrb[i] : 0.0f; q.ngr = ngr ? ngr[i] : 0;
        H->edit.fresh.push_back(q);
    }
    for (int i = 0; i < n_res; i++) {
        if (!(res[i].point >= 0 && res[i].point < n && res[i].target >= 0 && res[i].target < nF && !res[i].is_linearized)) {
            H->edit.fresh.resize(first); ldso_set_error("ldso_ba_add_points: residual names a point / frame outside the call, or is linearised"); return LDSO_E_INVALID;
        }
        H->edit.fresh[first + res[i].point].res.push_back(res[i]);
    }
    return LDSO_OK;
}
int ldso_ba_window_commit(ldso_ba_t *H) {
    REQ_EDIT("ldso_ba_window_commit");
    ldso_ba::WindowEdit &E = H->edit;
    const int nIns = (int) E.insertedSlots.size();
    std::vector<int32_t> idToNew(E.oF + nIns, -1), frameFrom, slots;
    for (int f = 0; f < E.oF; f++) if (!E.frameGone[f]) { idToNew[f] = (int) frameFrom.size(); frameFrom.push_back(f); slots.push_back(H->imageSlot[f]); }
    for (int k = 0; k < nIns; k++) { idToNew[E.oF + k] = (int) frameFrom.size(); frameFrom.push_back(-1); slots.push_back(E.insertedSlots[k]); }
    const int F = (int) frameFrom.size();
    auto translate = [&](uint32_t m) { uint32_t o = 0; for (int f = 0; f < E.oF + nIns; f++) if (((m >> f) & 1u) && idToNew[f] >= 0) o |= 1u << idToNew[f]; return o; };
    std::vector<int> order(E.fresh.size());
    for (size_t i = 0; i < order.size(); i++) order[i] = (int) i;
    std::stable_sort(order.begin(), order.end(), [&](int a, int b) { return E.fresh[a].before < E.fresh[b].before; });
    std::vector<int32_t> pointFrom; std::vector<uint32_t> mask; std::vector<ldso_point_t> fp; std::vector<ldso_residual_t> fr; std::vector<float> fm; std::vector<int32_t> fg;
    size_t nx = 0;
    int rc = LDSO_OK;
    auto emitFresh = [&](int idx) {
        ldso_ba::NewPoint q = E.fresh[idx];
        const int k = (int) fp.size();
        if (idToNew[q.p.host] < 0) { rc = LDSO_E_INVALID; return; }
        q.p.host = idToNew[q.p.host];
        uint32_t m = 0;
        for (ldso_residual_t &r : q.res) { if (idToNew[r.target] < 0) { rc = LDSO_E_INVALID; return; } r.target = idToNew[r.target]; r.host = q.p.host; r.point = k; m |= 1u << r.target; }
        std::sort(q.res.begin(), q.res.end(), [](const ldso_residual_t &a, const ldso_residual_t &b) { return a.target < b.target; });
        fp.push_back(q.p); fm.push_back(q.mrb); fg.push_back(q.ngr);
        for (const ldso_residual_t &r : q.res) fr.push_back(r);
        pointFrom.push_back(-1 - k); mask.push_back(m);
    };
    for (int r = 0; r <= E.oP; r++) {
        while (nx < order.size() && E.fresh[order[nx]].before == r) emitFresh(order[nx++]);
        if (r < E.oP && !E.rowGone[r]) { pointFrom.push_back(r); mask.push_back(translate(E.mask[r])); }
    }
    E.active = false;
    if (rc != LDSO_OK) { ldso_set_error("ldso_ba_window_commit: a fresh point or residual names a removed frame"); return rc; }
    REQ(!pointFrom.empty() && F >= 2, "ldso_ba_window_commit: the edit leaves no window");
    return ldso_ba_update_window(H, F, slots.data(), frameFrom.data(), (int) pointFrom.size(), pointFrom.data(), mask.data(), (int) fp.size(), fp.data(), (int) fr.size(), fr.data(), fm.data(), fg.data());
}

int ldso_ba_set_chunk_points(ldso_ba_t *H, int points_per_workgroup) {
    REQ(H && points_per_workgroup >= 0 && points_per_workgroup % 4 == 0 && points_per_workgroup <= 1024, "ldso_ba_set_chunk_points: 0 or a multiple of 4 up to 1024");
    REQ(!H->pendingApply, "ldso_ba_set_chunk_points: a linearisation is pending (ldso_ba_apply_res first)");
    H->chunkPoints = points_per_workgroup;
    if (H->D.P > 0) { CHK(hipSetDevice(H->device)); return rechunk(H); }
    return LDSO_OK;
}
int ldso_ba_set_reduce_splits(ldso_ba_t *H, int splits) {
    REQ(H && splits >= 1 && splits <= 16, "ldso_ba_set_reduce_splits: bad arguments");
    REQ(!H->inBatch, "ldso_ba_set_reduce_splits: the handle is part of a batch");
    H->reduceSplits = splits; H->D.ks = splits;
    return LDSO_OK;
}

int ldso_ba_get_chunk_cuts(ldso_ba_t *H, int32_t *ends, int cap, int *n_out) {
    REQ(H && n_out && H->D.P > 0, "ldso_ba_get_chunk_cuts: bad arguments / no window");
    const int n = (int) H->h_blocks.size();
    *n_out = n;
    if (ends) { REQ(cap >= n, "ldso_ba_get_chunk_cuts: buffer too small"); for (int i = 0; i < n; i++) ends[i] = H->h_blocks[i].p0 + H->h_blocks[i].np; }
    return LDSO_OK;
}
int ldso_ba_set_chunk_cuts(ldso_ba_t *H, const int32_t *ends, int n) {
    REQ(H && n >= 0 && (n == 0 || ends), "ldso_ba_set_chunk_cuts: bad arguments");
    REQ(!H->pendingApply, "ldso_ba_set_chunk_cuts: a linearisation is pending (ldso_ba_apply_res first)");
    REQ(H->inBatch == nullptr, "ldso_ba_set_chunk_cuts: the handle belongs to a batch (its chunks are the batch's)");
    for (int i = 0; i < n; i++) REQ(ends[i] > (i ? ends[i - 1] : 0) && ends[i] <= (H->D.P > 0 ? H->D.P : H->maxP), "ldso_ba_set_chunk_cuts: ends must ascend and stay inside the window");
    H->chunkCuts.assign(ends, ends + n);
    if (H->D.P > 0) { CHK(hipSetDevice(H->device)); return rechunk(H); }
    return LDSO_OK;
}
int ldso_ba_get_chunk_points(ldso_ba_t *H, int *points_per_workgroup, int *workgroups) {
    REQ(H && points_per_workgroup, "ldso_ba_get_chunk_points: null argument");
    *points_per_workgroup = H->chunkPoints;
    if (workgroups) *workgroups = H->D.nChunks;
    return LDSO_OK;
}

int ldso_ba_set_shard(ldso_ba_t *H, int pb, int pe) {
    REQ(H && pb >= 0 && pe >= pb && pe <= H->D.P, "ldso_ba_set_shard: bad range");
    H->D.pBegin = pb; H->D.pEnd = pe;
    return build_chunks(H);
}

}
```

Before: 29210 GN iters/s.

## Spread fused-reduce accumulator atomics across four Hessian copies summed in solve

The fused GN path now gives the global Hessian accumulator four strided copies. Pair blocks choose a copy by (h+t) mod 4 and Schur tiles by split index, so atomic adds to the same addresses are spread out. The solve kernel sums the copies when loading H. The aim is less double-atomic contention in the reduce, paid for with extra memory, extra init work and four loads per element in the solve.

```diff
diff --git a/ldso_amd/csrc/ba_api.hip b/ldso_amd/csrc/ba_api.hip
--- a/ldso_amd/csrc/ba_api.hip
+++ b/ldso_amd/csrc/ba_api.hip
@@ -144,7 +144,7 @@
     const size_t GSPmax = (8 * FS + LD_GEXTRA + 15) / 16 * 16;
     DA(B.scPart, (size_t) LD_SC_SPLITS * GSPmax * GSPmax);
     DA(B.sys, 4 * (nmax * nmax + nmax));
-    DA(B.acc, nmax * nmax + nmax); H->ownAcc = B.acc;
+    DA(B.acc, (size_t) LD_ACC_COPIES * acc_stride((int) nmax)); H->ownAcc = B.acc;
     DA(B.x, nmax); DA(B.xAd, F * F * 8); DA(B.xc, 4); DA(B.scalars, 16); DA(B.energyLog, 64);
     DA(H->d_dumpJ, P * FS);
     B.dumpJ = nullptr;
@@ -503,7 +503,7 @@
         REQ(!H->pendingApply, "ldso_ba_get_jacobians: a linearisation is pending (call ldso_ba_apply_res first, or enable ldso_ba_set_debug_dump)");
         BaPtrs Bd = H->B;
         Bd.dumpJ = H->d_dumpJ;
-        CHK(ba_launch_linearize(Bd, H->D, H->sets[H->cur], H->sets[H->cur ^ 1], H->settings, H->hasL, false, 0, GnInit{0, 0, 0.0f, -1}, H->stream));
+        CHK(ba_launch_linearize(Bd, H->D, H->sets[H->cur], H->sets[H->cur ^ 1], H->settings, H->hasL, false, 0, GnInit{0, 0, 0.0f, -1, 1}, H->stream));
     }
     D2H(all, H->d_dumpJ, (size_t) H->R);
     CHK(hipStreamSynchronize(H->stream));
diff --git a/ldso_amd/csrc/ba_batch.hip b/ldso_amd/csrc/ba_batch.hip
--- a/ldso_amd/csrc/ba_batch.hip
+++ b/ldso_amd/csrc/ba_batch.hip
@@ -10,6 +10,7 @@
             BatchItem &it = Bt->items[pass * n + i];
             if (pass == 1 && (int) i == Bt->n0) { Bt->halfChunks[0] = lin; Bt->halfReduce[0] = red; lin = 0; red = 0; }
             if (H->B.acc != H->ownAcc) H->B.acc = H->ownAcc;
+            H->accCopiesReady = false;
             it.B = H->B; it.D = H->D; it.D.ks = Bt->ks; it.set[0] = H->sets[H->cur]; it.set[1] = H->sets[H->cur ^ 1]; it.cs = H->chunkStarts;
             it.hasPrior = H->hasPrior ? 1 : 0; it.GSP = H->GSP; it.linBlock0 = lin; it.redBlock0 = red; it.outSlot = (int32_t) i;
             lin += H->D.nChunks;
diff --git a/ldso_amd/csrc/ba_dev.h b/ldso_amd/csrc/ba_dev.h
--- a/ldso_amd/csrc/ba_dev.h
+++ b/ldso_amd/csrc/ba_dev.h
@@ -149,6 +149,7 @@
     int enable, hasPrior;
     float calibPrior;
     int itCheck;
+    int copies;
 };
 
 #define LD_SC_STOP 11
@@ -164,6 +165,7 @@
 #define LD_SC_SPLITS 16
 #define LD_SCT_KS 8
 #define LD_SYS_MATS 4
+#define LD_ACC_COPIES 4
 
 #ifdef __HIPCC__
 struct ReduceGrid { int nPair, nTile, nExtra, total; };
@@ -173,6 +175,7 @@
     const int nTile = reduce_tiles(ks, GSP), nPair = reduce_pairs(F, hasL);
     return ReduceGrid{nPair, nTile, 1, nPair + nTile + 1};
 }
+__host__ __device__ inline int acc_stride(int n) { return (n * n + n + 15) & ~15; }
 #define LD_FUSED_CTL 2
 __host__ __device__ inline int optimize_iteration_cap(int F, int mnumOptIts, int forceAll) {
     if (!forceAll) { if (F < 3) mnumOptIts = 20; if (F < 4) mnumOptIts = 15; }
diff --git a/ldso_amd/csrc/ba_host.h b/ldso_amd/csrc/ba_host.h
--- a/ldso_amd/csrc/ba_host.h
+++ b/ldso_amd/csrc/ba_host.h
@@ -75,6 +75,7 @@
     int selLdsLimit = -1, selLdsSet = 0;
     std::vector<char> selHost;
     double *ownAcc = nullptr;
+    bool accCopiesReady = false;
     ChunkStarts chunkStarts;
     ldso_rawjac_t *d_dumpJ = nullptr;
     std::vector<int32_t> flat2slot;
@@ -183,6 +184,7 @@
 struct Damping { double lam, l1, il; };
 Damping damping(const ldso_settings_t &St, double lambda);
 GnInit gn_init(const ldso_ba *H, int itCheck);
+bool fused_launch_applies(const ldso_ba *H);
 int lend_acc(ldso_ba *H, double *buf);
 template <class Launch> int time_launches(hipStream_t st, int reps, double *avg_us, Launch launch) {
     hipEvent_t a, b;
diff --git a/ldso_amd/csrc/ba_linearize.hip b/ldso_amd/csrc/ba_linearize.hip
--- a/ldso_amd/csrc/ba_linearize.hip
+++ b/ldso_amd/csrc/ba_linearize.hip
@@ -241,7 +241,7 @@
     float *sRec = (float *) (sImg + FS);
 
     if (gi.enable) {
-        const int n = D.n, N1 = n * n + n, per = (N1 + gridBlocks - 1) / gridBlocks;
+        const int n = D.n, stride = acc_stride(n), N1 = (gi.copies - 1) * stride + n * n + n, per = (N1 + gridBlocks - 1) / gridBlocks;
         const int z0 = chunk * per, z1 = min(N1, z0 + per);
         for (int e = z0 + tid; e < z1; e += blockDim.x) {
             double v = 0.0;
@@ -1086,7 +1086,7 @@
     for (int b = b0; b < b1; b++) {
         const BatchBlock bb = blocks[b];
         const BatchItem &it = items[bb.win];
-        GnInit gi; gi.enable = 1; gi.hasPrior = it.hasPrior; gi.calibPrior = calibPrior; gi.itCheck = itCheck;
+        GnInit gi; gi.enable = 1; gi.hasPrior = it.hasPrior; gi.calibPrior = calibPrior; gi.itCheck = itCheck; gi.copies = 1;
         linearize_body<NSG, false, false, false, true>(it.B, it.D, it.set[cur], it.set[cur ^ 1], S, stepMode, gi, nullptr, bb.host_chunk >> 8, it.D.nChunks, bb.p0, bb.np, bb.host_chunk & 0xFF);
         __syncthreads();
     }
@@ -1101,7 +1101,7 @@
         const BatchBlock bb = blocks[b];
         const BatchItem &it = items[bb.win];
         const int applied = __builtin_amdgcn_readfirstlane((int) it.B.scalars[LD_SC_STOP]) & 1;
-        GnInit gi; gi.enable = 1; gi.hasPrior = it.hasPrior; gi.calibPrior = calibPrior; gi.itCheck = -1;
+        GnInit gi; gi.enable = 1; gi.hasPrior = it.hasPrior; gi.calibPrior = calibPrior; gi.itCheck = -1; gi.copies = 1;
         linearize_body<1, false, true, false, true>(it.B, it.D, it.set[applied], it.set[applied ^ 1], S, 0, gi, nullptr, bb.host_chunk >> 8, it.D.nChunks, bb.p0, bb.np, bb.host_chunk & 0xFF);
         __syncthreads();
     }
@@ -1163,7 +1163,7 @@
 hipError_t ba_launch_linearize_marg(const BaPtrs &B, const BaDims &D, const ResSet &cur, const ResSet &nxt, const ldso_settings_t &S, const int32_t *margFlags,
                                     hipStream_t st) {
     if (D.nChunks == 0) return hipSuccess;
-    const GnInit gi{0, 0, 0.0f};
+    const GnInit gi{0, 0, 0.0f, 0, 1};
     if (D.nsg == 1) return launch_one<1, false, false, true>(B, D, cur, nxt, S, 0, gi, st, margFlags);
     return launch_one<2, false, false, true>(B, D, cur, nxt, S, 0, gi, st, margFlags);
 }
diff --git a/ldso_amd/csrc/ba_optimize.hip b/ldso_amd/csrc/ba_optimize.hip
--- a/ldso_amd/csrc/ba_optimize.hip
+++ b/ldso_amd/csrc/ba_optimize.hip
@@ -38,6 +38,7 @@
     } else
     CHK(ba_launch_linearize(H->B, H->D, H->sets[H->cur], H->sets[H->cur ^ 1], H->settings, H->hasL, fix, stepMode, gi, H->stream));
     t_end(H);
+    H->accCopiesReady = gi.copies == LD_ACC_COPIES;
     if (H->profile) { t_begin(H, 4); t_end(H); }
     return LDSO_OK;
 }
@@ -78,13 +79,22 @@
 }
 GnInit gn_init(const ldso_ba *H, int itCheck) {
     GnInit gi; gi.enable = (H->D.pBegin > 0) ? 2 : 1; gi.hasPrior = H->hasPrior ? 1 : 0; gi.calibPrior = H->settings.initialCalibHessian; gi.itCheck = itCheck;
+    gi.copies = fused_launch_applies(H) ? LD_ACC_COPIES : 1;
     return gi;
+}
+bool fused_launch_applies(const ldso_ba *H) {
+    return reduce_grid(H->D.F, H->hasL, H->D.ks, H->GSP).total + LD_FUSED_CTL <= H->numCU && !H->noFusedLaunch && H->B.acc == H->ownAcc;
+}
+static int init_acc(ldso_ba *H) {
+    const GnInit gi = gn_init(H, -1);
+    CHK(ba_launch_acc_init(H->B, H->D, gi, H->stream));
+    H->accCopiesReady = gi.copies == LD_ACC_COPIES;
+    return LDSO_OK;
 }
 int lend_acc(ldso_ba *H, double *buf) {
     if (H->B.acc == buf) return LDSO_OK;
     H->B.acc = buf;
-    CHK(ba_launch_acc_init(H->B, H->D, gn_init(H, -1), H->stream));
-    return LDSO_OK;
+    return init_acc(H);
 }
 
 extern "C" {
@@ -175,7 +185,8 @@
     RUN(lend_acc(H, H->ownAcc));
     SolveArgs A = solve_args(H, 0);
     A.iteration = iteration; A.lambda = lambda; A.logIdx = logIdx; A.itCheck = itCheck; A.hostStop = (itCheck >= 0) ? H->d_stop : nullptr; A.lastIt = lastIt;
-    if (reduce_grid(H->D.F, H->hasL, H->D.ks, H->GSP).total + LD_FUSED_CTL <= H->numCU && !H->noFusedLaunch) {
+    if (fused_launch_applies(H)) {
+        if (!H->accCopiesReady) RUN(init_acc(H));
         A.waitCtr = H->d_waitCtr;
         const Damping d = damping(H->settings, lambda);
         t_begin(H, 2);
@@ -202,8 +213,8 @@
     auto put = [&key](const void *p, size_t n) { const unsigned char *b = (const unsigned char *) p; key.insert(key.end(), b, b + n); };
     put(&H->B, sizeof(H->B)); put(&H->D, sizeof(H->D)); put(H->sets, sizeof(H->sets)); put(&H->settings, sizeof(H->settings));
     put(&H->chunkStarts, sizeof(H->chunkStarts)); put(&H->linHead, sizeof(H->linHead));
-    const long long misc[12] = {first_iteration, iters, H->cur, H->hasL, H->hasPrior, H->GSP, H->linHeadOk, H->noFusedLaunch, H->numCU, (long long) (size_t) H->stream, (long long) (size_t) H->ownAcc,
-                                (long long) (size_t) H->d_waitCtr};
+    const long long misc[13] = {first_iteration, iters, H->cur, H->hasL, H->hasPrior, H->GSP, H->linHeadOk, H->noFusedLaunch, H->numCU, (long long) (size_t) H->stream, (long long) (size_t) H->ownAcc,
+                                (long long) (size_t) H->d_waitCtr, H->accCopiesReady};
     put(misc, sizeof(misc));
 }
 static unsigned long long gn_signature(const std::vector<unsigned char> &key) { return fnv1a(1469598103934665603ull, key.data(), key.size()); }
@@ -227,6 +238,7 @@
             CHK(hipGraphLaunch(g.exec, H->stream));
             if (iters & 1) H->cur ^= 1;
             H->appliedValid = true;
+            H->accCopiesReady = fused_launch_applies(H);
             return LDSO_OK;
         }
     const int cur0 = H->cur;
diff --git a/ldso_amd/csrc/ba_reduce.hip b/ldso_amd/csrc/ba_reduce.hip
--- a/ldso_amd/csrc/ba_reduce.hip
+++ b/ldso_amd/csrc/ba_reduce.hip
@@ -217,8 +217,8 @@
 }
 
 __global__ __launch_bounds__(256) void k_acc_init(BaPtrs B, BaDims D, GnInit gi) {
-    const int n = D.n, e = blockIdx.x * blockDim.x + threadIdx.x;
-    if (e >= n * n + n) return;
+    const int n = D.n, e = blockIdx.x * blockDim.x + threadIdx.x, stride = acc_stride(n);
+    if (e >= (gi.copies - 1) * stride + n * n + n) return;
     double v = 0.0;
     if (e < n * n && gi.enable == 1) {
         const int i = e / n, j = e % n;
@@ -231,7 +231,7 @@
 }
 
 hipError_t ba_launch_acc_init(const BaPtrs &B, const BaDims &D, const GnInit &gi, hipStream_t st) {
-    const int N = D.n * D.n + D.n;
+    const int N = (gi.copies - 1) * acc_stride(D.n) + D.n * D.n + D.n;
     hipLaunchKernelGGL(k_acc_init, dim3((N + 255) / 256), dim3(256), 0, st, B, D, gi);
     return hipGetLastError();
 }
diff --git a/ldso_amd/csrc/ba_reduce_body.h b/ldso_amd/csrc/ba_reduce_body.h
--- a/ldso_amd/csrc/ba_reduce_body.h
+++ b/ldso_amd/csrc/ba_reduce_body.h
@@ -18,7 +18,7 @@
 template <int NT, int W> static __device__ __forceinline__ void schur_wave(const float *sG, int GSP, int cnt, int wcol, int li, int lk, f32x4 *acc);
 
 static __device__ __forceinline__ void reduce_body(const BaPtrs &B, const BaDims &D, const ResSet &S, const ChunkStarts &chunkStart, int hasL, int GSP, int atomicMode,
-                                   int hasPrior, float calibPrior, double l1, double il, int itCheck, const int bid) {
+                                   int hasPrior, float calibPrior, double l1, double il, int itCheck, const int bid, const int accCopies = 1) {
     if (LD_ITER_SKIPPED(B, itCheck)) return;
     const int F = D.F, FS = D.FS;
     const int nPairBlocks = reduce_pairs(F, hasL);
@@ -79,7 +79,7 @@
         }
         __syncthreads();
         const int n = D.n;
-        double *accT = B.acc, *accb = B.acc + (size_t) n * n;
+        double *accT = B.acc + (size_t) ((h + t) % accCopies) * acc_stride(n), *accb = accT + (size_t) n * n;
         const int rh = 4 + 8 * h, rt = 4 + 8 * t;
         if (tid < 64) {
             int i = tid >> 3, j = tid & 7;
@@ -181,9 +181,10 @@
             const int I = (rr < F8) ? 4 + rr : (rr >= FS8 && rr < FS8 + 4) ? rr - FS8 : (rr == FS8 + 4) ? n : -1;
             const int J = (cc < F8) ? 4 + cc : (cc >= FS8 && cc < FS8 + 4) ? cc - FS8 : (cc == FS8 + 4) ? n : -1;
             const bool use = !(ti == tj && rr > cc) && I >= 0 && J >= 0 && I != n;
+            double *accK = B.acc + (size_t) (ks % accCopies) * acc_stride(n);
             if (use) {
-                if (J == n) acc_add(&B.acc[(size_t) n * n + I], -(double) v);
-                else acc_add(&B.acc[(size_t) max(I, J) * n + min(I, J)], -(double) v * il);
+                if (J == n) acc_add(&accK[(size_t) n * n + I], -(double) v);
+                else acc_add(&accK[(size_t) max(I, J) * n + min(I, J)], -(double) v * il);
             }
         }
         if (bb == 0) RSTAMP(27);
diff --git a/ldso_amd/csrc/ba_solve.hip b/ldso_amd/csrc/ba_solve.hip
--- a/ldso_amd/csrc/ba_solve.hip
+++ b/ldso_amd/csrc/ba_solve.hip
@@ -534,24 +534,38 @@
     } else { mta[0] = 15; mtb[0] = 0; }
     ld_d4 Dv[NS];
     if (GN) { HF = B.acc; bF = HF + (size_t) n * n; }
+#define LD_SUM_H(dst, off) do { \
+        double q_[NC]; \
+_Pragma("unroll") \
+        for (int c_ = 0; c_ < NC; c_++) q_[c_] = HF[(size_t) c_ * accStride + (off)]; \
+        dst = q_[0]; \
+_Pragma("unroll") \
+        for (int c_ = 1; c_ < NC; c_++) dst += q_[c_]; \
+    } while (0)
 #define LD_LOAD_H() do { \
         const int nn_ = n * n + n - 1; \
+_Pragma("nounroll") \
+        for (int c_ = 0; c_ < NC; c_++) { \
+            const double *Hc_ = HF + (size_t) c_ * accStride; \
 _Pragma("unroll") \
-        for (int a = 0; a < NB; a++) { \
-            const int i = ty + 16 * a, j = tx + 16 * a; \
-            const double vi = HF[min(i * n + i, nn_)], vj = HF[min(j * n + j, nn_)]; \
-            dI[a] = (i < n) ? vi : 0.0; \
-            dJ[a] = (j < n) ? vj : 0.0; \
+            for (int a = 0; a < NB; a++) { \
+                const int i = ty + 16 * a, j = tx + 16 * a; \
+                const double vi = Hc_[min(i * n + i, nn_)], vj = Hc_[min(j * n + j, nn_)]; \
+                const double mi = (i < n) ? vi : 0.0, mj = (j < n) ? vj : 0.0; \
+                dI[a] = c_ ? dI[a] + mi : mi; \
+                dJ[a] = c_ ? dJ[a] + mj : mj; \
+            } \
+_Pragma("unroll") \
+            for (int a = 0; a < NB; a++) \
+_Pragma("unroll") \
+                for (int b = 0; b <= a; b++) { \
+                    const int i = ty + 16 * a, j = tx + 16 * b; \
+                    const double q = Hc_[min(i * n + j, nn_)]; \
+                    const double m = (j < n && (!GN || j <= i) && i <= n) ? q : 0.0; \
+                    v[a * (a + 1) / 2 + b] = c_ ? v[a * (a + 1) / 2 + b] + m : m; \
+                } \
+            { const double q = Hc_[min(tid * n + tid, nn_)], m = (tid < n) ? q : 0.0; dS = c_ ? dS + m : m; } \
         } \
-_Pragma("unroll") \
-        for (int a = 0; a < NB; a++) \
-_Pragma("unroll") \
-            for (int b = 0; b <= a; b++) { \
-                const int i = ty + 16 * a, j = tx + 16 * b; \
-                const double q = HF[min(i * n + j, nn_)]; \
-                v[a * (a + 1) / 2 + b] = (j < n && (!GN || j <= i) && i <= n) ? q : 0.0; \
-            } \
-        { const double q = HF[min(tid * n + tid, nn_)]; dS = (tid < n) ? q : 0.0; } \
     } while (0)
 #define LD_LOAD_H_MF() do { \
         const int nn_ = n * n + n - 1; \
@@ -560,12 +574,15 @@
 _Pragma("unroll") \
             for (int r = 0; r < 4; r++) { \
                 const int i = 16 * mta[s_] + (lane >> 4) + 4 * r, j = 16 * mtb[s_] + (lane & 15); \
-                const double q = HF[min(i * n + j, nn_)]; \
+                double q; \
+                LD_SUM_H(q, min(i * n + j, nn_)); \
                 Dv[s_][r] = (mta[s_] < NB && j < n && (!GN || j <= i) && i <= n) ? q : 0.0; \
             } \
-        { const double q = HF[min(tid * n + tid, nn_)]; dS = (tid < n) ? q : 0.0; } \
+        { double q; LD_SUM_H(q, min(tid * n + tid, nn_)); dS = (tid < n) ? q : 0.0; } \
     } while (0)
     constexpr bool waitH = GN && WAIT;
+    constexpr int NC = waitH ? LD_ACC_COPIES : 1;
+    const int accStride = acc_stride(n);
     if constexpr (!waitH) { if constexpr (MF) { LD_LOAD_H_MF(); } else { LD_LOAD_H(); } }
     double nsv[4];
     if (ortho) {
@@ -1182,9 +1199,10 @@
         const ReduceGrid rg = reduce_grid(D.F, A.hasL, D.ks, A.GSP);
         const int q = (int) blockIdx.x - LD_FUSED_CTL;
         const int bid = (q < rg.nTile) ? rg.nPair + q : (q < rg.nTile + rg.nPair) ? q - rg.nTile : q;
-        reduce_body(B, D, S, chunkStart, A.hasL, A.GSP, atomicMode, A.hasPrior, calibPrior, l1, il, -1, bid);
+        reduce_body(B, D, S, chunkStart, A.hasL, A.GSP, atomicMode, A.hasPrior, calibPrior, l1, il, -1, bid, LD_ACC_COPIES);
         __builtin_amdgcn_s_waitcnt(0);
         __syncthreads();
+        if (LD_STAMP_ON && threadIdx.x == 0 && (bid == rg.nPair || bid == 0)) B.energyLog[bid == 0 ? 33 : 32] = (double) (wall_clock64() - tStart_);
         if (threadIdx.x == 0) {
             const int prev = __hip_atomic_fetch_add(A.waitCtr, 1, __ATOMIC_RELAXED, __HIP_MEMORY_SCOPE_AGENT);
             if (LD_STAMP_ON && prev == A.waitTarget - 1) { B.energyLog[29] = (double) wall_clock64(); B.energyLog[30] = (double) bid; B.energyLog[31] = (double) tStart_; }
diff --git a/ldso_amd/csrc/ba_window.hip b/ldso_amd/csrc/ba_window.hip
--- a/ldso_amd/csrc/ba_window.hip
+++ b/ldso_amd/csrc/ba_window.hip
@@ -201,6 +201,7 @@
     D.F = F; D.FS = (F + 7) / 8 * 8; D.P = P; D.R = R; D.n = 8 * F + 4; D.GS = 8 * D.FS + LD_GEXTRA; D.w = H->w; D.h = H->h; D.nsg = D.FS / 8; D.ks = H->reduceSplits;
     D.pBegin = 0; D.pEnd = P; D.wM3G = (float) (H->w - 3); D.hM3G = (float) (H->h - 3);
     H->GSP = (D.GS + 15) / 16 * 16;
+    H->accCopiesReady = false;
     H->R = R;
     H->imageSlot.assign(image_slot, image_slot + F);
     for (int f = 0; f < F; f++) {
@@ -422,6 +423,7 @@
     D.F = F; D.FS = FS; D.P = P; D.R = R; D.n = 8 * F + 4; D.GS = 8 * D.FS + LD_GEXTRA; D.w = H->w; D.h = H->h; D.nsg = D.FS / 8; D.ks = H->reduceSplits;
     D.pBegin = 0; D.pEnd = P; D.wM3G = (float) (H->w - 3); D.hM3G = (float) (H->h - 3); D.nL = 0;
     H->GSP = (D.GS + 15) / 16 * 16;
+    H->accCopiesReady = false;
     H->R = R;
     H->imageSlot.assign(image_slot, image_slot + F);
     for (int f = 0; f < F; f++) B.img[f] = H->imgSlots[image_slot[f]];
@@ -569,6 +571,7 @@
     REQ(H && splits >= 1 && splits <= 16, "ldso_ba_set_reduce_splits: bad arguments");
     REQ(!H->inBatch, "ldso_ba_set_reduce_splits: the handle is part of a batch");
     H->reduceSplits = splits; H->D.ks = splits;
+    H->accCopiesReady = false;
     return LDSO_OK;
 }
 
```

After: 27960 GN iters/s. -4.3%, worse.
